# yangt1013/SPEINet

Measured on AMD Instinct MI355X. Metric: deblurred 720p frames/sec, higher is better.
Workload: dtype f16 (correlation top2)

## Files before the change

include/speinet_hip.h:

```cpp
#ifndef SPEINET_HIP_H
#define SPEINET_HIP_H

#include <stdint.h>

#ifdef __cplusplus
extern "C" {
#endif

typedef void* spei_stream_t;

#define SPEI_ACT_NONE 0
#define SPEI_ACT_RELU 1
#define SPEI_ACT_GELU 2

#define SPEI_F32 0
#define SPEI_BF16 1
#define SPEI_F16 2

#define SPEI_CONV 0
#define SPEI_CONV_TRANSPOSED 1

int spei_version(void);
const char* spei_last_error(void);
const char* spei_arch(void);

int spei_any_nonzero(const float* x, int64_t n, int32_t* flag, spei_stream_t stream);

int spei_rl_prior(const float* img, float* out, float* scratch, int C, int H, int W, int iters, float lam,
                  spei_stream_t stream);

int spei_conv5_in(const float* img_chw, const float* w, const float* bias, float* out_hwc, int H, int W,
                  int Cout, spei_stream_t stream);

int spei_conv5_out(const float* in_hwc, int ldi, const float* w, const float* bias, float* out_chw, int H,
                   int W, int Cin, spei_stream_t stream);

int spei_igemm_f32(const float* a0, int lda0, int k0, const float* a1, int lda1, int k1, const float* w,
                   const float* bias, float* out, int ldo, const float* residual, int ldr,
                   const float* rowscale, int Hin, int Win, int Hout, int Wout, int N, int ksize, int stride,
                   int pad, int mode, int act, spei_stream_t stream);

int spei_igemm_f32_batched(const float* a0, int lda0, int k0, const float* a1, int lda1, int k1, const float* w,
                           const float* bias, float* out, int ldo, const float* residual, int ldr,
                           const float* rowscale, int Hin, int Win, int Hout, int Wout, int N, int ksize, int stride,
                           int pad, int mode, int act, int batch, spei_stream_t stream);

int spei_conv_slab16(int fmt, const void* a0, int lda0, int k0, const void* a1, int lda1, int k1, int a_fmt,
                     const void* wfrag_hi, const void* wfrag_lo, const float* bias, void* out, int ldo, int out_fmt,
                     const float* residual, int ldr, const float* rowscale, int Hin, int Win, int Hout, int Wout,
                     int N, int ksize, int stride, int pad, int act, int ln_input, spei_stream_t stream);

int spei_conv_slab16_batched(int fmt, const void* a0, int k0, int a_fmt, const void* wfrag, const void* wfrag_lo, const float* bias,
                             void* out, int out_fmt, const float* residual, int batch, int Hin, int Win, int Hout, int Wout, int N,
                             int ksize, int stride, int pad, int act, spei_stream_t stream);

int spei_conv32_ws16(int fmt, const void* a, int a_fmt, const void* wfrag, const float* bias, void* out, int out_fmt, int batch,
                     int H, int W, int act, spei_stream_t stream);

int spei_conv64_ws16(int fmt, const void* a, int a_fmt, const void* wfrag, const float* bias, void* out, int out_fmt, int batch,
                     int H, int W, int act, spei_stream_t stream);

int spei_mlp_fused16(int fmt, const float* x, float* out, const void* w1_frag, const float* b1, const void* w2_frag,
                     const float* b2, int64_t M, spei_stream_t stream);

int spei_convt2_slab16(int fmt, const void* a0, int lda0, int k0, int a_fmt, const void* wfrag00, const void* wfrag01,
                       const void* wfrag10, const void* wfrag11, const float* bias, void* out, int ldo, int out_fmt,
                       int Hin, int Win, int N, int act, spei_stream_t stream);

int spei_convt2_slab16x3(const float* a0, int lda0, int k0, const void* const* whi4, const void* const* wlo4, const float* bias,
                         float* out, int ldo, int Hin, int Win, int N, int act, spei_stream_t stream);

int spei_conv3x3_256_pipe16(int fmt, const float* x, const void* w_frag, const float* bias, const float* residual, float* out,
                            int batch, int H, int W, spei_stream_t stream);

int spei_conv5_out_slab16(int fmt, const void* in, int ldi, int in_fmt, const void* wfrag, const float* bias32, float* out_chw,
                          int H, int W, spei_stream_t stream);

int spei_attn_fused16(int fmt, const float* x, float* out, const void* yhat, const void* wq_frag, const float* bq,
                      const void* wkv_frag, const float* bkv, const void* wproj_frag, const float* bproj,
                      const float* relbias, int H, int W, int shift, spei_stream_t stream);

int spei_attn_win4_16(int fmt, const float* x, float* out, const void* yhat, const void* wq_frag, const float* bq,
                      const void* wkv_frag, const float* bkv, const void* wproj_frag, const float* bproj,
                      const float* relbias, int batch, int H, int W, int shift, spei_stream_t stream);

int64_t spei_frame_metrics_ws_doubles(int H, int W, int border);
int spei_frame_metrics(const unsigned char* out_hwc, const unsigned char* gt_hwc, int H, int W, int border, double* ws, double* result,
                       spei_stream_t stream);

int64_t spei_gate_ws_floats(int H, int W, int C);
int spei_resblock_gates(const void* x1, int x1_fmt, int H, int W, int C, const float* se_w1, const float* se_b1,
                        const float* se_w2, const float* se_b2, const float* cw_w, const float* cw_bn,
                        const float* hc_w, const float* hc_bn, float* s, float* g1, float* g2, float* ws,
                        spei_stream_t stream);
int spei_resblock_apply(const float* x, const void* x1, int x1_fmt, const float* s, const float* g1, const float* g2,
                        const float* extra, float* out, int ldo, int H, int W, int C, spei_stream_t stream);

int spei_resblock_gates_batched(const void* x1, int x1_fmt, int batch, int H, int W, int C, const float* se_w1, const float* se_b1,
                                const float* se_w2, const float* se_b2, const float* cw_w, const float* cw_bn, const float* hc_w,
                                const float* hc_bn, float* s, float* g1, float* g2, float* ws, spei_stream_t stream);
int spei_resblock_apply_batched(const float* x, const void* x1, int x1_fmt, const float* s, const float* g1, const float* g2, float* out,
                                int batch, int H, int W, int C, spei_stream_t stream);

int spei_layernorm256(const float* x, void* y, int out_fmt, const float* gamma, const float* beta, int64_t M,
                      spei_stream_t stream);

int spei_window_attention(const void* q, const void* kv, int io_fmt, const float* relbias, void* out, int H, int W,
                          int shift, spei_stream_t stream);
int spei_window_attention_batched(const void* q, const void* kv, int io_fmt, const float* relbias, void* out, int H, int W,
                                  int shift, int batch, spei_stream_t stream);

int spei_patch_invnorm(const float* f, int ldf, float* inv, int H, int W, int C, spei_stream_t stream);

int64_t spei_corr_ws_floats(int64_t n_lr);
int spei_corr_argmax(const float* lr, int ldl, const float* ref, int ldr, const float* inv_lr,
                     const float* inv_ref, int Hl, int Wl, int Hr, int Wr, int C, float* S, int32_t* arg,
                     float* ws, spei_stream_t stream);

int spei_split16(int fmt, const float* x, int ld, void* hi, void* lo, int64_t M, int C, spei_stream_t stream);
int spei_corr_argmax_bf16(const void* lr_hi, const void* lr_lo, const void* ref_hi, const void* ref_lo,
                          const float* inv_lr, const float* inv_ref, int Hl, int Wl, int Hr, int Wr, int C, float* S,
                          int32_t* arg, float* ws, spei_stream_t stream);

int spei_corr_slab16(int fmt, const void* lr_hi, const void* lr_lo, const void* ref_hi, const void* ref_lo,
                     const float* inv_lr, const float* inv_ref, int Hl, int Wl, int Hr, int Wr, int C, float* S,
                     int32_t* arg, float* ws, spei_stream_t stream);

int spei_corr_slab_top2_16(int fmt, const void* lr16, const void* ref16, const float* inv_lr, const float* inv_ref,
                           int Hl, int Wl, int Hr, int Wr, int C, float* S, int32_t* arg, float* S2, int32_t* arg2,
                           float* ws, spei_stream_t stream);
int64_t spei_corr_diag_ws_floats(int Hl, int Wl, int Hr, int Wr);
int spei_corr_diag_top2_16(int fmt, const void* lr16, const void* ref16, const float* inv_ref, int Hl, int Wl, int Hr, int Wr,
                           int C, float* S, int32_t* arg, float* S2, int32_t* arg2, float* ws, spei_stream_t stream);
int spei_corr_rescore(const float* lr, int ldl, const float* ref, int ldr, const float* inv_lr, const float* inv_ref,
                      int Hl, int Wl, int Hr, int Wr, int C, float* S, int32_t* arg, const float* S2, const int32_t* arg2,
                      spei_stream_t stream);

int spei_gather_fold(const float* ref, int ldr, const int32_t* arg, float* out, int ldo, int H3, int W3,
                     int Hr3, int Wr3, int C, int s, spei_stream_t stream);

int spei_rot90(const float* in, int ldi, float* out, int H, int W, int C, spei_stream_t stream);

int spei_upsample_bicubic(const float* in, int ldi, float* out, int ldo, int H, int W, int C, int s, int act,
                          spei_stream_t stream);

int spei_add(const float* a, const float* b, float* out, int64_t n, spei_stream_t stream);


int64_t spei_wgrad_ws_floats(int Hout, int Wout, int N, int K, int ksize);
int spei_conv_wgrad_f32(const float* x, int ldx, const float* dy, int ldy, float* dw, float* dbias, float* ws, int Hin, int Win,
                        int Hout, int Wout, int N, int K, int ksize, int stride, int pad, spei_stream_t stream);

int spei_conv_wgrad_f32_batched(const float* x, int ldx, const float* dy, int ldy, float* dw, float* dbias, float* ws, int Hin, int Win,
                                int Hout, int Wout, int N, int K, int ksize, int stride, int pad, int batch, spei_stream_t stream);

int spei_pack_split16(const float* w, int N, int K, int ksize, int mode, void* frag_hi, void* frag_lo, spei_stream_t stream);

int spei_conv_wgrad_bf16x3_batched(const float* x, int ldx, const float* dy, int ldy, float* dw, float* dbias, float* ws, int Hin, int Win,
                                   int Hout, int Wout, int N, int K, int ksize, int stride, int pad, int batch, spei_stream_t stream);

int spei_conv_wgrad_bf16_batched(const float* x, int ldx, const float* dy, int ldy, float* dw, float* dbias, float* ws, int Hin, int Win,
                                 int Hout, int Wout, int N, int K, int ksize, int stride, int pad, int batch, spei_stream_t stream);

int spei_conv_s2_adjoint_slab16(const float* dy, int k0, const void* const* wfrag4, float* out, int N, int Hin, int Win, int ksize,
                                int batch, spei_stream_t stream);

int spei_relu_bwd(const float* y, const float* dy, float* dz, int64_t n, spei_stream_t stream);

int64_t spei_plane_ws_floats(int H, int W, int C);
int spei_plane_stats(const float* a, const float* b, int prod, int H, int W, int C, float* rowmax, int* rowarg, float* rowmean,
                     float* colmax, int* colarg, float* colmean, float* mean, float* ws, spei_stream_t stream);

int spei_plane_stats_batched(const float* a, const float* b, int prod, int H, int W, int C, float* rowmax, int* rowarg, float* rowmean,
                             float* colmax, int* colarg, float* colmean, float* mean, float* ws, int batch, spei_stream_t stream);

int spei_resblock_apply_bwd(const float* dout, const float* s, const float* g1, const float* g2, const int* rowarg, const int* colarg,
                            const float* d_rowmax, const float* d_rowmean, const float* d_colmax, const float* d_colmean,
                            const float* d_mean, float* dx1, int H, int W, int C, spei_stream_t stream);
int spei_resblock_apply_bwd_batched(const float* dout, const float* s, const float* g1, const float* g2, const int* rowarg,
                                    const int* colarg, const float* d_rowmax, const float* d_rowmean, const float* d_colmax,
                                    const float* d_colmean, const float* d_mean, float* dx1, int batch, int H, int W, int C,
                                    spei_stream_t stream);

int64_t spei_gate_train_saved_floats(int N, int groups, int H, int W, int C);
int64_t spei_gate_train_ws_floats(int N, int groups, int H, int W, int C);
int spei_gate_train_nparams(int C);
int spei_gate_maps_fwd(const float* rowmax, const float* rowmean, const float* colmax, const float* colmean, const float* mean,
                       const float* const* prm, float* const* run, int N, int groups, int H, int W, int C, int bn_train,
                       int update_running, float* s, float* g1, float* g2, float* saved, float* ws, spei_stream_t stream);
int spei_gate_maps_bwd(const float* rowmax, const float* rowmean, const float* colmax, const float* colmean, const float* mean,
                       const float* const* prm, float* const* run, int N, int groups, int H, int W, int C, int bn_train,
                       const float* s, const float* saved, const float* ds, const float* dg1, const float* dg2, float* d_rowmax,
                       float* d_rowmean, float* d_colmax, float* d_colmean, float* d_mean, float* dprm, float* ws,
                       spei_stream_t stream);


int64_t spei_ln_bwd_blocks(int64_t M);
int spei_layernorm256_bwd(const float* x, const float* gamma, const float* dy, float* dx, float* part, int64_t M, spei_stream_t stream);

int spei_gelu_fwd(const float* pre, float* out, int64_t n, spei_stream_t stream);
int spei_gelu_bwd(const float* pre, const float* dy, float* dpre, int64_t n, spei_stream_t stream);

int spei_window_attention_bwd(const float* q, const float* kv, const float* relbias, const float* dout, float* dq, float* dkv,
                              float* dbias_part, int H, int W, int shift, int batch, spei_stream_t stream);

int spei_window_attention16_train(const float* q, const float* kv, const float* relbias, float* out, int H, int W, int shift, int batch,
                                  spei_stream_t stream);
int spei_window_attention16_bwd(const float* q, const float* kv, const float* relbias, const float* dout, float* dq, float* dkv,
                                float* dbias_part, int H, int W, int shift, int batch, spei_stream_t stream);

int spei_scale_rows(const float* x, const float* rowscale, float* out, int64_t M, int N, spei_stream_t stream);


int spei_corr_s_bwd_lr(const float* lr, const float* ref, const float* inv_lr, const float* inv_ref, const float* S, const int32_t* arg,
                       const float* dS, float* dlr, int H, int W, int Hr, int Wr, int C, spei_stream_t stream);

int spei_search_bwd_ref(const float* ref, const float* dT, const float* lr, const float* inv_lr, const float* inv_ref, const float* S,
                        const float* dS, const int32_t* order, const int32_t* start, float* dref, int H3, int W3, int Hr3, int Wr3,
                        int C, int s, spei_stream_t stream);

int spei_upsample_bicubic_bwd(const float* dy, float* dx, int H, int W, int C, int s, spei_stream_t stream);

int spei_rowdot(const float* a, const float* b, float* out, int64_t M, int N, spei_stream_t stream);

int spei_det_gray(const float* rgb, float* gray, int N, int H, int W, spei_stream_t stream);
int64_t spei_det_ws_floats(int N, int H, int W, int k);
int spei_det_features(const float* gray, float* out, float* ws, int N, int H, int W, int k, spei_stream_t stream);


int spei_frames_u8_in(const unsigned char* src, int64_t frame_stride, float* dst, float* gray, int N, int H, int W, spei_stream_t stream);

int spei_frame_u8_out(const float* src, unsigned char* dst, int* nonfinite, int H, int W, int Hp, int Wp, spei_stream_t stream);


#define SPEI_CROP_HFLIP 1
#define SPEI_CROP_VFLIP 2
#define SPEI_CROP_ROT90 4
#define SPEI_CROP_ZERO 8
typedef struct {
    uint64_t src;
    int32_t pitch;
    int32_t y0, x0;
    int32_t flags;
    int32_t H, W;
} spei_crop_record;

int spei_train_batch_u8(const spei_crop_record* table, const spei_crop_record* table_host, int n_in, int n_gt, float* input, float* gt,
                        int P, float rgb_range, spei_stream_t stream);

#define SPEI_PSNR_WS_DOUBLES 256
int spei_psnr_f32(const float* a, const float* b, int H, int W, int shave, float rgb_range, double* ws, double* result,
                  spei_stream_t stream);


int spei_window_mean_u8(const unsigned char* src, int64_t frame_stride, int T, const int* runs, const int* runs_host, int M,
                        unsigned char* blur, unsigned char* gt, float* gray, int H, int W, spei_stream_t stream);

#ifdef __cplusplus
}
#endif
#endif
```

speinet_amd/csrc/common.h:

```cpp
#pragma once
#include <hip/hip_runtime.h>
#include <stdint.h>
#include <stdio.h>
#include "../../include/speinet_hip.h"

void spei_set_error(const char* fmt, ...);

#define SPEI_REQUIRE(cond, ...)            \
    do {                                   \
        if (!(cond)) {                     \
            spei_set_error(__VA_ARGS__);   \
            return -1;                     \
        }                                  \
    } while (0)

#define SPEI_CHECK_LAUNCH(name)                                                          \
    do {                                                                                 \
        hipError_t e__ = hipGetLastError();                                              \
        if (e__ != hipSuccess) {                                                         \
            spei_set_error("%s: launch failed: %s", name, hipGetErrorString(e__));       \
            return -2;                                                                   \
        }                                                                                \
    } while (0)

static inline int cdiv(int64_t a, int64_t b) { return (int)((a + b - 1) / b); }

#ifdef SPEI_TUNING
#include <stdlib.h>
static inline int spei_knob(const char* name, int dflt) { const char* v = getenv(name); return v ? atoi(v) : dflt; }
static inline long long* spei_stamp_buffer() { const char* v = getenv("SPEI_STAMP_PTR"); return v ? (long long*)strtoull(v, nullptr, 0) : nullptr; }
#define SPEI_STAMP(buf, i)                                                                            \
    do {                                                                                              \
        if ((buf) && threadIdx.x == 0) (buf)[(size_t)blockIdx.x * 16 + (i)] = __builtin_amdgcn_s_memrealtime(); \
    } while (0)
#define SPEI_STAMP_CLK(buf, i)                                                                        \
    do {                                                                                              \
        if ((buf) && threadIdx.x == 0) (buf)[(size_t)blockIdx.x * 16 + (i)] = __builtin_readcyclecounter(); \
    } while (0)
#define SPEI_STAMP_AT(buf, i, t)                                                                      \
    do {                                                                                              \
        if ((buf) && threadIdx.x == (t)) (buf)[(size_t)blockIdx.x * 16 + (i)] = __builtin_amdgcn_s_memrealtime(); \
    } while (0)
#else
static constexpr int spei_knob(const char*, int dflt) { return dflt; }
static inline long long* spei_stamp_buffer() { return nullptr; }
#define SPEI_STAMP(buf, i) do { } while (0)
#define SPEI_STAMP_CLK(buf, i) do { } while (0)
#define SPEI_STAMP_AT(buf, i, t) do { } while (0)
#endif

template <auto Kernel>
inline void ensure_dyn_lds(size_t lds) {
    static size_t have[32] = {};
    int dev = 0;
    (void)hipGetDevice(&dev);
    if (dev < 0 || dev >= 32 || lds > have[dev]) {
        (void)hipFuncSetAttribute(reinterpret_cast<const void*>(Kernel), hipFuncAttributeMaxDynamicSharedMemorySize, (int)lds);
        if (dev >= 0 && dev < 32) have[dev] = lds;
    }
}

inline int spei_num_cus() {
    static int have[32] = {};
    int dev = 0;
    (void)hipGetDevice(&dev);
    if (dev < 0 || dev >= 32) return 256;
    if (have[dev] == 0) {
        int n = 0;
        if (hipDeviceGetAttribute(&n, hipDeviceAttributeMultiprocessorCount, dev) != hipSuccess || n <= 0) n = 256;
        have[dev] = n;
    }
    return have[dev];
}

__device__ __forceinline__ void spei_stagger_start(int ntiles, int unit) {
    const int G = gridDim.x, b = blockIdx.x;
    const int mine = (ntiles - b + G - 1) / G, most = (ntiles + G - 1) / G;
    const int phase = (mine < most ? 4 : 0) + ((b >> 3) & 3);
    for (int i = 0; i < phase * unit; ++i) __builtin_amdgcn_s_sleep(32);
}

template <int CTRL>
__device__ __forceinline__ float dpp_mov(float v) {
    return __int_as_float(__builtin_amdgcn_update_dpp(0, __float_as_int(v), CTRL, 0xF, 0xF, true));
}
struct OpSum { static __device__ __forceinline__ float f(float a, float b) { return a + b; } };
struct OpMax { static __device__ __forceinline__ float f(float a, float b) { return fmaxf(a, b); } };
template <int M, typename Op>
__device__ __forceinline__ float xor_combine(float v) {
    if constexpr (M == 8) {
        return Op::f(v, dpp_mov<0x128>(v));
    } else if constexpr (M == 16) {
        const auto r = __builtin_amdgcn_permlane16_swap(__float_as_uint(v), __float_as_uint(v), false, false);
        return Op::f(__uint_as_float(r[0]), __uint_as_float(r[1]));
    } else {
        static_assert(M == 32, "xor_combine: M must be 8, 16 or 32");
        const auto r = __builtin_amdgcn_permlane32_swap(__float_as_uint(v), __float_as_uint(v), false, false);
        return Op::f(__uint_as_float(r[0]), __uint_as_float(r[1]));
    }
}
template <typename Op>
__device__ __forceinline__ float wave_allreduce(float v) {
    v = Op::f(v, dpp_mov<0xB1>(v));
    v = Op::f(v, dpp_mov<0x4E>(v));
    v = Op::f(v, dpp_mov<0x141>(v));
    v = Op::f(v, dpp_mov<0x140>(v));
    v = xor_combine<16, Op>(v);
    return xor_combine<32, Op>(v);
}
__device__ __forceinline__ float wave_sum(float v) { return wave_allreduce<OpSum>(v); }
__device__ __forceinline__ float wave_max(float v) { return wave_allreduce<OpMax>(v); }

__device__ __forceinline__ void lds_barrier() { asm volatile("s_waitcnt lgkmcnt(0)\n\ts_barrier" ::: "memory"); }

typedef float f32x16 __attribute__((ext_vector_type(16)));
typedef float f32x4 __attribute__((ext_vector_type(4)));

template <typename T>
struct lpv {
    typedef T x8 __attribute__((ext_vector_type(8)));
    typedef T x4 __attribute__((ext_vector_type(4)));
    typedef T x2 __attribute__((ext_vector_type(2)));
};
__device__ __forceinline__ f32x16 mfma16(lpv<__bf16>::x8 a, lpv<__bf16>::x8 b, f32x16 c) {
    return __builtin_amdgcn_mfma_f32_32x32x16_bf16(a, b, c, 0, 0, 0);
}
__device__ __forceinline__ f32x16 mfma16(lpv<_Float16>::x8 a, lpv<_Float16>::x8 b, f32x16 c) {
    return __builtin_amdgcn_mfma_f32_32x32x16_f16(a, b, c, 0, 0, 0);
}
template <typename LP>
__device__ __forceinline__ LP to_lp(float v) { return (LP)v; }
template <typename LP>
__device__ __forceinline__ typename lpv<LP>::x4 to_lp4(f32x4 v) {
    typename lpv<LP>::x4 h;
    h[0] = to_lp<LP>(v[0]); h[1] = to_lp<LP>(v[1]); h[2] = to_lp<LP>(v[2]); h[3] = to_lp<LP>(v[3]);
    return h;
}
typedef unsigned u32x4 __attribute__((ext_vector_type(4)));

template <int CTRL>
__device__ __forceinline__ float dpp_quad(float v) {
    return __int_as_float(__builtin_amdgcn_update_dpp(0, __float_as_int(v), CTRL, 0xF, 0xF, true));
}
__device__ __forceinline__ void quad_transpose4(float& a0, float& a1, float& a2, float& a3, int t) {
    const bool b0 = t & 1, b1 = t & 2;
    float s = b0 ? a0 : a1, r = dpp_quad<0xB1>(s);
    if (b0) a0 = r; else a1 = r;
    s = b0 ? a2 : a3; r = dpp_quad<0xB1>(s);
    if (b0) a2 = r; else a3 = r;
    s = b1 ? a0 : a2; r = dpp_quad<0x4E>(s);
    if (b1) a0 = r; else a2 = r;
    s = b1 ? a1 : a3; r = dpp_quad<0x4E>(s);
    if (b1) a1 = r; else a3 = r;
}

__device__ __forceinline__ float spei_gray_px(float r, float g, float b) {
    return __fmaf_rn(0.114f, b, __fmaf_rn(0.2989f, r, 0.587f * g)) / 255.0f;
}
```

speinet_amd/csrc/search.hip:

```cpp
#include "common.h"

namespace {

__global__ __launch_bounds__(256) void patch_invnorm_kernel(const float* __restrict__ f, int ldf, float* __restrict__ inv,
                                                            int H, int W, int C) {
    const int lane = threadIdx.x & 63;
    const int64_t p = (int64_t)blockIdx.x * 4 + (threadIdx.x >> 6);
    if (p >= (int64_t)H * W) return;
    const int y = (int)(p / W), x = (int)(p % W);
    float acc = 0.f;
    for (int dy = -1; dy <= 1; ++dy) {
        const int yy = y + dy;
        if (yy < 0 || yy >= H) continue;
        for (int dx = -1; dx <= 1; ++dx) {
            const int xx = x + dx;
            if (xx < 0 || xx >= W) continue;
            const float* row = f + ((size_t)yy * W + xx) * ldf;
            for (int c = lane; c < C; c += 64) acc = fmaf(row[c], row[c], acc);
        }
    }
    acc = wave_sum(acc);
    if (lane == 0) inv[p] = 1.0f / fmaxf(sqrtf(acc), 1e-12f);
}

constexpr int CBM = 128, CBN = 128, CBK = 32, CLD = CBK + 1, CMAXSPLIT = 8;

struct CorrParams {
    const float* lr;
    const float* ref;
    const float* inv_lr;
    const float* inv_ref;
    float* pval;
    int32_t* pidx;
    int ldl, ldr, Hl, Wl, Hr, Wr, C, Nl, Nr, njt, jt_per_split;
};

__device__ __forceinline__ bool better(float v, int i, float bv, int bi) { return v > bv || (v == bv && i < bi); }

__global__ __launch_bounds__(256) void corr_argmax_kernel(const CorrParams p) {
    extern __shared__ __attribute__((aligned(16))) float smem[];
    float* As = smem;
    float* Bs = smem + 2 * CBM * CLD;
    const int tid = threadIdx.x, lane = tid & 63, wave = tid >> 6;
    const int wm = wave >> 1, wn = wave & 1;
    const int fr = lane & 31, fk = lane >> 5;
    const int i0 = blockIdx.x * CBN;
    const int jt0 = blockIdx.y * p.jt_per_split;
    const int jt1 = min(p.njt, jt0 + p.jt_per_split);
    const int lrow = tid >> 3, lcol = (tid & 7) * 4;
    const int kchunks = p.C / CBK;
    const int per_tile = 9 * kchunks;

    int b_y[4], b_x[4];
#pragma unroll
    for (int j = 0; j < 4; ++j) {
        const int i = i0 + lrow + 32 * j;
        if (i < p.Nl) { b_y[j] = i / p.Wl; b_x[j] = i - b_y[j] * p.Wl; }
        else { b_y[j] = -0x10000000; b_x[j] = 0; }
    }
    int a_y[4], a_x[4];
    auto set_jtile = [&](int jt) {
#pragma unroll
        for (int j = 0; j < 4; ++j) {
            const int jj = jt * CBM + lrow + 32 * j;
            if (jj < p.Nr) { a_y[j] = jj / p.Wr; a_x[j] = jj - a_y[j] * p.Wr; }
            else { a_y[j] = -0x10000000; a_x[j] = 0; }
        }
    };
    float4 ra[4], rb[4];
    auto load_tile = [&](int it) {
        const int t = it / kchunks, kc = it - t * kchunks;
        const int ty = t / 3 - 1, tx = t - (t / 3) * 3 - 1;
        const int kofs = kc * CBK + lcol;
#pragma unroll
        for (int j = 0; j < 4; ++j) {
            const int yy = a_y[j] + ty, xx = a_x[j] + tx;
            ra[j] = ((yy >= 0) & (yy < p.Hr) & (xx >= 0) & (xx < p.Wr))
                        ? *reinterpret_cast<const float4*>(p.ref + ((size_t)yy * p.Wr + xx) * p.ldr + kofs)
                        : make_float4(0.f, 0.f, 0.f, 0.f);
            const int y2 = b_y[j] + ty, x2 = b_x[j] + tx;
            rb[j] = ((y2 >= 0) & (y2 < p.Hl) & (x2 >= 0) & (x2 < p.Wl))
                        ? *reinterpret_cast<const float4*>(p.lr + ((size_t)y2 * p.Wl + x2) * p.ldl + kofs)
                        : make_float4(0.f, 0.f, 0.f, 0.f);
        }
    };
    auto store_tile = [&](int buf) {
        float* a = As + buf * CBM * CLD;
        float* b = Bs + buf * CBN * CLD;
#pragma unroll
        for (int j = 0; j < 4; ++j) {
            float* d = a + (lrow + 32 * j) * CLD + lcol;
            d[0] = ra[j].x; d[1] = ra[j].y; d[2] = ra[j].z; d[3] = ra[j].w;
            d = b + (lrow + 32 * j) * CLD + lcol;
            d[0] = rb[j].x; d[1] = rb[j].y; d[2] = rb[j].z; d[3] = rb[j].w;
        }
    };

    float bestv[2] = {-INFINITY, -INFINITY};
    int besti[2] = {0x7fffffff, 0x7fffffff};
    float il[2];
#pragma unroll
    for (int tn = 0; tn < 2; ++tn) {
        const int i = i0 + (wn * 2 + tn) * 32 + fr;
        il[tn] = i < p.Nl ? p.inv_lr[i] : 0.f;
    }

    f32x16 acc[2][2];
    int buf = 0;
    if (jt0 < jt1) {
        set_jtile(jt0);
        load_tile(0);
        store_tile(0);
    }
    __syncthreads();
    for (int jt = jt0; jt < jt1; ++jt) {
#pragma unroll
        for (int a = 0; a < 2; ++a)
#pragma unroll
            for (int b = 0; b < 2; ++b)
#pragma unroll
                for (int r = 0; r < 16; ++r) acc[a][b][r] = 0.f;
        for (int it = 0; it < per_tile; ++it) {
            const bool last = (it + 1 == per_tile);
            const bool more = !last || (jt + 1 < jt1);
            if (more) {
                if (last) set_jtile(jt + 1);
                load_tile(last ? 0 : it + 1);
            }
            const float* a = As + buf * CBM * CLD + (wm * 64 + fr) * CLD + fk;
            const float* b = Bs + buf * CBN * CLD + (wn * 64 + fr) * CLD + fk;
#pragma unroll
            for (int kk = 0; kk < CBK; kk += 2) {
                const float a0 = a[kk], a1 = a[32 * CLD + kk];
                const float b0 = b[kk], b1 = b[32 * CLD + kk];
                acc[0][0] = __builtin_amdgcn_mfma_f32_32x32x2f32(a0, b0, acc[0][0], 0, 0, 0);
                acc[0][1] = __builtin_amdgcn_mfma_f32_32x32x2f32(a0, b1, acc[0][1], 0, 0, 0);
                acc[1][0] = __builtin_amdgcn_mfma_f32_32x32x2f32(a1, b0, acc[1][0], 0, 0, 0);
                acc[1][1] = __builtin_amdgcn_mfma_f32_32x32x2f32(a1, b1, acc[1][1], 0, 0, 0);
            }
            if (more) store_tile(buf ^ 1);
            __syncthreads();
            buf ^= 1;
        }
#pragma unroll
        for (int tm = 0; tm < 2; ++tm) {
#pragma unroll
            for (int r = 0; r < 16; ++r) {
                const int j = jt * CBM + (wm * 2 + tm) * 32 + (r & 3) + 8 * (r >> 2) + 4 * fk;
                if (j < p.Nr) {
                    const float ir = p.inv_ref[j];
#pragma unroll
                    for (int tn = 0; tn < 2; ++tn) {
                        const float v = acc[tm][tn][r] * ir * il[tn];
                        if (v > bestv[tn]) { bestv[tn] = v; besti[tn] = j; }
                    }
                }
            }
        }
    }
    __syncthreads();
    float* rv = smem;
    int* ri = reinterpret_cast<int*>(smem + 2 * CBN);
#pragma unroll
    for (int tn = 0; tn < 2; ++tn) {
        const float ov = __shfl_xor(bestv[tn], 32, 64);
        const int oi = __shfl_xor(besti[tn], 32, 64);
        if (better(ov, oi, bestv[tn], besti[tn])) { bestv[tn] = ov; besti[tn] = oi; }
        if (fk == 0) {
            const int col = (wn * 2 + tn) * 32 + fr;
            rv[wm * CBN + col] = bestv[tn];
            ri[wm * CBN + col] = besti[tn];
        }
    }
    __syncthreads();
    if (tid < CBN) {
        const int i = i0 + tid;
        if (i < p.Nl) {
            float v = rv[tid];
            int ix = ri[tid];
            if (better(rv[CBN + tid], ri[CBN + tid], v, ix)) { v = rv[CBN + tid]; ix = ri[CBN + tid]; }
            p.pval[(size_t)blockIdx.y * p.Nl + i] = v;
            p.pidx[(size_t)blockIdx.y * p.Nl + i] = ix;
        }
    }
}

__global__ __launch_bounds__(256) void corr_final_kernel(const float* __restrict__ pval, const int32_t* __restrict__ pidx,
                                                         int splits, int Nl, float* __restrict__ S, int32_t* __restrict__ arg) {
    const int i = blockIdx.x * 256 + threadIdx.x;
    if (i >= Nl) return;
    float v = pval[i];
    int ix = pidx[i];
    for (int s = 1; s < splits; ++s) {
        const float ov = pval[(size_t)s * Nl + i];
        const int oi = pidx[(size_t)s * Nl + i];
        if (better(ov, oi, v, ix)) { v = ov; ix = oi; }
    }
    S[i] = v;
    arg[i] = ix == 0x7fffffff ? 0 : ix;
}

__global__ __launch_bounds__(256) void corr_rescore_kernel(const float* __restrict__ lr, int ldl, const float* __restrict__ ref, int ldr,
                                                           const float* __restrict__ inv_lr, const float* __restrict__ inv_ref,
                                                           int Hl, int Wl, int Hr, int Wr, int C, float* __restrict__ S,
                                                           int32_t* __restrict__ arg, const int32_t* __restrict__ arg2) {
    const int lane = threadIdx.x & 63;
    const int64_t q = (int64_t)blockIdx.x * 4 + (threadIdx.x >> 6);
    if (q >= (int64_t)Hl * Wl) return;
    const int qy = (int)(q / Wl), qx = (int)(q - (int64_t)qy * Wl);
    int cand[2] = {arg[q], arg2[q]};
    const int nc = cand[1] >= 0 ? 2 : 1;
    double d[2] = {0.0, 0.0};
    for (int t = 0; t < 9; ++t) {
        const int ty = t / 3 - 1, tx = t - (t / 3) * 3 - 1;
        const int y = qy + ty, x = qx + tx;
        if (y < 0 || y >= Hl || x < 0 || x >= Wl) continue;
        const float* a = lr + ((size_t)y * Wl + x) * ldl;
        for (int k = 0; k < nc; ++k) {
            const int cy = cand[k] / Wr + ty, cx = cand[k] % Wr + tx;
            if (cy < 0 || cy >= Hr || cx < 0 || cx >= Wr) continue;
            const float* b = ref + ((size_t)cy * Wr + cx) * ldr;
            double acc = 0.0;
            for (int c = lane * 2; c < C; c += 128) {
                const float2 av = *reinterpret_cast<const float2*>(a + c);
                const float2 bv = *reinterpret_cast<const float2*>(b + c);
                acc += (double)av.x * (double)bv.x + (double)av.y * (double)bv.y;
            }
            d[k] += acc;
        }
    }
    for (int k = 0; k < 2; ++k)
        for (int m = 32; m >= 1; m >>= 1) d[k] += __shfl_xor(d[k], m, 64);
    if (lane == 0) {
        const double s0 = d[0] * (double)inv_ref[cand[0]];
        int win = cand[0];
        double sw = s0;
        if (nc == 2) {
            const double s1 = d[1] * (double)inv_ref[cand[1]];
            if (s1 > s0 || (s1 == s0 && cand[1] < cand[0])) { win = cand[1]; sw = s1; }
        }
        S[q] = (float)(sw * (double)inv_lr[q]);
        arg[q] = win;
    }
}

__global__ __launch_bounds__(256) void gather_fold_kernel(const float* __restrict__ ref, int ldr, const int32_t* __restrict__ arg,
                                                          float* __restrict__ out, int ldo, int H3, int W3, int Hr3, int Wr3,
                                                          int C, int s) {
    const int cg = C / 4;
    const int Ho = H3 * s, Wo = W3 * s, Hs = Hr3 * s, Wsrc = Wr3 * s;
    const int64_t total = (int64_t)Ho * Wo * cg;
    for (int64_t i = (int64_t)blockIdx.x * 256 + threadIdx.x; i < total; i += (int64_t)gridDim.x * 256) {
        const int c = (int)(i % cg) * 4;
        const int64_t pix = i / cg;
        const int x = (int)(pix % Wo), y = (int)(pix / Wo);
        const int by = y / s, bx = x / s;
        int a9[9];
        bool ok9[9];
#pragma unroll
        for (int t = 0; t < 9; ++t) {
            const int qy = by + 1 - t / 3, qx = bx + 1 - t % 3;
            ok9[t] = qy >= 0 && qy < H3 && qx >= 0 && qx < W3;
            a9[t] = arg[min(max(qy, 0), H3 - 1) * W3 + min(max(qx, 0), W3 - 1)];
        }
        float4 v9[9];
#pragma unroll
        for (int t = 0; t < 9; ++t) {
            const int qy = by + 1 - t / 3, qx = bx + 1 - t % 3;
            const int py = y - qy * s + s, px = x - qx * s + s;
            const int ay = a9[t] / Wr3, ax = a9[t] - ay * Wr3;
            const int sy = ay * s - s + py, sx = ax * s - s + px;
            ok9[t] = ok9[t] && sy >= 0 && sy < Hs && sx >= 0 && sx < Wsrc;
            v9[t] = *reinterpret_cast<const float4*>(ref + ((size_t)min(max(sy, 0), Hs - 1) * Wsrc + min(max(sx, 0), Wsrc - 1)) * ldr + c);
        }
        float4 acc = make_float4(0.f, 0.f, 0.f, 0.f);
#pragma unroll
        for (int t = 0; t < 9; ++t)
            if (ok9[t]) { acc.x += v9[t].x; acc.y += v9[t].y; acc.z += v9[t].z; acc.w += v9[t].w; }
        *reinterpret_cast<float4*>(out + pix * ldo + c) = make_float4(acc.x / 9.0f, acc.y / 9.0f, acc.z / 9.0f, acc.w / 9.0f);
    }
}

}

extern "C" int spei_patch_invnorm(const float* f, int ldf, float* inv, int H, int W, int C, spei_stream_t stream) {
    SPEI_REQUIRE(f && inv && H > 0 && W > 0 && C > 0 && ldf >= C, "spei_patch_invnorm: bad arguments");
    hipLaunchKernelGGL(patch_invnorm_kernel, dim3(cdiv((int64_t)H * W, 4)), dim3(256), 0, (hipStream_t)stream, f, ldf, inv, H, W, C);
    SPEI_CHECK_LAUNCH("spei_patch_invnorm");
    return 0;
}

extern "C" int64_t spei_corr_ws_floats(int64_t n_lr) { return 4 * (int64_t)CMAXSPLIT * n_lr; }

extern "C" int spei_corr_argmax(const float* lr, int ldl, const float* ref, int ldr, const float* inv_lr,
                                const float* inv_ref, int Hl, int Wl, int Hr, int Wr, int C, float* S, int32_t* arg,
                                float* ws, spei_stream_t stream) {
    SPEI_REQUIRE(lr && ref && inv_lr && inv_ref && S && arg && ws, "spei_corr_argmax: null pointer");
    SPEI_REQUIRE(C > 0 && C % 32 == 0 && ldl % 4 == 0 && ldr % 4 == 0 && ldl >= C && ldr >= C, "spei_corr_argmax: C=%d ldl=%d ldr=%d", C, ldl, ldr);
    SPEI_REQUIRE(Hl > 0 && Wl > 0 && Hr > 0 && Wr > 0, "spei_corr_argmax: empty map");
    SPEI_REQUIRE((int64_t)Hl * Wl < (1ll << 30) && (int64_t)Hr * Wr < (1ll << 30), "spei_corr_argmax: map too large");
    SPEI_REQUIRE(((uintptr_t)lr | (uintptr_t)ref) % 16 == 0, "spei_corr_argmax: 16-byte alignment required");
    CorrParams p;
    p.lr = lr; p.ref = ref; p.inv_lr = inv_lr; p.inv_ref = inv_ref;
    p.ldl = ldl; p.ldr = ldr; p.Hl = Hl; p.Wl = Wl; p.Hr = Hr; p.Wr = Wr; p.C = C;
    p.Nl = Hl * Wl; p.Nr = Hr * Wr;
    p.njt = cdiv(p.Nr, CBM);
    const int itiles = cdiv(p.Nl, CBN);
    int splits = 1024 / itiles;
    if (splits < 1) splits = 1;
    if (splits > CMAXSPLIT) splits = CMAXSPLIT;
    if (splits > p.njt) splits = p.njt;
    p.jt_per_split = cdiv(p.njt, splits);
    splits = cdiv(p.njt, p.jt_per_split);
    p.pval = ws;
    p.pidx = reinterpret_cast<int32_t*>(ws + (size_t)CMAXSPLIT * p.Nl);
    const size_t lds = (size_t)2 * (CBM + CBN) * CLD * sizeof(float);
    ensure_dyn_lds<&corr_argmax_kernel>(lds);
    hipStream_t st = (hipStream_t)stream;
    hipLaunchKernelGGL(corr_argmax_kernel, dim3(itiles, splits), dim3(256), lds, st, p);
    hipLaunchKernelGGL(corr_final_kernel, dim3(cdiv(p.Nl, 256)), dim3(256), 0, st, p.pval, p.pidx, splits, p.Nl, S, arg);
    SPEI_CHECK_LAUNCH("spei_corr_argmax");
    return 0;
}

extern "C" int spei_corr_rescore(const float* lr, int ldl, const float* ref, int ldr, const float* inv_lr, const float* inv_ref,
                                 int Hl, int Wl, int Hr, int Wr, int C, float* S, int32_t* arg, const float* S2, const int32_t* arg2,
                                 spei_stream_t stream) {
    (void)S2;
    SPEI_REQUIRE(lr && ref && inv_lr && inv_ref && S && arg && arg2, "spei_corr_rescore: null pointer");
    SPEI_REQUIRE(C > 0 && C % 2 == 0 && ldl % 2 == 0 && ldr % 2 == 0 && ldl >= C && ldr >= C, "spei_corr_rescore: C=%d ldl=%d ldr=%d", C, ldl, ldr);
    SPEI_REQUIRE(Hl > 0 && Wl > 0 && Hr > 0 && Wr > 0, "spei_corr_rescore: empty map");
    SPEI_REQUIRE(((uintptr_t)lr | (uintptr_t)ref) % 8 == 0, "spei_corr_rescore: 8-byte alignment required");
    hipLaunchKernelGGL(corr_rescore_kernel, dim3(cdiv((int64_t)Hl * Wl, 4)), dim3(256), 0, (hipStream_t)stream, lr, ldl, ref, ldr, inv_lr,
                       inv_ref, Hl, Wl, Hr, Wr, C, S, arg, arg2);
    SPEI_CHECK_LAUNCH("spei_corr_rescore");
    return 0;
}

extern "C" int spei_gather_fold(const float* ref, int ldr, const int32_t* arg, float* out, int ldo, int H3, int W3,
                                int Hr3, int Wr3, int C, int s, spei_stream_t stream) {
    SPEI_REQUIRE(ref && arg && out, "spei_gather_fold: null pointer");
    SPEI_REQUIRE((s == 1 || s == 2 || s == 4) && C % 4 == 0 && ldr % 4 == 0 && ldo % 4 == 0 && ldr >= C && ldo >= C,
                 "spei_gather_fold: s=%d C=%d ldr=%d ldo=%d", s, C, ldr, ldo);
    SPEI_REQUIRE(H3 > 0 && W3 > 0 && Hr3 > 0 && Wr3 > 0, "spei_gather_fold: empty map");
    const int64_t total = (int64_t)H3 * s * W3 * s * (C / 4);
    const int blocks = (int)((total + 255) / 256 < 16384 ? (total + 255) / 256 : 16384);
    hipLaunchKernelGGL(gather_fold_kernel, dim3(blocks), dim3(256), 0, (hipStream_t)stream, ref, ldr, arg, out, ldo, H3, W3, Hr3, Wr3, C, s);
    SPEI_CHECK_LAUNCH("spei_gather_fold");
    return 0;
}
```

speinet_amd/csrc/search_bf16.hip:

```cpp
#include "common.h"

namespace {

typedef __bf16 bf16x8 __attribute__((ext_vector_type(8)));
typedef __bf16 bf16x4 __attribute__((ext_vector_type(4)));

template <typename LP>
__global__ __launch_bounds__(256) void split16_kernel(const float* __restrict__ x, int ld, LP* __restrict__ hi,
                                                      LP* __restrict__ lo, int64_t M, int C) {
    typedef typename lpv<LP>::x4 lp4;
    const int cg = C / 4;
    const int64_t total = M * cg;
    for (int64_t i = (int64_t)blockIdx.x * 256 + threadIdx.x; i < total; i += (int64_t)gridDim.x * 256) {
        const int c = (int)(i % cg) * 4;
        const int64_t m = i / cg;
        const float4 v = *reinterpret_cast<const float4*>(x + m * ld + c);
        lp4 h;
        h[0] = (LP)v.x; h[1] = (LP)v.y; h[2] = (LP)v.z; h[3] = (LP)v.w;
        *reinterpret_cast<lp4*>(hi + m * C + c) = h;
        if (lo) {
            lp4 l;
            l[0] = (LP)(v.x - (float)h[0]); l[1] = (LP)(v.y - (float)h[1]);
            l[2] = (LP)(v.z - (float)h[2]); l[3] = (LP)(v.w - (float)h[3]);
            *reinterpret_cast<lp4*>(lo + m * C + c) = l;
        }
    }
}

constexpr int CBM = 128, CBN = 128, CMAXSPLIT = 8;

struct CorrParams {
    const __bf16* lrh;
    const __bf16* lrl;
    const __bf16* refh;
    const __bf16* refl;
    const float* inv_lr;
    const float* inv_ref;
    float* pval;
    int32_t* pidx;
    int Hl, Wl, Hr, Wr, C, Nl, Nr, njt, jt_per_split;
};

__device__ __forceinline__ bool better(float v, int i, float bv, int bi) { return v > bv || (v == bv && i < bi); }

template <int BK, bool SPLIT>
__global__ __launch_bounds__(256) void corr_bf16_kernel(const CorrParams p) {
    constexpr int PITCH = 2 * BK + 16;
    constexpr int TPR = BK / 8;
    constexpr int RPP = 256 / TPR;
    constexpr int NP = 128 / RPP;
    constexpr int NPART = SPLIT ? 2 : 1;
    constexpr int T_BYTES = 128 * PITCH;
    constexpr int BUF_BYTES = 2 * NPART * T_BYTES;
    extern __shared__ __attribute__((aligned(16))) unsigned char smem[];
    const int tid = threadIdx.x, lane = tid & 63, wave = tid >> 6;
    const int wm = wave >> 1, wn = wave & 1;
    const int fr = lane & 31, fk = lane >> 5;
    const int i0 = blockIdx.x * CBN;
    const int jt0 = blockIdx.y * p.jt_per_split;
    const int jt1 = min(p.njt, jt0 + p.jt_per_split);
    const int lrow = tid / TPR, lcol = (tid % TPR) * 8;
    const int kchunks = p.C / BK;
    const int per_tile = 9 * kchunks;

    int b_y[NP], b_x[NP], a_y[NP], a_x[NP];
#pragma unroll
    for (int j = 0; j < NP; ++j) {
        const int i = i0 + lrow + RPP * j;
        if (i < p.Nl) { b_y[j] = i / p.Wl; b_x[j] = i - b_y[j] * p.Wl; }
        else { b_y[j] = -0x10000000; b_x[j] = 0; }
    }
    auto set_jtile = [&](int jt) {
#pragma unroll
        for (int j = 0; j < NP; ++j) {
            const int jj = jt * CBM + lrow + RPP * j;
            if (jj < p.Nr) { a_y[j] = jj / p.Wr; a_x[j] = jj - a_y[j] * p.Wr; }
            else { a_y[j] = -0x10000000; a_x[j] = 0; }
        }
    };
    u32x4 rah[NP], rbh[NP], ral[SPLIT ? NP : 1], rbl[SPLIT ? NP : 1];
    const u32x4 zero = u32x4{0u, 0u, 0u, 0u};
    auto load_tile = [&](int it) {
        const int t = it / kchunks, kc = it - t * kchunks;
        const int ty = t / 3 - 1, tx = t - (t / 3) * 3 - 1;
        const int kofs = kc * BK + lcol;
#pragma unroll
        for (int j = 0; j < NP; ++j) {
            const int yy = a_y[j] + ty, xx = a_x[j] + tx;
            const bool oka = (yy >= 0) & (yy < p.Hr) & (xx >= 0) & (xx < p.Wr);
            const size_t oa = ((size_t)yy * p.Wr + xx) * p.C + kofs;
            rah[j] = oka ? *reinterpret_cast<const u32x4*>(p.refh + oa) : zero;
            if (SPLIT) ral[j] = oka ? *reinterpret_cast<const u32x4*>(p.refl + oa) : zero;
            const int y2 = b_y[j] + ty, x2 = b_x[j] + tx;
            const bool okb = (y2 >= 0) & (y2 < p.Hl) & (x2 >= 0) & (x2 < p.Wl);
            const size_t ob = ((size_t)y2 * p.Wl + x2) * p.C + kofs;
            rbh[j] = okb ? *reinterpret_cast<const u32x4*>(p.lrh + ob) : zero;
            if (SPLIT) rbl[j] = okb ? *reinterpret_cast<const u32x4*>(p.lrl + ob) : zero;
        }
    };
    auto store_tile = [&](int buf) {
        unsigned char* base = smem + buf * BUF_BYTES;
#pragma unroll
        for (int j = 0; j < NP; ++j) {
            const int o = (lrow + RPP * j) * PITCH + lcol * 2;
            *reinterpret_cast<u32x4*>(base + o) = rah[j];
            if (SPLIT) *reinterpret_cast<u32x4*>(base + T_BYTES + o) = ral[j];
            *reinterpret_cast<u32x4*>(base + NPART * T_BYTES + o) = rbh[j];
            if (SPLIT) *reinterpret_cast<u32x4*>(base + (NPART + 1) * T_BYTES + o) = rbl[j];
        }
    };

    float bestv[2] = {-INFINITY, -INFINITY};
    int besti[2] = {0x7fffffff, 0x7fffffff};
    float il[2];
#pragma unroll
    for (int tn = 0; tn < 2; ++tn) {
        const int i = i0 + (wn * 2 + tn) * 32 + fr;
        il[tn] = i < p.Nl ? p.inv_lr[i] : 0.f;
    }

    f32x16 acc[2][2];
    int buf = 0;
    if (jt0 < jt1) {
        set_jtile(jt0);
        load_tile(0);
        store_tile(0);
    }
    __syncthreads();
    for (int jt = jt0; jt < jt1; ++jt) {
#pragma unroll
        for (int a = 0; a < 2; ++a)
#pragma unroll
            for (int b = 0; b < 2; ++b)
#pragma unroll
                for (int r = 0; r < 16; ++r) acc[a][b][r] = 0.f;
        for (int it = 0; it < per_tile; ++it) {
            const bool last = (it + 1 == per_tile);
            const bool more = !last || (jt + 1 < jt1);
            if (more) {
                if (last) set_jtile(jt + 1);
                load_tile(last ? 0 : it + 1);
            }
            const unsigned char* base = smem + buf * BUF_BYTES;
            const unsigned char* pa = base + (wm * 64 + fr) * PITCH + fk * 16;
            const unsigned char* pb = base + NPART * T_BYTES + (wn * 64 + fr) * PITCH + fk * 16;
#pragma unroll
            for (int ks = 0; ks < BK / 16; ++ks) {
                bf16x8 av[2], bv[2], avl[2], bvl[2];
#pragma unroll
                for (int i = 0; i < 2; ++i) {
                    av[i] = *reinterpret_cast<const bf16x8*>(pa + i * 32 * PITCH + ks * 32);
                    bv[i] = *reinterpret_cast<const bf16x8*>(pb + i * 32 * PITCH + ks * 32);
                    if (SPLIT) {
                        avl[i] = *reinterpret_cast<const bf16x8*>(pa + T_BYTES + i * 32 * PITCH + ks * 32);
                        bvl[i] = *reinterpret_cast<const bf16x8*>(pb + T_BYTES + i * 32 * PITCH + ks * 32);
                    }
                }
#pragma unroll
                for (int i = 0; i < 2; ++i)
#pragma unroll
                    for (int j = 0; j < 2; ++j) {
                        if (SPLIT) {
                            acc[i][j] = __builtin_amdgcn_mfma_f32_32x32x16_bf16(avl[i], bv[j], acc[i][j], 0, 0, 0);
                            acc[i][j] = __builtin_amdgcn_mfma_f32_32x32x16_bf16(av[i], bvl[j], acc[i][j], 0, 0, 0);
                        }
                        acc[i][j] = __builtin_amdgcn_mfma_f32_32x32x16_bf16(av[i], bv[j], acc[i][j], 0, 0, 0);
                    }
            }
            if (more) store_tile(buf ^ 1);
            __syncthreads();
            buf ^= 1;
        }
#pragma unroll
        for (int tm = 0; tm < 2; ++tm) {
#pragma unroll
            for (int r = 0; r < 16; ++r) {
                const int j = jt * CBM + (wm * 2 + tm) * 32 + (r & 3) + 8 * (r >> 2) + 4 * fk;
                if (j < p.Nr) {
                    const float ir = p.inv_ref[j];
#pragma unroll
                    for (int tn = 0; tn < 2; ++tn) {
                        const float v = acc[tm][tn][r] * ir * il[tn];
                        if (v > bestv[tn]) { bestv[tn] = v; besti[tn] = j; }
                    }
                }
            }
        }
    }
    __syncthreads();
    float* rv = reinterpret_cast<float*>(smem);
    int* ri = reinterpret_cast<int*>(smem) + 2 * CBN;
#pragma unroll
    for (int tn = 0; tn < 2; ++tn) {
        const float ov = __shfl_xor(bestv[tn], 32, 64);
        const int oi = __shfl_xor(besti[tn], 32, 64);
        if (better(ov, oi, bestv[tn], besti[tn])) { bestv[tn] = ov; besti[tn] = oi; }
        if (fk == 0) {
            const int col = (wn * 2 + tn) * 32 + fr;
            rv[wm * CBN + col] = bestv[tn];
            ri[wm * CBN + col] = besti[tn];
        }
    }
    __syncthreads();
    if (tid < CBN) {
        const int i = i0 + tid;
        if (i < p.Nl) {
            float v = rv[tid];
            int ix = ri[tid];
            if (better(rv[CBN + tid], ri[CBN + tid], v, ix)) { v = rv[CBN + tid]; ix = ri[CBN + tid]; }
            p.pval[(size_t)blockIdx.y * p.Nl + i] = v;
            p.pidx[(size_t)blockIdx.y * p.Nl + i] = ix;
        }
    }
}

__global__ __launch_bounds__(256) void corr_final_bf16_kernel(const float* __restrict__ pval, const int32_t* __restrict__ pidx,
                                                              int splits, int Nl, float* __restrict__ S, int32_t* __restrict__ arg) {
    const int i = blockIdx.x * 256 + threadIdx.x;
    if (i >= Nl) return;
    float v = pval[i];
    int ix = pidx[i];
    for (int s = 1; s < splits; ++s) {
        const float ov = pval[(size_t)s * Nl + i];
        const int oi = pidx[(size_t)s * Nl + i];
        if (better(ov, oi, v, ix)) { v = ov; ix = oi; }
    }
    S[i] = v;
    arg[i] = ix == 0x7fffffff ? 0 : ix;
}

template <int BK, bool SPLIT>
int launch_corr(const CorrParams& p, int itiles, int splits, hipStream_t st) {
    constexpr int PITCH = 2 * BK + 16;
    const size_t lds = (size_t)2 * 2 * (SPLIT ? 2 : 1) * 128 * PITCH;
    ensure_dyn_lds<&corr_bf16_kernel<BK, SPLIT>>(lds);
    hipLaunchKernelGGL((corr_bf16_kernel<BK, SPLIT>), dim3(itiles, splits), dim3(256), lds, st, p);
    return 0;
}

}

extern "C" int spei_split16(int fmt, const float* x, int ld, void* hi, void* lo, int64_t M, int C, spei_stream_t stream) {
    SPEI_REQUIRE(x && hi && M > 0 && C > 0 && C % 4 == 0 && ld % 4 == 0 && ld >= C, "spei_split16: bad arguments");
    SPEI_REQUIRE(fmt == SPEI_BF16 || fmt == SPEI_F16, "spei_split16: fmt=%d", fmt);
    const int64_t total = M * (C / 4);
    const int blocks = (int)((total + 255) / 256 < 8192 ? (total + 255) / 256 : 8192);
    if (fmt == SPEI_F16)
        hipLaunchKernelGGL(split16_kernel<_Float16>, dim3(blocks), dim3(256), 0, (hipStream_t)stream, x, ld, (_Float16*)hi, (_Float16*)lo, M, C);
    else
        hipLaunchKernelGGL(split16_kernel<__bf16>, dim3(blocks), dim3(256), 0, (hipStream_t)stream, x, ld, (__bf16*)hi, (__bf16*)lo, M, C);
    SPEI_CHECK_LAUNCH("spei_split16");
    return 0;
}

extern "C" int spei_corr_argmax_bf16(const void* lr_hi, const void* lr_lo, const void* ref_hi, const void* ref_lo,
                                     const float* inv_lr, const float* inv_ref, int Hl, int Wl, int Hr, int Wr, int C,
                                     float* S, int32_t* arg, float* ws, spei_stream_t stream) {
    SPEI_REQUIRE(lr_hi && ref_hi && inv_lr && inv_ref && S && arg && ws, "spei_corr_argmax_bf16: null pointer");
    SPEI_REQUIRE((lr_lo == nullptr) == (ref_lo == nullptr), "spei_corr_argmax_bf16: lo parts must both be given or both be NULL");
    SPEI_REQUIRE(C > 0 && C % 64 == 0, "spei_corr_argmax_bf16: C=%d must be a multiple of 64", C);
    SPEI_REQUIRE(Hl > 0 && Wl > 0 && Hr > 0 && Wr > 0, "spei_corr_argmax_bf16: empty map");
    SPEI_REQUIRE((int64_t)Hl * Wl < (1ll << 30) && (int64_t)Hr * Wr < (1ll << 30), "spei_corr_argmax_bf16: map too large");
    SPEI_REQUIRE(((uintptr_t)lr_hi | (uintptr_t)ref_hi | (uintptr_t)lr_lo | (uintptr_t)ref_lo) % 16 == 0, "spei_corr_argmax_bf16: 16-byte alignment required");
    CorrParams p;
    p.lrh = (const __bf16*)lr_hi; p.lrl = (const __bf16*)lr_lo; p.refh = (const __bf16*)ref_hi; p.refl = (const __bf16*)ref_lo;
    p.inv_lr = inv_lr; p.inv_ref = inv_ref;
    p.Hl = Hl; p.Wl = Wl; p.Hr = Hr; p.Wr = Wr; p.C = C;
    p.Nl = Hl * Wl; p.Nr = Hr * Wr;
    p.njt = cdiv(p.Nr, CBM);
    const int itiles = cdiv(p.Nl, CBN);
    int splits = 1024 / itiles;
    if (splits < 1) splits = 1;
    if (splits > CMAXSPLIT) splits = CMAXSPLIT;
    if (splits > p.njt) splits = p.njt;
    p.jt_per_split = cdiv(p.njt, splits);
    splits = cdiv(p.njt, p.jt_per_split);
    p.pval = ws;
    p.pidx = reinterpret_cast<int32_t*>(ws + (size_t)CMAXSPLIT * p.Nl);
    hipStream_t st = (hipStream_t)stream;
    if (lr_lo) launch_corr<32, true>(p, itiles, splits, st);
    else launch_corr<64, false>(p, itiles, splits, st);
    hipLaunchKernelGGL(corr_final_bf16_kernel, dim3(cdiv(p.Nl, 256)), dim3(256), 0, st, p.pval, p.pidx, splits, p.Nl, S, arg);
    SPEI_CHECK_LAUNCH("spei_corr_argmax_bf16");
    return 0;
}
```

speinet_amd/csrc/stencil.hip:

```cpp
#include <stdarg.h>
#include <string.h>
#include "common.h"

static thread_local char g_err[512] = "";
void spei_set_error(const char* fmt, ...) {
    va_list ap;
    va_start(ap, fmt);
    vsnprintf(g_err, sizeof(g_err), fmt, ap);
    va_end(ap);
}
extern "C" const char* spei_last_error(void) { return g_err; }
extern "C" int spei_version(void) { return 100; }
extern "C" const char* spei_arch(void) { return "gfx950"; }

__global__ void any_nonzero_kernel(const float* __restrict__ x, int64_t n, int32_t* flag) {
    int64_t i = (int64_t)blockIdx.x * blockDim.x + threadIdx.x;
    const int64_t step = (int64_t)gridDim.x * blockDim.x;
    bool nz = false;
    for (; i < n; i += step) nz |= (x[i] != 0.0f);
    if (__any(nz) && (threadIdx.x & 63) == 0) atomicOr(flag, 1);
}
extern "C" int spei_any_nonzero(const float* x, int64_t n, int32_t* flag, spei_stream_t stream) {
    SPEI_REQUIRE(x && flag && n > 0, "spei_any_nonzero: bad arguments");
    hipStream_t s = (hipStream_t)stream;
    (void)hipMemsetAsync(flag, 0, sizeof(int32_t), s);
    const int blocks = (int)((n + 256 * 16 - 1) / (256 * 16));
    hipLaunchKernelGGL(any_nonzero_kernel, dim3(blocks < 2048 ? blocks : 2048), dim3(256), 0, s, x, n, flag);
    SPEI_CHECK_LAUNCH("spei_any_nonzero");
    return 0;
}

constexpr int RL_T = 32;
__global__ __launch_bounds__(256) void rl_iter_kernel(const float* __restrict__ img, const float* __restrict__ d,
                                                      float* __restrict__ out, int H, int W, float lam) {
    __shared__ float t[RL_T + 4][RL_T + 4 + 1];
    const size_t plane = (size_t)blockIdx.z * H * W;
    const int x0 = blockIdx.x * RL_T, y0 = blockIdx.y * RL_T;
    for (int i = threadIdx.x; i < (RL_T + 4) * (RL_T + 4); i += 256) {
        const int ly = i / (RL_T + 4), lx = i - ly * (RL_T + 4);
        const int gy = y0 + ly - 2, gx = x0 + lx - 2;
        t[ly][lx] = (gy >= 0 && gy < H && gx >= 0 && gx < W) ? d[plane + (size_t)gy * W + gx] : 0.0f;
    }
    __syncthreads();
    const int lx = threadIdx.x & 31;
    for (int ly = threadIdx.x >> 5; ly < RL_T; ly += 8) {
        const int gy = y0 + ly, gx = x0 + lx;
        if (gy >= H || gx >= W) continue;
        float b = 0.0f;
#pragma unroll
        for (int dy = 0; dy < 5; ++dy)
#pragma unroll
            for (int dx = 0; dx < 5; ++dx) b = fmaf(t[ly + dy][lx + dx], 0.04f, b);
        const float c0 = t[ly + 2][lx + 2];
        float lap = -t[ly + 1][lx + 2];
        lap -= t[ly + 2][lx + 1];
        lap = fmaf(4.0f, c0, lap);
        lap -= t[ly + 2][lx + 3];
        lap -= t[ly + 3][lx + 2];
        const float I = img[plane + (size_t)gy * W + gx];
        float c = I / b;
        if (c != c) c = 0.0f;
        if (c < 0.0f) c = 0.0f;
        out[plane + (size_t)gy * W + gx] = c * (c0 + lam * lap);
    }
}
extern "C" int spei_rl_prior(const float* img, float* out, float* scratch, int C, int H, int W, int iters, float lam,
                             spei_stream_t stream) {
    SPEI_REQUIRE(img && out && scratch && C > 0 && H > 0 && W > 0 && iters >= 1, "spei_rl_prior: bad arguments");
    SPEI_REQUIRE(out != img && scratch != img && out != scratch, "spei_rl_prior: buffers must be distinct");
    hipStream_t s = (hipStream_t)stream;
    dim3 grid(cdiv(W, RL_T), cdiv(H, RL_T), C);
    const float* src = img;
    for (int it = 0; it < iters; ++it) {
        float* dst = ((iters - 1 - it) % 2 == 0) ? out : scratch;
        hipLaunchKernelGGL(rl_iter_kernel, grid, dim3(256), 0, s, img, src, dst, H, W, lam);
        src = dst;
    }
    SPEI_CHECK_LAUNCH("spei_rl_prior");
    return 0;
}

constexpr int CI_TH = 8, CI_TW = 32, CI_P = CI_TW + 4 + 1;
__global__ __launch_bounds__(256) void conv5_in_kernel(const float* __restrict__ img, const float* __restrict__ w,
                                                       const float* __restrict__ bias, float* __restrict__ out,
                                                       int H, int W, int tiles_x, int ntiles) {
    __shared__ float tin[3 * (CI_TH + 4) * CI_P];
    const int tid = threadIdx.x, lane = tid & 63, wave = tid >> 6;
    const int fr = lane & 31, fk = lane >> 5;
    int koff[38];
    float bw[38];
#pragma unroll
    for (int kk = 0; kk < 38; ++kk) {
        const int k = 2 * kk + fk;
        const int t = k / 3, ci = k - 3 * t;
        const int dy = t / 5, dx = t - 5 * dy;
        koff[kk] = k < 75 ? (ci * (CI_TH + 4) + dy) * CI_P + dx : 0;
        bw[kk] = k < 75 ? w[(t * 32 + fr) * 3 + ci] : 0.0f;
    }
    const float bv = bias[fr];
    const float* a0 = tin + (wave * 2) * CI_P + fr;
    const int et = fr & 3, ecol = (fr >> 2) * 4;
    for (int tile = blockIdx.x; tile < ntiles; tile += gridDim.x) {
        const int ty = tile / tiles_x, tx = tile - ty * tiles_x;
        const int x0 = tx * CI_TW, y0 = ty * CI_TH;
        for (int i = tid; i < 3 * (CI_TH + 4) * (CI_TW + 4); i += 256) {
            const int c = i / ((CI_TH + 4) * (CI_TW + 4));
            const int r = i - c * (CI_TH + 4) * (CI_TW + 4);
            const int ly = r / (CI_TW + 4), lx = r - ly * (CI_TW + 4);
            const int gy = y0 + ly - 2, gx = x0 + lx - 2;
            tin[(c * (CI_TH + 4) + ly) * CI_P + lx] = (gy >= 0 && gy < H && gx >= 0 && gx < W) ? img[((size_t)c * H + gy) * W + gx] : 0.0f;
        }
        __syncthreads();
        float av[2][38];
#pragma unroll
        for (int kk = 0; kk < 38; ++kk) {
            av[0][kk] = a0[koff[kk]];
            av[1][kk] = a0[koff[kk] + CI_P];
        }
        __syncthreads();
        f32x16 acc[2];
#pragma unroll
        for (int i = 0; i < 2; ++i)
#pragma unroll
            for (int r = 0; r < 16; ++r) acc[i][r] = 0.f;
#pragma unroll
        for (int kk = 0; kk < 38; ++kk) {
            acc[0] = __builtin_amdgcn_mfma_f32_32x32x2f32(av[0][kk], bw[kk], acc[0], 0, 0, 0);
            acc[1] = __builtin_amdgcn_mfma_f32_32x32x2f32(av[1][kk], bw[kk], acc[1], 0, 0, 0);
        }
#pragma unroll
        for (int i = 0; i < 2; ++i) {
            const int gy = y0 + wave * 2 + i;
#pragma unroll
            for (int k = 0; k < 4; ++k) {
                float a[4];
#pragma unroll
                for (int e = 0; e < 4; ++e) a[e] = fmaxf(acc[i][4 * k + e] + bv, 0.f);
                quad_transpose4(a[0], a[1], a[2], a[3], et);
                const int gx = x0 + 8 * k + 4 * fk + et;
                if (gy < H && gx < W) *reinterpret_cast<f32x4*>(out + ((size_t)gy * W + gx) * 32 + ecol) = f32x4{a[0], a[1], a[2], a[3]};
            }
        }
    }
}
extern "C" int spei_conv5_in(const float* img_chw, const float* w, const float* bias, float* out_hwc, int H, int W,
                             int Cout, spei_stream_t stream) {
    SPEI_REQUIRE(img_chw && w && bias && out_hwc && H > 0 && W > 0, "spei_conv5_in: bad arguments");
    SPEI_REQUIRE(Cout == 32, "spei_conv5_in: Cout=%d (only n_feat=32 is built)", Cout);
    const int tiles_x = cdiv(W, CI_TW), ntiles = tiles_x * cdiv(H, CI_TH);
    hipLaunchKernelGGL(conv5_in_kernel, dim3(ntiles < 1024 ? ntiles : 1024), dim3(256), 0, (hipStream_t)stream,
                       img_chw, w, bias, out_hwc, H, W, tiles_x, ntiles);
    SPEI_CHECK_LAUNCH("spei_conv5_in");
    return 0;
}

constexpr int CO_TH = 8, CO_TW = 32, CO_P = 36;
__global__ __launch_bounds__(256) void conv5_out_kernel(const float* __restrict__ in, int ldi, const float* __restrict__ w,
                                                        const float* __restrict__ bias, float* __restrict__ out,
                                                        int H, int W) {
    extern __shared__ __attribute__((aligned(16))) float sm[];
    float* tin = sm;
    float* wl = sm + (CO_TH + 4) * (CO_TW + 4) * CO_P;
    const int x0 = blockIdx.x * CO_TW, y0 = blockIdx.y * CO_TH;
    for (int i = threadIdx.x; i < (CO_TH + 4) * (CO_TW + 4) * 8; i += 256) {
        const int pix = i >> 3, q = i & 7;
        const int ly = pix / (CO_TW + 4), lx = pix - ly * (CO_TW + 4);
        const int gy = y0 + ly - 2, gx = x0 + lx - 2;
        float4 v = make_float4(0.f, 0.f, 0.f, 0.f);
        if (gy >= 0 && gy < H && gx >= 0 && gx < W) v = *reinterpret_cast<const float4*>(in + ((size_t)gy * W + gx) * ldi + q * 4);
        *reinterpret_cast<float4*>(tin + pix * CO_P + q * 4) = v;
    }
    for (int i = threadIdx.x; i < 25 * 3 * 32; i += 256) {
        const int t = i / 96, r = i - t * 96, co = r / 32, ci = r - co * 32;
        wl[(co * 25 + t) * 32 + ci] = w[i];
    }
    __syncthreads();
    const int lx = threadIdx.x & 31, ly = threadIdx.x >> 5;
    const int gy = y0 + ly, gx = x0 + lx;
    float a0 = bias[0], a1 = bias[1], a2 = bias[2];
    for (int t = 0; t < 25; ++t) {
        const int dy = t / 5, dx = t - dy * 5;
        const float4* pin = reinterpret_cast<const float4*>(tin + ((ly + dy) * (CO_TW + 4) + lx + dx) * CO_P);
        const float4* w0 = reinterpret_cast<const float4*>(wl + (0 * 25 + t) * 32);
        const float4* w1 = reinterpret_cast<const float4*>(wl + (1 * 25 + t) * 32);
        const float4* w2 = reinterpret_cast<const float4*>(wl + (2 * 25 + t) * 32);
#pragma unroll
        for (int q = 0; q < 8; ++q) {
            const float4 v = pin[q];
            const float4 u0 = w0[q], u1 = w1[q], u2 = w2[q];
            a0 = fmaf(v.x, u0.x, a0); a0 = fmaf(v.y, u0.y, a0); a0 = fmaf(v.z, u0.z, a0); a0 = fmaf(v.w, u0.w, a0);
            a1 = fmaf(v.x, u1.x, a1); a1 = fmaf(v.y, u1.y, a1); a1 = fmaf(v.z, u1.z, a1); a1 = fmaf(v.w, u1.w, a1);
            a2 = fmaf(v.x, u2.x, a2); a2 = fmaf(v.y, u2.y, a2); a2 = fmaf(v.z, u2.z, a2); a2 = fmaf(v.w, u2.w, a2);
        }
    }
    if (gy < H && gx < W) {
        const size_t o = (size_t)gy * W + gx, hw = (size_t)H * W;
        out[o] = a0; out[hw + o] = a1; out[2 * hw + o] = a2;
    }
}
extern "C" int spei_conv5_out(const float* in_hwc, int ldi, const float* w, const float* bias, float* out_chw, int H,
                              int W, int Cin, spei_stream_t stream) {
    SPEI_REQUIRE(in_hwc && w && bias && out_chw && H > 0 && W > 0, "spei_conv5_out: bad arguments");
    SPEI_REQUIRE(Cin == 32 && ldi % 4 == 0 && ldi >= 32, "spei_conv5_out: Cin=%d ldi=%d (only n_feat=32 is built)", Cin, ldi);
    const size_t lds = ((size_t)(CO_TH + 4) * (CO_TW + 4) * CO_P + 3 * 25 * 32) * sizeof(float);
    ensure_dyn_lds<&conv5_out_kernel>(lds);
    hipLaunchKernelGGL(conv5_out_kernel, dim3(cdiv(W, CO_TW), cdiv(H, CO_TH)), dim3(256), lds, (hipStream_t)stream,
                       in_hwc, ldi, w, bias, out_chw, H, W);
    SPEI_CHECK_LAUNCH("spei_conv5_out");
    return 0;
}

__device__ __forceinline__ void cubic_coeffs(float t, float c[4]) {
    const float A = -0.75f;
    float x = t + 1.0f;
    c[0] = ((A * x - 5.0f * A) * x + 8.0f * A) * x - 4.0f * A;
    x = t;
    c[1] = ((A + 2.0f) * x - (A + 3.0f)) * x * x + 1.0f;
    x = 1.0f - t;
    c[2] = ((A + 2.0f) * x - (A + 3.0f)) * x * x + 1.0f;
    x = 2.0f - t;
    c[3] = ((A * x - 5.0f * A) * x + 8.0f * A) * x - 4.0f * A;
}
template <int VEC>
__global__ __launch_bounds__(256) void bicubic_kernel(const float* __restrict__ in, int ldi, float* __restrict__ out, int ldo,
                                                      int H, int W, int C, int s, int relu) {
    const int cg = C / VEC;
    const int64_t total = (int64_t)H * s * W * s * cg;
    const float scale = 1.0f / (float)s;
    for (int64_t i = (int64_t)blockIdx.x * 256 + threadIdx.x; i < total; i += (int64_t)gridDim.x * 256) {
        const int c = (int)(i % cg) * VEC;
        const int64_t pix = i / cg;
        const int ox = (int)(pix % (W * s)), oy = (int)(pix / (W * s));
        const float ry = scale * ((float)oy + 0.5f) - 0.5f, rx = scale * ((float)ox + 0.5f) - 0.5f;
        const float fy = floorf(ry), fx = floorf(rx);
        float cy[4], cx[4];
        cubic_coeffs(ry - fy, cy);
        cubic_coeffs(rx - fx, cx);
        const int iy = (int)fy, ix = (int)fx;
        float acc[VEC];
#pragma unroll
        for (int a = 0; a < 4; ++a) {
            const int yy = min(max(iy - 1 + a, 0), H - 1);
            float row[VEC];
#pragma unroll
            for (int b = 0; b < 4; ++b) {
                const int xx = min(max(ix - 1 + b, 0), W - 1);
                const float* p = in + ((size_t)yy * W + xx) * ldi + c;
                if (VEC == 4) {
                    const float4 v = *reinterpret_cast<const float4*>(p);
                    const float vv[4] = {v.x, v.y, v.z, v.w};
#pragma unroll
                    for (int e = 0; e < VEC; ++e) row[e] = (b == 0) ? vv[e] * cx[0] : fmaf(vv[e], cx[b], row[e]);
                } else {
                    row[0] = (b == 0) ? p[0] * cx[0] : fmaf(p[0], cx[b], row[0]);
                }
            }
#pragma unroll
            for (int e = 0; e < VEC; ++e) acc[e] = (a == 0) ? row[e] * cy[0] : fmaf(row[e], cy[a], acc[e]);
        }
        if (relu) {
#pragma unroll
            for (int e = 0; e < VEC; ++e) acc[e] = fmaxf(acc[e], 0.f);
        }
        float* o = out + ((size_t)oy * (W * s) + ox) * ldo + c;
        if (VEC == 4) *reinterpret_cast<float4*>(o) = make_float4(acc[0], acc[1], acc[2], acc[3]);
        else o[0] = acc[0];
    }
}
__global__ __launch_bounds__(256) void bicubic2x_kernel(const float* __restrict__ in, int ldi, float* __restrict__ out, int ldo,
                                                        int H, int W, int C, int relu) {
    const int cg = C / 4;
    const int64_t total = (int64_t)H * W * cg;
    float ce[4], co[4];
    cubic_coeffs(0.75f, ce);
    cubic_coeffs(0.25f, co);
    for (int64_t i = (int64_t)blockIdx.x * 256 + threadIdx.x; i < total; i += (int64_t)gridDim.x * 256) {
        const int c = (int)(i % cg) * 4;
        const int64_t pix = i / cg;
        const int x = (int)(pix % W), y = (int)(pix / W);
        int xs[5];
#pragma unroll
        for (int b = 0; b < 5; ++b) xs[b] = min(max(x - 2 + b, 0), W - 1);
        f32x4 he[5], ho[5];
#pragma unroll
        for (int a = 0; a < 5; ++a) {
            const int yy = min(max(y - 2 + a, 0), H - 1);
            const float* rowp = in + (size_t)yy * W * ldi + c;
            f32x4 v[5];
#pragma unroll
            for (int b = 0; b < 5; ++b) v[b] = *reinterpret_cast<const f32x4*>(rowp + (size_t)xs[b] * ldi);
#pragma unroll
            for (int e = 0; e < 4; ++e) {
                float re = v[0][e] * ce[0], ro = v[1][e] * co[0];
#pragma unroll
                for (int b = 1; b < 4; ++b) { re = fmaf(v[b][e], ce[b], re); ro = fmaf(v[b + 1][e], co[b], ro); }
                he[a][e] = re;
                ho[a][e] = ro;
            }
        }
#pragma unroll
        for (int py = 0; py < 2; ++py)
#pragma unroll
            for (int px = 0; px < 2; ++px) {
                const f32x4* h = px ? ho : he;
                const float* cy = py ? co : ce;
                f32x4 acc;
#pragma unroll
                for (int e = 0; e < 4; ++e) {
                    float r = h[py][e] * cy[0];
#pragma unroll
                    for (int a = 1; a < 4; ++a) r = fmaf(h[py + a][e], cy[a], r);
                    acc[e] = relu ? fmaxf(r, 0.f) : r;
                }
                *reinterpret_cast<f32x4*>(out + ((size_t)(2 * y + py) * (2 * W) + 2 * x + px) * ldo + c) = acc;
            }
    }
}

extern "C" int spei_upsample_bicubic(const float* in, int ldi, float* out, int ldo, int H, int W, int C, int s, int act,
                                     spei_stream_t stream) {
    SPEI_REQUIRE(in && out && H > 0 && W > 0 && C > 0 && (s == 2 || s == 4), "spei_upsample_bicubic: bad arguments");
    SPEI_REQUIRE(act == SPEI_ACT_NONE || act == SPEI_ACT_RELU, "spei_upsample_bicubic: act=%d", act);
    SPEI_REQUIRE(ldi >= C && ldo >= C, "spei_upsample_bicubic: bad row strides");
    const bool v4 = (C % 4 == 0) && (ldi % 4 == 0) && (ldo % 4 == 0);
    if (v4 && s == 2 && ((uintptr_t)in | (uintptr_t)out) % 16 == 0) {
        const int64_t tot2 = (int64_t)H * W * (C / 4);
        const int blocks2 = (int)((tot2 + 255) / 256 < 8192 ? (tot2 + 255) / 256 : 8192);
        hipLaunchKernelGGL(bicubic2x_kernel, dim3(blocks2), dim3(256), 0, (hipStream_t)stream, in, ldi, out, ldo, H, W, C, act == SPEI_ACT_RELU);
        SPEI_CHECK_LAUNCH("spei_upsample_bicubic");
        return 0;
    }
    const int64_t total = (int64_t)H * s * W * s * (v4 ? C / 4 : C);
    const int blocks = (int)((total + 255) / 256 < 8192 ? (total + 255) / 256 : 8192);
    if (v4) hipLaunchKernelGGL(bicubic_kernel<4>, dim3(blocks), dim3(256), 0, (hipStream_t)stream, in, ldi, out, ldo, H, W, C, s, act == SPEI_ACT_RELU);
    else    hipLaunchKernelGGL(bicubic_kernel<1>, dim3(blocks), dim3(256), 0, (hipStream_t)stream, in, ldi, out, ldo, H, W, C, s, act == SPEI_ACT_RELU);
    SPEI_CHECK_LAUNCH("spei_upsample_bicubic");
    return 0;
}

__global__ __launch_bounds__(256) void rot90_kernel(const float* __restrict__ in, int ldi, float* __restrict__ out, int H, int W, int C) {
    const int cg = C / 4;
    const int64_t total = (int64_t)H * W * cg;
    for (int64_t i = (int64_t)blockIdx.x * 256 + threadIdx.x; i < total; i += (int64_t)gridDim.x * 256) {
        const int c = (int)(i % cg) * 4;
        const int64_t pix = i / cg;
        const int b = (int)(pix % H), a = (int)(pix / H);
        *reinterpret_cast<float4*>(out + ((size_t)a * H + b) * C + c) =
            *reinterpret_cast<const float4*>(in + ((size_t)b * W + (W - 1 - a)) * ldi + c);
    }
}
extern "C" int spei_rot90(const float* in, int ldi, float* out, int H, int W, int C, spei_stream_t stream) {
    SPEI_REQUIRE(in && out && H > 0 && W > 0 && C % 4 == 0 && ldi % 4 == 0, "spei_rot90: bad arguments");
    const int64_t total = (int64_t)H * W * (C / 4);
    const int blocks = (int)((total + 255) / 256 < 8192 ? (total + 255) / 256 : 8192);
    hipLaunchKernelGGL(rot90_kernel, dim3(blocks), dim3(256), 0, (hipStream_t)stream, in, ldi, out, H, W, C);
    SPEI_CHECK_LAUNCH("spei_rot90");
    return 0;
}

__global__ __launch_bounds__(256) void add_kernel(const float* __restrict__ a, const float* __restrict__ b, float* __restrict__ o, int64_t n4, int64_t n) {
    for (int64_t i = (int64_t)blockIdx.x * 256 + threadIdx.x; i < n4; i += (int64_t)gridDim.x * 256) {
        const float4 x = reinterpret_cast<const float4*>(a)[i], y = reinterpret_cast<const float4*>(b)[i];
        reinterpret_cast<float4*>(o)[i] = make_float4(x.x + y.x, x.y + y.y, x.z + y.z, x.w + y.w);
    }
    if (blockIdx.x == 0) for (int64_t i = n4 * 4 + threadIdx.x; i < n; i += 256) o[i] = a[i] + b[i];
}
extern "C" int spei_add(const float* a, const float* b, float* out, int64_t n, spei_stream_t stream) {
    SPEI_REQUIRE(a && b && out && n > 0, "spei_add: bad arguments");
    SPEI_REQUIRE(((uintptr_t)a | (uintptr_t)b | (uintptr_t)out) % 16 == 0, "spei_add: 16-byte alignment required");
    const int64_t n4 = n / 4;
    const int blocks = (int)((n4 + 255) / 256 < 4096 ? (n4 + 255) / 256 : 4096);
    hipLaunchKernelGGL(add_kernel, dim3(blocks > 0 ? blocks : 1), dim3(256), 0, (hipStream_t)stream, a, b, out, n4, n);
    SPEI_CHECK_LAUNCH("spei_add");
    return 0;
}
```

speinet_amd/csrc/swin.hip:

```cpp
#include "common.h"

namespace {

template <typename TO>
__global__ __launch_bounds__(256) void layernorm256_kernel(const float* __restrict__ x, TO* __restrict__ y,
                                                           const float* __restrict__ gamma, const float* __restrict__ beta,
                                                           int64_t M) {
    const int lane = threadIdx.x & 63;
    const int64_t wave = (int64_t)blockIdx.x * 4 + (threadIdx.x >> 6);
    const int64_t nwaves = (int64_t)gridDim.x * 4;
    float4 g = make_float4(1.f, 1.f, 1.f, 1.f), b = make_float4(0.f, 0.f, 0.f, 0.f);
    if (gamma) g = reinterpret_cast<const float4*>(gamma)[lane];
    if (beta) b = reinterpret_cast<const float4*>(beta)[lane];
    for (int64_t m = wave; m < M; m += nwaves) {
        const float4 v = reinterpret_cast<const float4*>(x + m * 256)[lane];
        const float mean = wave_sum((v.x + v.y) + (v.z + v.w)) * (1.0f / 256.0f);
        const float dx = v.x - mean, dy = v.y - mean, dz = v.z - mean, dw = v.w - mean;
        const float var = wave_sum((dx * dx + dy * dy) + (dz * dz + dw * dw)) * (1.0f / 256.0f);
        const float rstd = 1.0f / sqrtf(var + 1e-5f);
        float4 o;
        o.x = dx * rstd * g.x + b.x;
        o.y = dy * rstd * g.y + b.y;
        o.z = dz * rstd * g.z + b.z;
        o.w = dw * rstd * g.w + b.w;
        if (sizeof(TO) == 4) {
            reinterpret_cast<float4*>(y + m * 256)[lane] = o;
        } else {
            typename lpv<TO>::x4 h;
            h[0] = (TO)o.x; h[1] = (TO)o.y; h[2] = (TO)o.z; h[3] = (TO)o.w;
            reinterpret_cast<typename lpv<TO>::x4*>(y + m * 256)[lane] = h;
        }
    }
}

constexpr int WS = 5, NT = 25, HD = 32, LDT = HD + 1;

__device__ __forceinline__ int mask_region(int v, int n, int shift) {
    return v < n - WS ? 0 : (v < n - shift ? 1 : 2);
}

template <typename T>
__device__ __forceinline__ float4 load4(const T* p) {
    if constexpr (sizeof(T) == 4) {
        return *reinterpret_cast<const float4*>(p);
    } else {
        const typename lpv<T>::x4 h = *reinterpret_cast<const typename lpv<T>::x4*>(p);
        return make_float4((float)h[0], (float)h[1], (float)h[2], (float)h[3]);
    }
}

template <typename T>
__global__ __launch_bounds__(256) void window_attention_kernel(const T* __restrict__ q, const T* __restrict__ kv,
                                                               const float* __restrict__ relbias, T* __restrict__ out,
                                                               int H, int W, int shift) {
    __shared__ float sQ[4][32][LDT], sK[4][32][LDT], sV[4][32][LDT];
    __shared__ int tok_pix[32], tok_reg[32];
    {
        const size_t z = (size_t)blockIdx.y * H * W;
        q += z * 256; kv += z * 512; out += z * 256;
    }
    const int wave = threadIdx.x >> 6, lane = threadIdx.x & 63;
    const int nwx = W / WS;
    const int win = blockIdx.x >> 1;
    const int wy = win / nwx, wx = win - wy * nwx;
    if (threadIdx.x < 32) {
        int pix = 0, reg = 0;
        if (threadIdx.x < NT) {
            const int ys = wy * WS + threadIdx.x / WS, xs = wx * WS + threadIdx.x % WS;
            int yo = ys + shift, xo = xs + shift;
            if (yo >= H) yo -= H;
            if (xo >= W) xo -= W;
            pix = yo * W + xo;
            reg = shift > 0 ? 3 * mask_region(ys, H, shift) + mask_region(xs, W, shift) : 0;
        }
        tok_pix[threadIdx.x] = pix;
        tok_reg[threadIdx.x] = reg;
    }
    __syncthreads();
    const int h = (blockIdx.x & 1) * 4 + wave;
    const int hl = wave;
    for (int i = lane; i < 32 * 8; i += 64) {
        const int r = i >> 3, c4 = (i & 7) * 4;
        float4 vq = make_float4(0.f, 0.f, 0.f, 0.f), vk = vq, vv = vq;
        if (r < NT) {
            const size_t p = (size_t)tok_pix[r];
            vq = load4<T>(q + p * 256 + h * HD + c4);
            vk = load4<T>(kv + p * 512 + h * HD + c4);
            vv = load4<T>(kv + p * 512 + 256 + h * HD + c4);
        }
        float* d = &sQ[hl][r][c4]; d[0] = vq.x; d[1] = vq.y; d[2] = vq.z; d[3] = vq.w;
        d = &sK[hl][r][c4];        d[0] = vk.x; d[1] = vk.y; d[2] = vk.z; d[3] = vk.w;
        d = &sV[hl][r][c4];        d[0] = vv.x; d[1] = vv.y; d[2] = vv.z; d[3] = vv.w;
    }
    __syncthreads();
    const int fr = lane & 31, fk = lane >> 5;
    f32x16 st;
#pragma unroll
    for (int r = 0; r < 16; ++r) st[r] = 0.f;
#pragma unroll
    for (int kk = 0; kk < HD; kk += 2)
        st = __builtin_amdgcn_mfma_f32_32x32x2f32(sK[hl][fr][kk + fk], sQ[hl][fr][kk + fk], st, 0, 0, 0);
    const int qi = fr < NT ? fr : 0;
    const int qreg = tok_reg[qi];
    float mx = -INFINITY;
#pragma unroll
    for (int r = 0; r < 16; ++r) {
        const int key = (r & 3) + 8 * (r >> 2) + 4 * fk;
        float v = -INFINITY;
        if (key < NT) {
            v = st[r] + relbias[(h * NT + qi) * NT + key];
            if (shift > 0 && tok_reg[key] != qreg) v += -100.0f;
        }
        st[r] = v;
        mx = fmaxf(mx, v);
    }
    mx = fmaxf(mx, __shfl_xor(mx, 32, 64));
    float sum = 0.f;
#pragma unroll
    for (int r = 0; r < 16; ++r) {
        const float e = expf(st[r] - mx);
        st[r] = e;
        sum += e;
    }
    sum += __shfl_xor(sum, 32, 64);
    const float inv = 1.0f / sum;
    f32x16 o;
#pragma unroll
    for (int r = 0; r < 16; ++r) o[r] = 0.f;
#pragma unroll
    for (int r = 0; r < 16; ++r) {
        const int key = (r & 3) + 8 * (r >> 2) + 4 * fk;
        o = __builtin_amdgcn_mfma_f32_32x32x2f32(st[r] * inv, sV[hl][key][fr], o, 0, 0, 0);
    }
#pragma unroll
    for (int r = 0; r < 16; ++r) {
        const int qq = (r & 3) + 8 * (r >> 2) + 4 * fk;
        if (qq < NT) out[(size_t)tok_pix[qq] * 256 + h * HD + fr] = (T)o[r];
    }
}

}

extern "C" int spei_layernorm256(const float* x, void* y, int out_fmt, const float* gamma, const float* beta, int64_t M,
                                 spei_stream_t stream) {
    SPEI_REQUIRE(x && y && M > 0, "spei_layernorm256: bad arguments");
    SPEI_REQUIRE(out_fmt == SPEI_F32 || out_fmt == SPEI_BF16 || out_fmt == SPEI_F16, "spei_layernorm256: out_fmt=%d", out_fmt);
    const int64_t blocks = (M + 3) / 4;
    const dim3 grid((unsigned)(blocks < 8192 ? blocks : 8192));
    if (out_fmt == SPEI_BF16) hipLaunchKernelGGL(layernorm256_kernel<__bf16>, grid, dim3(256), 0, (hipStream_t)stream, x, (__bf16*)y, gamma, beta, M);
    else if (out_fmt == SPEI_F16) hipLaunchKernelGGL(layernorm256_kernel<_Float16>, grid, dim3(256), 0, (hipStream_t)stream, x, (_Float16*)y, gamma, beta, M);
    else hipLaunchKernelGGL(layernorm256_kernel<float>, grid, dim3(256), 0, (hipStream_t)stream, x, (float*)y, gamma, beta, M);
    SPEI_CHECK_LAUNCH("spei_layernorm256");
    return 0;
}

static int window_attention_run(const void* q, const void* kv, int io_fmt, const float* relbias, void* out, int H, int W, int shift, int batch,
                                spei_stream_t stream) {
    SPEI_REQUIRE(q && kv && relbias && out, "spei_window_attention: null pointer");
    SPEI_REQUIRE(batch >= 1 && batch <= 65535, "spei_window_attention: batch=%d", batch);
    SPEI_REQUIRE(H > 0 && W > 0 && H % WS == 0 && W % WS == 0, "spei_window_attention: %dx%d is not a multiple of the 5x5 window", H, W);
    SPEI_REQUIRE(shift >= 0 && shift < WS, "spei_window_attention: shift=%d", shift);
    SPEI_REQUIRE(io_fmt == SPEI_F32 || io_fmt == SPEI_BF16 || io_fmt == SPEI_F16, "spei_window_attention: io_fmt=%d", io_fmt);
    const dim3 grid(2 * (H / WS) * (W / WS), batch);
    if (io_fmt == SPEI_BF16) hipLaunchKernelGGL(window_attention_kernel<__bf16>, grid, dim3(256), 0, (hipStream_t)stream, (const __bf16*)q, (const __bf16*)kv, relbias, (__bf16*)out, H, W, shift);
    else if (io_fmt == SPEI_F16) hipLaunchKernelGGL(window_attention_kernel<_Float16>, grid, dim3(256), 0, (hipStream_t)stream, (const _Float16*)q, (const _Float16*)kv, relbias, (_Float16*)out, H, W, shift);
    else hipLaunchKernelGGL(window_attention_kernel<float>, grid, dim3(256), 0, (hipStream_t)stream, (const float*)q, (const float*)kv, relbias, (float*)out, H, W, shift);
    SPEI_CHECK_LAUNCH("spei_window_attention");
    return 0;
}

extern "C" int spei_window_attention(const void* q, const void* kv, int io_fmt, const float* relbias, void* out, int H, int W,
                                     int shift, spei_stream_t stream) {
    return window_attention_run(q, kv, io_fmt, relbias, out, H, W, shift, 1, stream);
}

extern "C" int spei_window_attention_batched(const void* q, const void* kv, int io_fmt, const float* relbias, void* out, int H, int W,
                                             int shift, int batch, spei_stream_t stream) {
    return window_attention_run(q, kv, io_fmt, relbias, out, H, W, shift, batch, stream);
}
```

speinet_amd/engine.py:

```python
from __future__ import annotations

import torch

from .ops import ACT_GELU, ACT_RELU, CONV_T, BMap, Ctx, FMap


def _resblocks(ctx: Ctx, f: FMap, blocks, extra=None, out=None) -> FMap:
    n = len(blocks)
    for i, pk in enumerate(blocks):
        last = i == n - 1
        f = ctx.resblock(f, pk, extra=extra if last else None, out=out if last else None)
    return f


def in_block(ctx: Ctx, frame: torch.Tensor, pk: dict) -> FMap:
    ctx = ctx.for_stage("enc")
    return _resblocks(ctx, ctx.conv5_in(frame, pk["head_w"], pk["head_b"]), pk["blocks"])


def enc_stage(ctx: Ctx, f: FMap, pk: dict, extra=None, out=None) -> FMap:
    ctx = ctx.for_stage("enc")
    n = pk["head_b"].numel()
    f = ctx.igemm(f, pk["head_w"], pk["head_b"], n, ksize=5, stride=2, act=ACT_RELU)
    return _resblocks(ctx, f, pk["blocks"], extra, out)


def enc(ctx: Ctx, frame: torch.Tensor, P: dict, extra=None, out=None) -> FMap:
    return enc_stage(ctx, enc_stage(ctx, in_block(ctx, frame, P["inBlock"]), P["encoder_first"]), P["encoder_second"], extra, out)


def enc_batched(ctx: Ctx, frames: list, P: dict):
    ctx = ctx.for_stage("enc")
    assert ctx.batched_available()
    b, (h, w) = len(frames), frames[0].shape[-2:]
    ib = P["inBlock"]
    lv1 = BMap.empty(b, h, w, ib["head_b"].numel(), frames[0].device)
    lib_in = lambda i: ctx.conv5_in(frames[i], ib["head_w"], ib["head_b"], out=lv1.map(i))
    for i in range(b):
        lib_in(i)
    for pk in ib["blocks"]:
        lv1 = ctx.resblock_batched(lv1, pk)
    levels = [lv1]
    f = lv1
    for name in ("encoder_first", "encoder_second"):
        st = P[name]
        f = ctx.igemm_batched(f, st["head_w"], st["head_b"], st["head_b"].numel(), 5, stride=2, act=ACT_RELU)
        for pk in st["blocks"]:
            f = ctx.resblock_batched(f, pk)
        levels.append(f)
    return levels


def dec_stage(ctx: Ctx, f: FMap, pk: dict) -> FMap:
    f = _resblocks(ctx, f, pk["blocks"])
    return ctx.for_stage("convt").igemm(f, pk["tail_w"], pk["tail_b"], pk["tail_b"].numel(), ksize=3, stride=2, mode=CONV_T, act=ACT_RELU)


class SwinX:

    def __init__(self, ctx: Ctx, f_mid: FMap, sw: dict):
        ctx = ctx.for_stage("swin")
        self.f_mid = f_mid
        self.x_first = ctx.igemm(f_mid, sw["conv_first_w"], sw["conv_first_b"], 256, ksize=3)
        self.xt0 = ctx.layernorm(self.x_first.t, sw["pe_g"], sw["pe_b"])


def swin(ctx: Ctx, sx: SwinX, feat: FMap, sw: dict, out: FMap) -> FMap:
    ctx = ctx.for_stage("swin")
    h, w = feat.H, feat.W
    m = h * w
    dev = feat.t.device
    y_first = ctx.igemm(feat, sw["conv_first_w"], sw["conv_first_b"], 256, ksize=3)
    yt = ctx.layernorm(y_first.t, sw["pe_g"], sw["pe_b"])
    idt = ctx.inter_dtype()
    yhat = ctx.layernorm(yt, out_dtype=idt)
    del y_first, yt
    r = sx.xt0.clone()
    bufs = [torch.empty(m, 256, device=dev), torch.empty(m, 256, device=dev)]
    xh = torch.empty(m, 256, device=dev, dtype=idt)
    q = torch.empty(m, 256, device=dev, dtype=idt)
    kv = torch.empty(m, 512, device=dev, dtype=idt)
    att = torch.empty(m, 256, device=dev, dtype=idt)
    hid = torch.empty(m, 512, device=dev, dtype=idt)
    for layer in sw["layers"]:
        cur = r
        for bi, bk in enumerate(layer["blocks"]):
            shift = 0 if bi % 2 == 0 else 2
            nxt = bufs[bi % 2]
            if ctx.attn_fused_available():
                ctx.attn_fused(cur, yhat, bk, h, w, shift, out=nxt)
            else:
                if ctx.ln_fused_available():
                    ctx.linear(cur, bk["wkv"], bk["bkv"], out=kv, ln_input=True)
                else:
                    ctx.layernorm(cur, out=xh)
                    ctx.linear(xh, bk["wkv"], bk["bkv"], out=kv)
                ctx.linear(yhat, bk["wq"], bk["bq"], out=q)
                ctx.window_attention(q, kv, bk["relbias"], h, w, shift, out=att)
                ctx.linear(att, bk["wproj"], bk["bproj"], residual=cur, out=nxt)
            if ctx.mlp_fused_available():
                ctx.mlp_fused(nxt, bk["w1"], bk["b1"], bk["w2"], bk["b2"], out=nxt)
            else:
                if ctx.ln_fused_available():
                    ctx.linear(nxt, bk["w1"], bk["b1"], act=ACT_GELU, out=hid, ln_input=True)
                else:
                    ctx.layernorm(nxt, out=xh)
                    ctx.linear(xh, bk["w1"], bk["b1"], act=ACT_GELU, out=hid)
                ctx.linear(hid, bk["w2"], bk["b2"], residual=nxt, out=nxt)
            cur = nxt
        rf = FMap(r, h, w, 256)
        ctx.igemm(FMap(cur, h, w, 256), layer["conv_w"], layer["conv_b"], 256, ksize=3, residual=rf, out=rf)
    xt = ctx.layernorm(r, sw["norm_g"], sw["norm_b"])
    res = ctx.igemm(FMap(xt, h, w, 256), sw["cab_w"], sw["cab_b"], 256, ksize=3, residual=sx.x_first)
    return ctx.igemm(res, sw["conv_last_w"], sw["conv_last_b"], 128, ksize=3, residual=sx.f_mid, out=out)


def swin_multi(ctx: Ctx, sx: SwinX, feats: BMap, sw: dict, outs: list) -> None:
    ctx = ctx.for_stage("swin")
    B, h, w = feats.B, feats.H, feats.W
    m = h * w
    dev = feats.t.device
    y_first = ctx.igemm_batched(feats, sw["conv_first_w"], sw["conv_first_b"], 256, 3)
    yt = ctx.layernorm(y_first.t, sw["pe_g"], sw["pe_b"])
    idt = ctx.inter_dtype()
    yhat = ctx.layernorm(yt, out_dtype=idt)
    del y_first, yt
    r = sx.xt0.repeat(B, 1)
    bufs = [torch.empty(B * m, 256, device=dev), torch.empty(B * m, 256, device=dev)]
    for layer in sw["layers"]:
        cur = r
        for bi, bk in enumerate(layer["blocks"]):
            shift = 0 if bi % 2 == 0 else 2
            nxt = bufs[bi % 2]
            ctx.attn_fused(cur, yhat, bk, h, w, shift, out=nxt)
            ctx.mlp_fused(nxt, bk["w1"], bk["b1"], bk["w2"], bk["b2"], out=nxt)
            cur = nxt
        rb = BMap(r, B, h, w, 256)
        ctx.igemm_batched(BMap(cur, B, h, w, 256), layer["conv_w"], layer["conv_b"], 256, 3, residual=rb, out=rb)
    xt = ctx.layernorm(r, sw["norm_g"], sw["norm_b"])
    x_first = BMap(sx.x_first.t.repeat(B, 1), B, h, w, 256)
    res = ctx.igemm_batched(BMap(xt, B, h, w, 256), sw["cab_w"], sw["cab_b"], 256, 3, residual=x_first)
    for b in range(B):
        ctx.igemm(res.map(b), sw["conv_last_w"], sw["conv_last_b"], 128, ksize=3, residual=sx.f_mid, out=outs[b])


def search_plan(ctx: Ctx, f_fusion: FMap, lv3: FMap):
    ctx = ctx.for_stage("search")
    return ctx.corr_plan(f_fusion, lv3, ctx.patch_invnorm(f_fusion), ctx.patch_invnorm(lv3))


def search_finish(ctx: Ctx, plan, f_fusion: FMap, lv1: FMap, lv2: FMap, lv3: FMap, return_arg=False):
    ctx = ctx.for_stage("search")
    s, arg = plan.s, plan.arg
    if ctx.capture is not None:
        ctx.capture.update(arg=arg, s=s)
    h3, w3 = f_fusion.H, f_fusion.W
    t3 = ctx.gather_fold(lv3, arg, h3, w3, lv3.H, lv3.W, 1)
    t2 = ctx.gather_fold(lv2, arg, h3, w3, lv3.H, lv3.W, 2)
    t1 = ctx.gather_fold(lv1, arg, h3, w3, lv3.H, lv3.W, 4)
    if return_arg:
        return s, t3, t2, t1, arg
    return s, t3, t2, t1


def search_transfer(ctx: Ctx, f_fusion: FMap, lv1: FMap, lv2: FMap, lv3: FMap, return_arg=False):
    plan = search_plan(ctx, f_fusion, lv3)
    plan.launch()
    return search_finish(ctx, plan, f_fusion, lv1, lv2, lv3, return_arg)


def self_plan(ctx: Ctx, f_fusion: FMap):
    ctx = ctx.for_stage("search")
    ref = ctx.rot90(f_fusion)
    return ctx.corr_plan(f_fusion, ref, ctx.patch_invnorm(f_fusion), ctx.patch_invnorm(ref))


def self_finish(ctx: Ctx, plan, f_fusion: FMap, P: dict):
    ctx = ctx.for_stage("search")
    s = plan.s
    if ctx.capture is not None:
        ctx.capture.update(s_self=s)
    p1, p2 = P["SelfTransfer.search1"], P["SelfTransfer.search2"]
    t2 = ctx.up_conv1x1_relu(f_fusion, p1["w"], p1["b"], 64)
    t1 = ctx.up_conv1x1_relu(t2, p2["w"], p2["b"], 32)
    return s, f_fusion, t2, t1


def self_transfer(ctx: Ctx, f_fusion: FMap, P: dict):
    plan = self_plan(ctx, f_fusion)
    plan.launch()
    return self_finish(ctx, plan, f_fusion, P)


def decode(ctx: Ctx, ff: FMap, s: torch.Tensor, t3: FMap, t2: FMap, t1: FMap, P: dict, out: torch.Tensor) -> torch.Tensor:
    ctx = ctx.for_stage("decode")
    g = ctx.for_stage("glue")
    g1 = ctx.for_stage("glue1")
    c = lambda name: (P[name]["w"], P[name]["b"])
    h3, w3 = ff.H, ff.W
    smap = FMap(s.view(h3 * w3, 1), h3, w3, 1)
    f_lv3 = g.igemm(ff, *c("conv_lv3"), 128, a1=t3, rowscale=s, residual=ff)
    dec2 = dec_stage(ctx.for_stage("dec2"), f_lv3, P["decoder_second"])
    s2 = ctx.upsample(smap, 2).t.view(-1)
    f_lv2 = g.igemm(dec2, *c("conv_lv2"), 64, a1=t2, rowscale=s2, residual=dec2)
    s1 = g.up_conv1x1_relu(f_lv3, *c("search1"), 64)
    sr2 = g.igemm(f_lv2, *c("search3"), 64, ksize=3, act=ACT_RELU)
    f_v3 = g.igemm(dec2, *c("search2"), 64, a1=s1, act=ACT_RELU, residual=dec2)
    f_lv2 = g.igemm(f_lv2, *c("search2"), 64, a1=sr2, act=ACT_RELU, residual=f_lv2)
    dec1 = dec_stage(ctx.for_stage("dec1"), f_lv2, P["decoder_first"])
    s4 = ctx.upsample(smap, 4).t.view(-1)
    f_lv1 = g1.igemm(dec1, *c("conv_lv1"), 32, a1=t1, rowscale=s4, residual=dec1)
    s13 = g.up_conv1x1_relu(f_v3, *c("search13"), 32)
    s23 = g1.igemm(ctx.upsample(f_lv2, 2), *c("search33"), 32, ksize=3, act=ACT_RELU)
    s33 = g1.igemm(f_lv1, *c("search43"), 32, ksize=3, act=ACT_RELU)
    acc = g1.igemm(s13, *c("search33"), 32, ksize=3, a1=s23, act=ACT_RELU, residual=f_lv1)
    g1.igemm(s13, *c("search33"), 32, ksize=3, a1=s33, act=ACT_RELU, residual=acc, out=acc)
    g1.igemm(s23, *c("search33"), 32, ksize=3, a1=s33, act=ACT_RELU, residual=acc, out=acc)
    ob = P["outBlock"]
    ctx = ctx.for_stage("out")
    f = _resblocks(ctx, acc, ob["blocks"])
    return ctx.for_stage("tail").conv5_out(f, ob["tail_w"], ob["tail_b"], out, ob.get("tail_w32"), ob.get("tail_b32"))


def _lanes(ctx: Ctx, sides) -> list:
    return [torch.cuda.current_stream(ctx.device)] + list(sides or ())


def forward_sample(ctx: Ctx, x: torch.Tensor, P: dict, n_seq: int, has_ref: bool, out: torch.Tensor, sides=()) -> torch.Tensor:
    return _run(forward_sample_steps(ctx, x, P, n_seq, has_ref, out, sides), out)


def _run(steps, out):
    for plan in steps:
        plan.launch()
    return out


def forward_sample_steps(ctx: Ctx, x: torch.Tensor, P: dict, n_seq: int, has_ref: bool, out: torch.Tensor, sides=()):
    h, w = x.shape[-2:]
    h3, w3 = h // 4, w // 4
    dev = x.device
    lanes = _lanes(ctx, sides)
    main = lanes[0]
    if ctx.for_stage("enc").batched_available():
        yield from forward_batch_steps(ctx, x[None], P, n_seq, [not has_ref], out[None], sides)
        return
    for s_ in lanes[1:]:
        s_.wait_stream(main)
    lv = None
    if has_ref:
        with torch.cuda.stream(lanes[-1]):
            lv = reference_pyramid(ctx, x[n_seq + 1], P)
    cat = FMap(torch.empty(h3 * w3, 128 * n_seq, device=dev), h3, w3, 128 * n_seq)
    mid = x[n_seq // 2]
    e0 = enc(ctx, mid, P)
    f_mid = enc(ctx, ctx.rl_prior(mid, 5, 0.01), P, extra=e0, out=cat.view(0, 128))
    others = [i for i in range(n_seq) if i != n_seq // 2]
    if ctx.for_stage("swin").swin_multi_available():
        fb = BMap.empty(len(others), h3, w3, 128, dev)
        for k, i in enumerate(others):
            with torch.cuda.stream(lanes[k % len(lanes)]):
                e = enc(ctx, x[i], P)
                enc(ctx, ctx.rl_prior(x[i], 1, 0.01), P, extra=e, out=fb.map(k))
                del e
        for s_ in lanes[1:]:
            main.wait_stream(s_)
        yield from _fuse_tail(ctx, f_mid, fb, cat, lv, P, out, lanes)
        return
    sx = SwinX(ctx, f_mid, P["swin"])
    ready = torch.cuda.Event()
    ready.record(main)
    for slot, i in enumerate(others, start=1):
        lane = lanes[(slot - 1) % len(lanes)]
        with torch.cuda.stream(lane):
            e = enc(ctx, x[i], P)
            feat = enc(ctx, ctx.rl_prior(x[i], 1, 0.01), P, extra=e)
            if lane is not main:
                lane.wait_event(ready)
            swin(ctx, sx, feat, P["swin"], out=cat.view(128 * slot, 128))
            del e, feat
    for s_ in lanes[1:]:
        main.wait_stream(s_)
    yield from _tail(ctx, cat, lv, P, out)


def forward_batch_steps(ctx: Ctx, x: torch.Tensor, P: dict, n_seq: int, zero_ref: list, out: torch.Tensor, sides=(), max_maps: int = 16):
    B = x.shape[0]
    h, w = x.shape[-2:]
    h3, w3 = h // 4, w // 4
    dev = x.device
    lanes = _lanes(ctx, sides)
    main = lanes[0]
    others = [i for i in range(n_seq) if i != n_seq // 2]
    b0 = 0
    while b0 < B:
        group, maps = [], 0
        while b0 + len(group) < B:
            need = 2 + 2 * len(others) + (0 if zero_ref[b0 + len(group)] else 1)
            if group and maps + need > max_maps:
                break
            group.append(b0 + len(group))
            maps += need
        frames, first = [], {}
        for b in group:
            first[b] = len(frames)
            mid = x[b, n_seq // 2]
            frames += [mid, ctx.rl_prior(mid, 5, 0.01)]
            for i in others:
                frames += [x[b, i], ctx.rl_prior(x[b, i], 1, 0.01)]
            if not zero_ref[b]:
                frames.append(x[b, n_seq + 1])
        lv1, lv2, lv3 = enc_batched(ctx, frames, P)
        del frames
        for b in group:
            m0 = first[b]
            cat = FMap(torch.empty(h3 * w3, 128 * n_seq, device=dev), h3, w3, 128 * n_seq)
            f_mid = FMap(ctx.add(lv3.map(m0 + 1).t, lv3.map(m0).t), h3, w3, 128)
            cat.t[:, :128].copy_(f_mid.t)
            fb = BMap.empty(len(others), h3, w3, 128, dev)
            for k in range(len(others)):
                ctx.add(lv3.map(m0 + 3 + 2 * k).t, lv3.map(m0 + 2 + 2 * k).t, out=fb.map(k).t)
            mr = m0 + 2 + 2 * len(others)
            lv = None if zero_ref[b] else (lv1.map(mr), lv2.map(mr), lv3.map(mr))
            yield from _fuse_tail(ctx, f_mid, fb, cat, lv, P, out[b], lanes)
        b0 += len(group)


def _fuse_tail(ctx: Ctx, f_mid: FMap, fb: BMap, cat: FMap, lv, P: dict, out: torch.Tensor, lanes: list):
    main = lanes[0]
    sx = SwinX(ctx, f_mid, P["swin"])
    if ctx.for_stage("swin").swin_multi_available():
        swin_multi(ctx, sx, fb, P["swin"], [cat.view(128 * slot, 128) for slot in range(1, fb.B + 1)])
    else:
        ready = torch.cuda.Event()
        ready.record(main)
        for slot in range(1, fb.B + 1):
            lane = lanes[(slot - 1) % len(lanes)]
            if lane is not main:
                lane.wait_event(ready)
            with torch.cuda.stream(lane):
                swin(ctx, sx, fb.map(slot - 1), P["swin"], out=cat.view(128 * slot, 128))
        for s_ in lanes[1:]:
            main.wait_stream(s_)
    yield from _tail(ctx, cat, lv, P, out)


def _tail(ctx: Ctx, cat: FMap, lv, P: dict, out: torch.Tensor):
    fw = P["fusion"]
    ff = ctx.igemm(cat, fw["w"], fw["b"], 128)
    plan = search_plan(ctx, ff, lv[2]) if lv is not None else self_plan(ctx, ff)
    yield plan
    if lv is not None:
        s, t3, t2, t1 = search_finish(ctx, plan, ff, *lv)
    else:
        s, t3, t2, t1 = self_finish(ctx, plan, ff, P)
    decode(ctx, ff, s, t3, t2, t1, P, out)


def encode_raw(ctx: Ctx, frame: torch.Tensor, P: dict) -> FMap:
    return enc(ctx, frame, P)


def encode_sum(ctx: Ctx, frame: torch.Tensor, iters: int, e_raw: FMap, P: dict) -> FMap:
    return enc(ctx, ctx.rl_prior(frame, iters, 0.01), P, extra=e_raw)


def reference_pyramid(ctx: Ctx, frame: torch.Tensor, P: dict):
    lv1 = in_block(ctx, frame, P["inBlock"])
    lv2 = enc_stage(ctx, lv1, P["encoder_first"])
    return lv1, lv2, enc_stage(ctx, lv2, P["encoder_second"])


def fuse_and_decode(ctx: Ctx, f_mid: FMap, feats: list, lv, P: dict, n_seq: int, out: torch.Tensor, sides=()) -> torch.Tensor:
    return _run(fuse_and_decode_steps(ctx, f_mid, feats, lv, P, n_seq, out, sides), out)


def fuse_and_decode_steps(ctx: Ctx, f_mid: FMap, feats: list, lv, P: dict, n_seq: int, out: torch.Tensor, sides=()):
    h3, w3 = f_mid.H, f_mid.W
    dev = f_mid.t.device
    lanes = _lanes(ctx, sides)
    main = lanes[0]
    cat = FMap(torch.empty(h3 * w3, 128 * n_seq, device=dev), h3, w3, 128 * n_seq)
    cat.t[:, :128].copy_(f_mid.t)
    fb = BMap(torch.cat([f.t for f in feats]), len(feats), h3, w3, 128)
    yield from _fuse_tail(ctx, f_mid, fb, cat, lv, P, out, lanes)


def forward_swint(ctx: Ctx, x: torch.Tensor, P: dict, n_seq: int, out: torch.Tensor, sides=()) -> torch.Tensor:
    h, w = x.shape[-2:]
    h3, w3 = h // 4, w // 4
    dev = x.device
    lanes = _lanes(ctx, sides)
    main = lanes[0]
    for s_ in lanes[1:]:
        s_.wait_stream(main)
    cat = FMap(torch.empty(h3 * w3, 128 * n_seq, device=dev), h3, w3, 128 * n_seq)
    f_mid = enc(ctx, x[n_seq // 2], P, out=cat.view(0, 128))
    sx = SwinX(ctx, f_mid, P["swin"])
    if n_seq == 1:
        f_trans = FMap.empty(h3, w3, 128, dev)
        swin(ctx, sx, f_mid, P["swin"], out=f_trans)
        cat = FMap(ctx.add(f_mid.t, f_trans.t), h3, w3, 128)
    else:
        ready = torch.cuda.Event()
        ready.record(main)
        for slot, i in enumerate([i for i in range(n_seq) if i != n_seq // 2], start=1):
            lane = lanes[(slot - 1) % len(lanes)]
            if lane is not main:
                lane.wait_event(ready)
            with torch.cuda.stream(lane):
                swin(ctx, sx, enc(ctx, x[i], P), P["swin"], out=cat.view(128 * slot, 128))
        for s_ in lanes[1:]:
            main.wait_stream(s_)
    fw = P["conv"]
    ff = ctx.igemm(cat, fw["w"], fw["b"], 128)
    dctx = ctx.for_stage("decode")
    dec1 = dec_stage(dctx, dec_stage(dctx, ff, P["decoder_second"]), P["decoder_first"])
    ob = P["outBlock"]
    octx = dctx.for_stage("out")
    f = _resblocks(octx, dec1, ob["blocks"])
    return octx.for_stage("tail").conv5_out(f, ob["tail_w"], ob["tail_b"], out, ob.get("tail_w32"), ob.get("tail_b32"))
```

speinet_amd/ops.py:

```python
from __future__ import annotations

import ctypes as C
import dataclasses
from typing import Optional

import numpy as np
import torch

from . import _lib
from .pack import BF16, F16, F32, LP_DTYPE, PackedW, fmt_of

ACT_NONE, ACT_RELU, ACT_GELU = 0, 1, 2
CONV, CONV_T = 0, 1

PRECISIONS = ("f32", "bf16x3", "bf16", "f16")
CORR_PRECISIONS = ("bf16x3", "single", "top2")
_CORR_ALIASES = {"bf16": "single", "bf16r": "top2", "f16": "single"}


class FMap:
    __slots__ = ("t", "H", "W", "C", "ld", "off")

    def __init__(self, t: torch.Tensor, H: int, W: int, C_: int, off: int = 0):
        assert t.is_cuda and t.dtype in (torch.float32, torch.bfloat16, torch.float16) and t.is_contiguous() and t.dim() == 2 and t.shape[0] == H * W
        self.t, self.H, self.W, self.C, self.ld, self.off = t, H, W, C_, t.shape[1], off
        assert off + C_ <= self.ld

    @staticmethod
    def empty(H: int, W: int, C_: int, device, dtype=torch.float32) -> "FMap":
        return FMap(torch.empty(H * W, C_, device=device, dtype=dtype), H, W, C_)

    @property
    def lp(self) -> bool:
        return self.t.dtype != torch.float32

    @property
    def fmt(self) -> int:
        return fmt_of(self.t.dtype)

    def view(self, off: int, C_: int) -> "FMap":
        return FMap(self.t, self.H, self.W, C_, self.off + off)

    @property
    def ptr(self) -> int:
        return self.t.data_ptr() + self.t.element_size() * self.off

    def dense(self) -> torch.Tensor:
        return self.t[:, self.off:self.off + self.C].float().reshape(self.H, self.W, self.C)

    def nchw(self) -> torch.Tensor:
        return self.dense().permute(2, 0, 1).unsqueeze(0).contiguous()

    @staticmethod
    def from_nchw(x: torch.Tensor) -> "FMap":
        if x.dim() == 4:
            x = x[0]
        c, h, w = x.shape
        return FMap(x.permute(1, 2, 0).reshape(h * w, c).contiguous().float(), h, w, c)


class BMap:
    __slots__ = ("t", "B", "H", "W", "C")

    def __init__(self, t: torch.Tensor, B: int, H: int, W: int, C_: int):
        assert t.is_cuda and t.is_contiguous() and t.shape == (B * H * W, C_)
        self.t, self.B, self.H, self.W, self.C = t, B, H, W, C_

    @staticmethod
    def empty(B: int, H: int, W: int, C_: int, device, dtype=torch.float32) -> "BMap":
        return BMap(torch.empty(B * H * W, C_, device=device, dtype=dtype), B, H, W, C_)

    @property
    def fmt(self) -> int:
        return fmt_of(self.t.dtype)

    def map(self, b: int) -> FMap:
        n = self.H * self.W
        return FMap(self.t[b * n:(b + 1) * n], self.H, self.W, self.C)


def _vp(p) -> C.c_void_p:
    return C.c_void_p(p)


class _timed:
    def __init__(self, ctx: "Ctx", name: str):
        self.on = ctx.profile is not None and name in ctx.profile
        self.ctx, self.name = ctx, name

    def __enter__(self):
        if self.on:
            self.s = torch.cuda.Event(enable_timing=True)
            self.e = torch.cuda.Event(enable_timing=True)
            self.s.record(torch.cuda.current_stream(self.ctx.device))
        return self

    def __exit__(self, *a):
        if self.on:
            self.e.record(torch.cuda.current_stream(self.ctx.device))
            self.ctx.profile[self.name].append((self.s, self.e))
        return False


def _tensor_bytes(x) -> int:
    t = x.t if hasattr(x, "t") else x
    return t.numel() * t.element_size() if torch.is_tensor(t) else 0


def _conv_sub(method: str, a, k, out):
    if method == "conv5_in":
        return "level1", 2.0 * 25 * 3 * 32 * a[0].shape[-2] * a[0].shape[-1], _tensor_bytes(a[0]) + _tensor_bytes(out)
    if method == "conv5_out":
        return "level1", 2.0 * 25 * 32 * 3 * a[0].H * a[0].W, _tensor_bytes(a[0]) + 12 * a[0].H * a[0].W
    src, n = a[0], a[3]
    ks = a[4] if len(a) > 4 else k.get("ksize", 1)
    if n == 32 and src.C == 32 and ks == 5 and k.get("stride", a[5] if len(a) > 5 else 1) == 1:
        maps = getattr(src, "B", 1)
        return "level1", 2.0 * 25 * 32 * 32 * maps * src.H * src.W, _tensor_bytes(src) + _tensor_bytes(out)
    return "rest", 0.0, 0


def _family(name: str):
    def deco(fn):
        def wrapper(self, *a, **k):
            pr = self.profile
            if pr is None or "families" not in pr:
                return fn(self, *a, **k)
            st = torch.cuda.current_stream(self.device)
            s_, e_ = torch.cuda.Event(enable_timing=True), torch.cuda.Event(enable_timing=True)
            s_.record(st)
            out = fn(self, *a, **k)
            e_.record(st)
            pr["families"].setdefault(name, []).append((s_, e_))
            if name == "conv":
                sub, fl, by = _conv_sub(fn.__name__, a, k, out)
                rec = pr.setdefault("conv_sub", {}).setdefault(sub, {"events": [], "flops": 0.0, "bytes": 0})
                rec["events"].append((s_, e_))
                rec["flops"] += fl
                rec["bytes"] += by
            return out
        wrapper.__name__, wrapper.__doc__ = fn.__name__, fn.__doc__
        return wrapper
    return deco


def frame_metrics(u8: torch.Tensor, gt_hwc: torch.Tensor, border: int = 4) -> torch.Tensor:
    assert u8.is_cuda and u8.dtype == torch.uint8 and u8.dim() == 3 and u8.shape[2] == 3 and u8.is_contiguous()
    h, w = u8.shape[:2]
    assert gt_hwc.shape == u8.shape and gt_hwc.dtype == torch.uint8 and gt_hwc.device == u8.device and gt_hwc.is_contiguous()
    lib = _lib.lib()
    n = lib.spei_frame_metrics_ws_doubles(h, w, border)
    if n < 0:
        raise ValueError(f"frame {w}x{h} with border {border} is smaller than the 11x11 SSIM window")
    dev = u8.device
    ws = torch.empty(n, dtype=torch.float64, device=dev)
    res = torch.empty(2, dtype=torch.float64, device=dev)
    with torch.cuda.device(dev):
        st = C.c_void_p(torch.cuda.current_stream(dev).cuda_stream)
        _lib.check(lib.spei_frame_metrics(_vp(u8.data_ptr()), _vp(gt_hwc.data_ptr()), h, w, border, _vp(ws.data_ptr()), _vp(res.data_ptr()),
                                          st), "spei_frame_metrics")
    return res


def padded_size(n: int) -> int:
    return -(-n // 20) * 20


def frames_u8_in(u8: torch.Tensor, out: Optional[torch.Tensor] = None, gray: bool = False, planes: bool = True):
    assert u8.is_cuda and u8.dtype == torch.uint8 and u8.dim() in (3, 4) and (planes or gray)
    fr = u8 if u8.dim() == 4 else u8.unsqueeze(0)
    n, h, w, c = fr.shape
    assert c == 3 and fr.stride()[1:] == (w * 3, 3, 1), "frames must be packed [H,W,3] (any frame stride)"
    hp, wp = padded_size(h), padded_size(w)
    dev = u8.device
    if planes:
        if out is None:
            out = torch.empty(n, 3, hp, wp, device=dev)
        assert out.is_cuda and out.device == dev and out.dtype == torch.float32 and out.is_contiguous() and out.numel() == n * 3 * hp * wp
    else:
        out = None
    g = torch.empty(n, h, w, device=dev) if gray else None
    lib = _lib.lib()
    with torch.cuda.device(dev):
        st = C.c_void_p(torch.cuda.current_stream(dev).cuda_stream)
        _lib.check(lib.spei_frames_u8_in(_vp(fr.data_ptr()), fr.stride(0), _vp(out.data_ptr() if out is not None else 0),
                                         _vp(g.data_ptr() if g is not None else 0), n, h, w, st), "spei_frames_u8_in")
    return out, g


def window_mean_u8(u8: torch.Tensor, starts, lengths, gray: bool = False, blur: Optional[torch.Tensor] = None,
                   gt: Optional[torch.Tensor] = None):
    assert u8.is_cuda and u8.dtype == torch.uint8 and u8.dim() == 4
    t, h, w, c = u8.shape
    assert c == 3 and u8.stride()[1:] == (w * 3, 3, 1), "frames must be packed [H,W,3] (any frame stride)"
    runs_host = torch.from_numpy(np.ascontiguousarray(np.stack([np.asarray(starts), np.asarray(lengths)], axis=1).astype(np.int32)))
    m = runs_host.shape[0]
    dev = u8.device
    for name, buf in (("blur", blur), ("gt", gt)):
        assert buf is None or (buf.device == dev and buf.dtype == torch.uint8 and tuple(buf.shape) == (m, h, w, 3) and buf.is_contiguous()), name
    blur = torch.empty(m, h, w, 3, dtype=torch.uint8, device=dev) if blur is None else blur
    gt = torch.empty(m, h, w, 3, dtype=torch.uint8, device=dev) if gt is None else gt
    g = torch.empty(m, h, w, device=dev) if gray else None
    lib = _lib.lib()
    with torch.cuda.device(dev):
        runs = runs_host.to(dev)
        st = C.c_void_p(torch.cuda.current_stream(dev).cuda_stream)
        _lib.check(lib.spei_window_mean_u8(_vp(u8.data_ptr()), u8.stride(0), t, _vp(runs.data_ptr()), _vp(runs_host.data_ptr()), m,
                                           _vp(blur.data_ptr()), _vp(gt.data_ptr()), _vp(g.data_ptr() if g is not None else 0), h, w, st),
                   "spei_window_mean_u8")
    return blur, gt, g


def frame_u8_out(x: torch.Tensor, h: int, w: int, out: Optional[torch.Tensor] = None,
                 nonfinite: Optional[torch.Tensor] = None) -> torch.Tensor:
    assert x.is_cuda and x.dtype == torch.float32 and x.dim() == 3 and x.shape[0] == 3 and x.is_contiguous()
    hp, wp = x.shape[1:]
    if out is None:
        out = torch.empty(h, w, 3, dtype=torch.uint8, device=x.device)
    assert out.device == x.device and out.dtype == torch.uint8 and tuple(out.shape) == (h, w, 3) and out.is_contiguous()
    assert nonfinite is None or (nonfinite.device == x.device and nonfinite.dtype == torch.int32 and nonfinite.numel() >= 1)
    lib = _lib.lib()
    with torch.cuda.device(x.device):
        st = C.c_void_p(torch.cuda.current_stream(x.device).cuda_stream)
        _lib.check(lib.spei_frame_u8_out(_vp(x.data_ptr()), _vp(out.data_ptr()), _vp(nonfinite.data_ptr() if nonfinite is not None else 0),
                                         h, w, hp, wp, st), "spei_frame_u8_out")
    return out


def psnr_f32(a: torch.Tensor, b: torch.Tensor, shave: int = 4, rgb_range: float = 1.0) -> torch.Tensor:
    assert a.is_cuda and a.dtype == torch.float32 and a.dim() == 3 and a.shape[0] == 3 and a.is_contiguous()
    assert b.shape == a.shape and b.dtype == torch.float32 and b.device == a.device and b.is_contiguous()
    lib = _lib.lib()
    dev = a.device
    ws = torch.empty(PSNR_WS_DOUBLES, dtype=torch.float64, device=dev)
    res = torch.empty(2, dtype=torch.float64, device=dev)
    with torch.cuda.device(dev):
        st = C.c_void_p(torch.cuda.current_stream(dev).cuda_stream)
        _lib.check(lib.spei_psnr_f32(_vp(a.data_ptr()), _vp(b.data_ptr()), a.shape[1], a.shape[2], shave, float(rgb_range), _vp(ws.data_ptr()),
                                     _vp(res.data_ptr()), st), "spei_psnr_f32")
    return res


PSNR_WS_DOUBLES = 256


def psnr_of(sq_sum: float, count: float) -> float:
    import math
    mse = sq_sum / count
    return 100.0 if mse == 0 else 20 * math.log10(1.0 / math.sqrt(mse))


CORR_DIAG_WS_MAX = 8 << 30


class CorrPlan:
    __slots__ = ("ctx", "s", "arg", "kernel", "main", "post", "keep")

    def __init__(self, ctx, s, arg, kernel, main, post, keep):
        self.ctx, self.s, self.arg, self.kernel, self.main, self.post, self.keep = ctx, s, arg, kernel, main, post, keep

    def launch(self, profile: Optional[dict] = None) -> None:
        ctx = self.ctx if profile is None else self.ctx.replace(profile=profile)
        st = ctx._stream()
        if ctx.profile is not None:
            ctx.profile["corr_kernel"] = self.kernel
        fam = ctx.profile is not None and "families" in ctx.profile
        if fam:
            f0, f1 = torch.cuda.Event(enable_timing=True), torch.cuda.Event(enable_timing=True)
            f0.record(torch.cuda.current_stream(ctx.device))
        with _timed(ctx, "corr_argmax"):
            for fn, name, args in self.main:
                _lib.check(fn(*args, st), name)
        for fn, name, args in self.post:
            _lib.check(fn(*args, st), name)
        if fam:
            f1.record(torch.cuda.current_stream(ctx.device))
            ctx.profile["families"].setdefault("correlation", []).append((f0, f1))


@dataclasses.dataclass(frozen=True, slots=True, eq=False)
class Ctx:
    ACT_NONE, ACT_RELU, ACT_GELU = ACT_NONE, ACT_RELU, ACT_GELU
    CONV, CONV_T = CONV, CONV_T
    SPLIT_STAGES = ("glue", "dec2")

    precision: str = "f32"
    corr_precision: str = "bf16x3"
    device: Optional[torch.device] = None
    bf16_storage: bool = True
    x1_bf16: bool = True
    fuse_mlp: bool = True
    fuse_attn: bool = True
    commute_upconv: bool = True
    commute_any: bool = False
    corr_bf16: bool = True
    corr_diag: bool = True
    split_decode: bool = True
    batch_enc: bool = True
    attn_win4: bool = True
    conv32_ws: bool = True
    conv64_ws: Optional[bool] = None
    conv3_pipe: bool = True
    stage: Optional[dict] = None
    profile: Optional[dict] = None
    capture: Optional[dict] = None

    def __post_init__(self):
        put = object.__setattr__
        if self.precision not in PRECISIONS:
            raise ValueError(f"unknown precision {self.precision!r}")
        put(self, "corr_precision", _CORR_ALIASES.get(self.corr_precision, self.corr_precision))
        if self.corr_precision not in CORR_PRECISIONS:
            raise ValueError(f"unknown correlation precision {self.corr_precision!r}")
        cur = torch.cuda.current_device() if torch.cuda.is_available() else 0
        device = torch.device("cuda", cur) if self.device is None else torch.device(self.device)
        if device.type != "cuda":
            raise RuntimeError("speinet_amd runs on MI355X only (HIP kernels); there is no CPU path")
        put(self, "device", torch.device("cuda", cur) if device.index is None else device)
        for k in _BOOL_KNOBS:
            if type(getattr(self, k)) is not bool:
                put(self, k, bool(getattr(self, k)))
        if self.conv64_ws is not None:
            put(self, "conv64_ws", bool(self.conv64_ws))
        put(self, "stage", dict(self.stage) if self.stage else {})

    def replace(self, **kw) -> "Ctx":
        return dataclasses.replace(self, **kw)

    def for_stage(self, name: str) -> "Ctx":
        o = self.stage.get(name)
        if o is None and self.split_decode and self.precision == "f16" and name in self.SPLIT_STAGES:
            o = {"precision": "bf16x3", "commute_any": True}
        return self.replace(**o) if o else self

    def _tp(self, t: Optional[torch.Tensor]) -> C.c_void_p:
        if t is None:
            return C.c_void_p(0)
        assert t.is_cuda and t.is_contiguous()
        assert t.device == self.device, f"tensor on {t.device}, call context on {self.device}"
        return C.c_void_p(t.data_ptr())

    def _fp(self, f: Optional[FMap]) -> C.c_void_p:
        if f is None:
            return C.c_void_p(0)
        assert f.t.device == self.device, f"feature map on {f.t.device}, call context on {self.device}"
        return C.c_void_p(f.ptr)

    def _stream(self) -> C.c_void_p:
        assert torch.cuda.current_device() == self.device.index, \
            f"current device cuda:{torch.cuda.current_device()} != call context {self.device}"
        return C.c_void_p(torch.cuda.current_stream(self.device).cuda_stream)

    @property
    def lp16(self) -> bool:
        return self.precision in ("bf16", "f16")

    @property
    def fmt(self) -> int:
        return F16 if self.precision == "f16" else BF16

    def inter_dtype(self) -> torch.dtype:
        return LP_DTYPE[self.fmt] if (self.lp16 and self.bf16_storage) else torch.float32

    def any_nonzero(self, x: torch.Tensor, flag: torch.Tensor) -> None:
        _lib.check(_lib.lib().spei_any_nonzero(self._tp(x), x.numel(), self._tp(flag), self._stream()), "spei_any_nonzero")

    def train_batch(self, table: torch.Tensor, table_host: torch.Tensor, n_in: int, n_gt: int, input: torch.Tensor, gt: torch.Tensor,
                    patch: int, rgb_range: float = 1.0) -> None:
        nb = (n_in + n_gt) * 32
        assert table.dtype == torch.uint8 and table.numel() >= nb and not table_host.is_cuda and table_host.dtype == torch.uint8 \
            and table_host.is_contiguous() and table_host.numel() >= nb
        assert input.dtype == torch.float32 and input.numel() == n_in * 3 * patch * patch
        assert gt.dtype == torch.float32 and gt.numel() == n_gt * 3 * patch * patch
        _lib.check(_lib.lib().spei_train_batch_u8(self._tp(table), C.c_void_p(table_host.data_ptr()), n_in, n_gt, self._tp(input), self._tp(gt),
                                                  patch, float(rgb_range), self._stream()), "spei_train_batch_u8")

    def rl_prior(self, img: torch.Tensor, iters: int, lam: float = 0.01) -> torch.Tensor:
        c, h, w = img.shape
        out = torch.empty_like(img)
        scratch = torch.empty_like(img)
        _lib.check(_lib.lib().spei_rl_prior(self._tp(img), self._tp(out), self._tp(scratch), c, h, w, iters, lam, self._stream()),
                   "spei_rl_prior")
        return out

    @_family("conv")
    def conv5_in(self, img: torch.Tensor, w: torch.Tensor, b: torch.Tensor, out: Optional[FMap] = None) -> FMap:
        c, h, wd = img.shape
        assert c == 3
        if out is None:
            out = FMap.empty(h, wd, b.numel(), img.device)
        assert (out.H, out.W, out.C, out.ld, out.off) == (h, wd, b.numel(), b.numel(), 0) and not out.lp
        _lib.check(_lib.lib().spei_conv5_in(self._tp(img), self._tp(w), self._tp(b), self._fp(out), h, wd, b.numel(), self._stream()),
                   "spei_conv5_in")
        return out

    @_family("conv")
    def conv5_out(self, f: FMap, w: torch.Tensor, b: torch.Tensor, out: torch.Tensor, w32=None,
                  b32: Optional[torch.Tensor] = None) -> torch.Tensor:
        assert out.shape == (3, f.H, f.W) and out.is_contiguous() and out.dtype == torch.float32
        if self.lp16 and w32 is not None and f.C == 32:
            _lib.check(_lib.lib().spei_conv5_out_slab16(self.fmt, self._fp(f), f.ld, f.fmt, self._tp(w32.frag(self.fmt)), self._tp(b32),
                                                       self._tp(out), f.H, f.W, self._stream()), "spei_conv5_out_slab16")
            return out
        if f.lp:
            f = FMap(f.t.float(), f.H, f.W, f.C, f.off)
        _lib.check(_lib.lib().spei_conv5_out(self._fp(f), f.ld, self._tp(w), self._tp(b), self._tp(out), f.H, f.W, f.C, self._stream()),
                   "spei_conv5_out")
        return out

    def _conv3_pipe_ok(self, a, w, N: int, ksize: int, stride: int, act: int, residual, out) -> bool:
        return (self.conv3_pipe and self.lp16 and ksize == 3 and stride == 1 and N == 256 and a.C == 256 and act == ACT_NONE
                and a.H % 6 == 0 and a.W % 16 == 0 and a.H * a.W <= (1 << 21) and a.t.dtype == torch.float32 and getattr(a, "ld", 256) == 256
                and getattr(a, "off", 0) == 0 and getattr(w, "fhi", None) is not None and tuple(w.shape) == (9, 256, 256)
                and (out is None or (out.t.dtype == torch.float32 and getattr(out, "ld", 256) == 256 and getattr(out, "off", 0) == 0
                                     and out.t.data_ptr() != a.t.data_ptr()))
                and (residual is None or (residual.t.dtype == torch.float32 and getattr(residual, "ld", 256) == 256 and getattr(residual, "off", 0) == 0)))

    def _persistent_conv(self, a, w, bias, N: int, ksize: int, stride: int, act: int, residual, out, batch: int) -> bool:
        tp, lib, f = self._tp, _lib.lib(), self.fmt
        if self._conv3_pipe_ok(a, w, N, ksize, stride, act, residual, out):
            _lib.check(lib.spei_conv3x3_256_pipe16(f, tp(a.t), tp(w.frag(f)), tp(bias), tp(residual.t) if residual is not None else _vp(0),
                                                   tp(out.t), batch, a.H, a.W, self._stream()), "spei_conv3x3_256_pipe16")
            return True
        if not (ksize == 5 and stride == 1 and a.C == N and residual is None and act in (ACT_NONE, ACT_RELU) and w.fhi is not None
                and (getattr(a, "ld", N), getattr(a, "off", 0), getattr(out, "ld", N), getattr(out, "off", 0)) == (N, 0, N, 0)
                and a.t.data_ptr() != out.t.data_ptr()):
            return False
        if N == 32 and self.conv32_ws_available():
            _lib.check(lib.spei_conv32_ws16(f, tp(a.t), a.fmt, tp(w.frag(f)), tp(bias), tp(out.t), out.fmt, batch, a.H, a.W, act,
                                            self._stream()), "spei_conv32_ws16")
            return True
        if N == 64 and self.conv64_ws_available():
            _lib.check(lib.spei_conv64_ws16(f, tp(a.t), a.fmt, tp(w.frag(f)), tp(bias), tp(out.t), out.fmt, batch, a.H, a.W, act,
                                            self._stream()), "spei_conv64_ws16")
            return True
        return False

    @_family("conv")
    def igemm(self, a0: FMap, w, bias: Optional[torch.Tensor], N: int, ksize: int = 1, stride: int = 1,
              mode: int = CONV, act: int = ACT_NONE, a1: Optional[FMap] = None, residual: Optional[FMap] = None,
              rowscale: Optional[torch.Tensor] = None, out: Optional[FMap] = None, out_dtype=torch.float32,
              ln_input: bool = False) -> FMap:
        prec = self.precision
        pad = ksize // 2
        if mode == CONV:
            ho, wo = (a0.H + 2 * pad - ksize) // stride + 1, (a0.W + 2 * pad - ksize) // stride + 1
        else:
            ho, wo = a0.H * stride, a0.W * stride
        if out is None:
            out = FMap.empty(ho, wo, N, a0.t.device, out_dtype)
        assert out.H == ho and out.W == wo and out.C == N
        k0, k1 = a0.C, (a1.C if a1 is not None else 0)
        slab = prec != "f32" and mode == CONV
        assert slab or (mode == CONV_T and self.lp16) or not (a0.lp or out.lp), \
            "16-bit activations are only supported by the slab kernel"
        assert a1 is None or a1.t.dtype == a0.t.dtype
        assert residual is None or not residual.lp
        assert all(f.t.dtype in (torch.float32, LP_DTYPE[self.fmt]) for f in (a0, out)), "16-bit tensors must be in the mode's format"
        if torch.is_tensor(w):
            w = PackedW(w, a0.t.device)
        assert not ln_input or (slab and w.fhi is not None), "ln_input is a feature of the slab kernel"
        assert tuple(w.shape) == (ksize * ksize, N, k0 + k1), (tuple(w.shape), ksize, N, k0, k1)
        if a1 is not None:
            assert (a1.H, a1.W) == (a0.H, a0.W)
        if residual is not None:
            assert (residual.H, residual.W, residual.C) == (ho, wo, N)
        if rowscale is not None:
            assert rowscale.numel() == ho * wo
        tp, fp = self._tp, self._fp
        srcs = (fp(a0), a0.ld, k0, fp(a1), a1.ld if a1 is not None else 0, k1)
        lib = _lib.lib()
        if (mode == CONV and a1 is None and rowscale is None and not ln_input
                and self._persistent_conv(a0, w, bias, N, ksize, stride, act, residual, out, 1)):
            return out
        if (mode == CONV_T and self.lp16 and ksize == 3 and stride == 2 and a1 is None and residual is None
                and rowscale is None and N % 32 == 0 and k0 % 32 == 0):
            cf = w.convT_class_frags(self.fmt)
            _lib.check(lib.spei_convt2_slab16(self.fmt, fp(a0), a0.ld, k0, a0.fmt, tp(cf[(0, 0)]), tp(cf[(0, 1)]), tp(cf[(1, 0)]),
                                              tp(cf[(1, 1)]), tp(bias), fp(out), out.ld, out.fmt, a0.H, a0.W, N, act,
                                              self._stream()), "spei_convt2_slab16")
        elif (mode == CONV_T and prec == "bf16x3" and ksize == 3 and stride == 2 and a1 is None and residual is None
                and rowscale is None and N % 32 == 0 and k0 % 32 == 0 and not a0.lp and not out.lp):
            _hi, _lo, ph, pl = w.convT_class_frags_split()
            _lib.check(lib.spei_convt2_slab16x3(fp(a0), a0.ld, k0, ph, pl, tp(bias), fp(out), out.ld, a0.H, a0.W, N, act, self._stream()),
                       "spei_convt2_slab16x3")
        elif prec == "f32":
            _lib.check(lib.spei_igemm_f32(*srcs, tp(w.f32), tp(bias), fp(out), out.ld, fp(residual), residual.ld if residual is not None else 0,
                                          tp(rowscale), a0.H, a0.W, ho, wo, N, ksize, stride, pad, mode, act, self._stream()), "spei_igemm_f32")
        elif slab and w.fhi is not None:
            dims = (a0.H * a0.W, 1, ho * wo, 1) if (ksize == 1 and stride == 1) else (a0.H, a0.W, ho, wo)
            _lib.check(lib.spei_conv_slab16(
                self.fmt, *srcs, a0.fmt, tp(w.frag(self.fmt)), tp(w.flo) if prec == "bf16x3" else _vp(0), tp(bias), fp(out), out.ld,
                out.fmt, fp(residual), residual.ld if residual is not None else 0,
                tp(rowscale), *dims, N, ksize, stride, pad, act, int(ln_input), self._stream()), "spei_conv_slab16")
        else:
            raise ValueError(f"no {prec} kernel for N={N} K={k0 + k1} ksize={ksize} stride={stride} mode={mode}: N and K must be multiples "
                             "of 32; transposed convs 3x3 stride 2")
        return out

    def linear(self, x: torch.Tensor, w, b: Optional[torch.Tensor], act: int = ACT_NONE,
               residual: Optional[torch.Tensor] = None, out: Optional[torch.Tensor] = None, out_dtype=torch.float32,
               ln_input: bool = False) -> torch.Tensor:
        m, k = x.shape
        if torch.is_tensor(w):
            w = PackedW(w.reshape(1, *w.shape), x.device)
        n = w.shape[1]
        if out is None:
            out = torch.empty(m, n, device=x.device, dtype=out_dtype)
        self.igemm(FMap(x, m, 1, k), w, b, n, act=act, ln_input=ln_input,
                   residual=FMap(residual, m, 1, n) if residual is not None else None, out=FMap(out, m, 1, n))
        return out

    @_family("streaming")
    def resblock_gates(self, x1: FMap, pk: dict):
        dev = x1.t.device
        lib = _lib.lib()
        tp = self._tp
        assert x1.off == 0 and x1.ld == x1.C
        s = torch.empty(x1.C, device=dev)
        g1 = torch.empty(x1.H, x1.C, device=dev)
        g2 = torch.empty(x1.W, x1.C, device=dev)
        ws = torch.empty(lib.spei_gate_ws_floats(x1.H, x1.W, x1.C), device=dev)
        _lib.check(lib.spei_resblock_gates(self._fp(x1), x1.fmt, x1.H, x1.W, x1.C, tp(pk["se_w1"]), tp(pk["se_b1"]), tp(pk["se_w2"]),
                                           tp(pk["se_b2"]), tp(pk["cw_w"]), tp(pk["cw_bn"]), tp(pk["hc_w"]), tp(pk["hc_bn"]),
                                           tp(s), tp(g1), tp(g2), tp(ws), self._stream()), "spei_resblock_gates")
        return s, g1, g2

    def resblock(self, x: FMap, pk: dict, extra: Optional[FMap] = None, out: Optional[FMap] = None) -> FMap:
        idt = self.inter_dtype()
        c = x.C
        assert x.off == 0 and x.ld == c
        t = self.igemm(x, pk["w1"], pk["b1"], c, ksize=5, act=ACT_RELU, out_dtype=idt)
        x1 = self.igemm(t, pk["w2"], pk["b2"], c, ksize=5, out_dtype=idt if self.x1_bf16 else torch.float32)
        s, g1, g2 = self.resblock_gates(x1, pk)
        if out is None:
            out = FMap.empty(x.H, x.W, c, x.t.device)
        if extra is not None:
            assert extra.off == 0 and extra.ld == c
        self._apply(x, x1, s, g1, g2, extra, out, c)
        return out

    @_family("streaming")
    def _apply(self, x, x1, s, g1, g2, extra, out, c):
        _lib.check(_lib.lib().spei_resblock_apply(self._fp(x), self._fp(x1), x1.fmt, self._tp(s), self._tp(g1), self._tp(g2),
                                                  self._fp(extra), self._fp(out), out.ld, x.H, x.W, c, self._stream()),
                   "spei_resblock_apply")

    def batched_available(self) -> bool:
        return self.batched_kernels() and self.x1_bf16 and self.bf16_storage and self.batch_enc

    def conv32_ws_available(self) -> bool:
        return self.lp16 and self.conv32_ws

    def conv64_ws_available(self) -> bool:
        return self.lp16 and (self.conv32_ws if self.conv64_ws is None else self.conv64_ws)

    def batched_kernels(self) -> bool:
        return self.lp16

    @_family("conv")
    def igemm_batched(self, a: BMap, w, bias: torch.Tensor, N: int, ksize: int, stride: int = 1, act: int = ACT_NONE,
                      out_dtype=torch.float32, residual: Optional[BMap] = None, out: Optional[BMap] = None) -> BMap:
        assert self.batched_kernels() and not torch.is_tensor(w) and w.fhi is not None
        pad = ksize // 2
        ho, wo = (a.H + 2 * pad - ksize) // stride + 1, (a.W + 2 * pad - ksize) // stride + 1
        assert tuple(w.shape) == (ksize * ksize, N, a.C) and a.t.dtype in (torch.float32, LP_DTYPE[self.fmt])
        if out is None:
            out = BMap.empty(a.B, ho, wo, N, a.t.device, out_dtype)
        assert (out.B, out.H, out.W, out.C) == (a.B, ho, wo, N) and out.t.data_ptr() != a.t.data_ptr()
        if residual is not None:
            assert (residual.B, residual.H, residual.W, residual.C) == (a.B, ho, wo, N) and residual.t.dtype == torch.float32
            assert residual.t.data_ptr() != a.t.data_ptr()
        tp = self._tp
        if self._persistent_conv(a, w, bias, N, ksize, stride, act, residual, out, a.B):
            return out
        _lib.check(_lib.lib().spei_conv_slab16_batched(self.fmt, tp(a.t), a.C, a.fmt, tp(w.frag(self.fmt)), _vp(0), tp(bias), tp(out.t), out.fmt,
                                                       tp(residual.t) if residual is not None else _vp(0), a.B, a.H, a.W, ho, wo, N, ksize,
                                                       stride, pad, act, self._stream()),
                   "spei_conv_slab16_batched")
        return out

    def resblock_batched(self, x: BMap, pk: dict) -> BMap:
        idt = self.inter_dtype()
        c, dev = x.C, x.t.device
        lib = _lib.lib()
        tp = self._tp
        t = self.igemm_batched(x, pk["w1"], pk["b1"], c, 5, act=ACT_RELU, out_dtype=idt)
        x1 = self.igemm_batched(t, pk["w2"], pk["b2"], c, 5, out_dtype=idt)
        del t
        return self._gates_apply_batched(x, x1, pk)

    @_family("streaming")
    def _gates_apply_batched(self, x: BMap, x1: BMap, pk: dict) -> BMap:
        c, dev = x.C, x.t.device
        lib = _lib.lib()
        tp = self._tp
        s = torch.empty(x.B, c, device=dev)
        g1 = torch.empty(x.B, x.H, c, device=dev)
        g2 = torch.empty(x.B, x.W, c, device=dev)
        ws = torch.empty(x.B * lib.spei_gate_ws_floats(x.H, x.W, c), device=dev)
        _lib.check(lib.spei_resblock_gates_batched(tp(x1.t), x1.fmt, x.B, x.H, x.W, c, tp(pk["se_w1"]), tp(pk["se_b1"]), tp(pk["se_w2"]),
                                                   tp(pk["se_b2"]), tp(pk["cw_w"]), tp(pk["cw_bn"]), tp(pk["hc_w"]), tp(pk["hc_bn"]),
                                                   tp(s), tp(g1), tp(g2), tp(ws), self._stream()), "spei_resblock_gates_batched")
        out = BMap.empty(x.B, x.H, x.W, c, dev)
        _lib.check(lib.spei_resblock_apply_batched(tp(x.t), tp(x1.t), x1.fmt, tp(s), tp(g1), tp(g2), tp(out.t), x.B, x.H, x.W, c,
                                                   self._stream()), "spei_resblock_apply_batched")
        return out

    def ln_fused_available(self) -> bool:
        return self.precision != "f32"

    def attn_fused_available(self) -> bool:
        return self.lp16 and self.fuse_attn and self.bf16_storage

    def mlp_fused_available(self) -> bool:
        return self.lp16 and self.fuse_mlp

    def swin_multi_available(self) -> bool:
        return self.attn_fused_available() and self.attn_win4 and self.mlp_fused_available() and self.batched_kernels()

    @_family("swin")
    def attn_fused(self, x: torch.Tensor, yhat: torch.Tensor, bk: dict, H: int, W: int, shift: int, out: torch.Tensor) -> torch.Tensor:
        assert x.shape[0] % (H * W) == 0 and x.shape[1] == 256 and x.dtype == torch.float32 and out.shape == x.shape and out.dtype == torch.float32
        f = self.fmt
        assert yhat.shape == x.shape and yhat.dtype == LP_DTYPE[f]
        tp = self._tp
        batch = x.shape[0] // (H * W)
        if self.attn_win4:
            _lib.check(_lib.lib().spei_attn_win4_16(f, tp(x), tp(out), tp(yhat), tp(bk["wq"].frag(f)), tp(bk["bq"]), tp(bk["wkv"].frag(f)),
                                                    tp(bk["bkv"]), tp(bk["wproj"].frag(f)), tp(bk["bproj"]), tp(bk["relbias"]), batch, H, W,
                                                    shift, self._stream()), "spei_attn_win4_16")
            return out
        assert batch == 1, "the two-window kernel takes one map per launch"
        _lib.check(_lib.lib().spei_attn_fused16(f, tp(x), tp(out), tp(yhat), tp(bk["wq"].frag(f)), tp(bk["bq"]), tp(bk["wkv"].frag(f)),
                                                tp(bk["bkv"]), tp(bk["wproj"].frag(f)), tp(bk["bproj"]), tp(bk["relbias"]), H, W, shift,
                                                self._stream()), "spei_attn_fused16")
        return out

    @_family("swin")
    def mlp_fused(self, x: torch.Tensor, w1, b1: torch.Tensor, w2, b2: torch.Tensor, out: torch.Tensor) -> torch.Tensor:
        assert x.shape[1] == 256 and x.dtype == torch.float32 and out.shape == x.shape and out.dtype == torch.float32
        assert tuple(w1.shape) == (1, 512, 256) and tuple(w2.shape) == (1, 256, 512)
        tp = self._tp
        f = self.fmt
        _lib.check(_lib.lib().spei_mlp_fused16(f, tp(x), tp(out), tp(w1.frag(f)), tp(b1), tp(w2.frag(f)), tp(b2), x.shape[0], self._stream()),
                   "spei_mlp_fused16")
        return out

    def layernorm(self, x: torch.Tensor, g: Optional[torch.Tensor] = None, b: Optional[torch.Tensor] = None,
                  out: Optional[torch.Tensor] = None, out_dtype=torch.float32) -> torch.Tensor:
        assert x.shape[1] == 256 and x.is_contiguous() and x.dtype == torch.float32
        if out is None:
            out = torch.empty(x.shape, device=x.device, dtype=out_dtype)
        tp = self._tp
        _lib.check(_lib.lib().spei_layernorm256(tp(x), tp(out), fmt_of(out.dtype), tp(g), tp(b), x.shape[0], self._stream()),
                   "spei_layernorm256")
        return out

    def window_attention(self, q: torch.Tensor, kv: torch.Tensor, relbias: torch.Tensor, H: int, W: int, shift: int,
                         out: Optional[torch.Tensor] = None) -> torch.Tensor:
        assert q.shape == (H * W, 256) and kv.shape == (H * W, 512) and relbias.shape == (8, 25, 25)
        if out is None:
            out = torch.empty_like(q)
        assert q.dtype == kv.dtype == out.dtype
        tp = self._tp
        _lib.check(_lib.lib().spei_window_attention(tp(q), tp(kv), fmt_of(q.dtype), tp(relbias), tp(out), H, W, shift,
                                                    self._stream()), "spei_window_attention")
        return out

    def patch_invnorm(self, f: FMap) -> torch.Tensor:
        inv = torch.empty(f.H * f.W, device=f.t.device)
        _lib.check(_lib.lib().spei_patch_invnorm(self._fp(f), f.ld, self._tp(inv), f.H, f.W, f.C, self._stream()), "spei_patch_invnorm")
        return inv

    def corr_plan(self, lr: FMap, ref: FMap, inv_lr: torch.Tensor, inv_ref: torch.Tensor) -> "CorrPlan":
        lib = _lib.lib()
        dev = lr.t.device
        tp, fp = self._tp, self._fp
        n = lr.H * lr.W
        s = torch.empty(n, device=dev)
        arg = torch.empty(n, device=dev, dtype=torch.int32)
        dims = (lr.H, lr.W, ref.H, ref.W, lr.C)
        rescore = self.precision != "f32" and self.corr_precision == "top2" and lr.C == 128
        diag, diag_floats = False, 0
        if rescore and self.corr_diag and ref.H >= lr.H:
            diag_floats = lib.spei_corr_diag_ws_floats(lr.H, lr.W, ref.H, ref.W)
            diag = 4 * diag_floats <= min(torch.cuda.mem_get_info(dev)[0] // 4, CORR_DIAG_WS_MAX)
        ws = torch.empty(diag_floats if diag else lib.spei_corr_ws_floats(n), device=dev)
        if self.precision == "f32":
            args = (fp(lr), lr.ld, fp(ref), ref.ld, tp(inv_lr), tp(inv_ref), *dims, tp(s), tp(arg), tp(ws))
            return CorrPlan(self, s, arg, "corr_argmax_kernel (f32 MFMA)", [(lib.spei_corr_argmax, "spei_corr_argmax", args)], [],
                            (lr, ref, inv_lr, inv_ref, ws))
        split = self.corr_precision == "bf16x3"
        f16 = BF16 if (rescore and self.corr_bf16) else self.fmt
        assert f16 == BF16 or (not split and lr.C == 128), "f16 correlation: slab kernel, single / top2"
        parts = []
        for f in (lr, ref):
            hi = torch.empty(f.H * f.W, f.C, device=dev, dtype=LP_DTYPE[f16])
            lo = torch.empty_like(hi) if split else None
            _lib.check(lib.spei_split16(f16, fp(f), f.ld, tp(hi), tp(lo), f.H * f.W, f.C, self._stream()), "spei_split16")
            parts += [hi, lo]
        fname = "f16" if f16 == F16 else "bf16"
        if rescore:
            arg2 = torch.empty(n, device=dev, dtype=torch.int32)
            s2 = torch.empty(n, device=dev)
            if diag:
                main = (lib.spei_corr_diag_top2_16, "spei_corr_diag_top2_16",
                        (f16, tp(parts[0]), tp(parts[2]), tp(inv_ref), *dims, tp(s), tp(arg), tp(s2), tp(arg2), tp(ws)))
            else:
                main = (lib.spei_corr_slab_top2_16, "spei_corr_slab_top2_16",
                        (f16, tp(parts[0]), tp(parts[2]), tp(inv_lr), tp(inv_ref), *dims, tp(s), tp(arg), tp(s2), tp(arg2), tp(ws)))
            post = (lib.spei_corr_rescore, "spei_corr_rescore",
                    (fp(lr), lr.ld, fp(ref), ref.ld, tp(inv_lr), tp(inv_ref), *dims, tp(s), tp(arg), tp(s2), tp(arg2)))
            return CorrPlan(self, s, arg, f"corr_{'diag' if diag else 'slab'}_kernel<top2, {fname}>", [main], [post],
                            (lr, ref, inv_lr, inv_ref, ws, parts, s2, arg2))
        args = (tp(parts[0]), tp(parts[1]), tp(parts[2]), tp(parts[3]), tp(inv_lr), tp(inv_ref), *dims, tp(s), tp(arg), tp(ws))
        if lr.C == 128:
            main = (lib.spei_corr_slab16, "spei_corr_slab16", (f16, *args))
            kname = f"corr_slab_kernel<{'bf16x3' if split else 'top1, ' + fname}>"
        else:
            main = (lib.spei_corr_argmax_bf16, "spei_corr_argmax_bf16", args)
            kname = f"corr_bf16_kernel<{'bf16x3' if split else 'bf16'}>"
        return CorrPlan(self, s, arg, kname, [main], [], (lr, ref, inv_lr, inv_ref, ws, parts))

    def corr_argmax(self, lr: FMap, ref: FMap, inv_lr: torch.Tensor, inv_ref: torch.Tensor):
        plan = self.corr_plan(lr, ref, inv_lr, inv_ref)
        plan.launch()
        return plan.s, plan.arg

    def gather_fold(self, ref: FMap, arg: torch.Tensor, H3: int, W3: int, Hr3: int, Wr3: int, s: int) -> FMap:
        assert ref.H == Hr3 * s and ref.W == Wr3 * s
        out = FMap.empty(H3 * s, W3 * s, ref.C, ref.t.device)
        _lib.check(_lib.lib().spei_gather_fold(self._fp(ref), ref.ld, self._tp(arg), self._fp(out), out.ld, H3, W3, Hr3, Wr3, ref.C, s,
                                               self._stream()), "spei_gather_fold")
        return out

    def rot90(self, f: FMap) -> FMap:
        out = FMap.empty(f.W, f.H, f.C, f.t.device)
        _lib.check(_lib.lib().spei_rot90(self._fp(f), f.ld, self._fp(out), f.H, f.W, f.C, self._stream()), "spei_rot90")
        return out

    def upsample(self, f: FMap, s: int, act: int = ACT_NONE) -> FMap:
        out = FMap.empty(f.H * s, f.W * s, f.C, f.t.device)
        _lib.check(_lib.lib().spei_upsample_bicubic(self._fp(f), f.ld, self._fp(out), out.ld, f.H, f.W, f.C, s, act, self._stream()),
                   "spei_upsample_bicubic")
        return out

    def up_conv1x1_relu(self, f: FMap, w, b: torch.Tensor, n: int, s: int = 2) -> FMap:
        if (self.lp16 and self.commute_upconv) or self.commute_any:
            return self.upsample(self.igemm(f, w, b, n), s, act=ACT_RELU)
        return self.igemm(self.upsample(f, s), w, b, n, act=ACT_RELU)

    def add(self, a: torch.Tensor, b: torch.Tensor, out: Optional[torch.Tensor] = None) -> torch.Tensor:
        if out is None:
            out = torch.empty_like(a)
        assert out.shape == a.shape == b.shape and out.dtype == a.dtype == torch.float32
        _lib.check(_lib.lib().spei_add(self._tp(a), self._tp(b), self._tp(out), a.numel(), self._stream()), "spei_add")
        return out


_BOOL_KNOBS = tuple(f.name for f in dataclasses.fields(Ctx) if f.type in (bool, "bool"))
```

Baseline: 42.41.

## Fuse correlation prep, layernorm pair, batched adds, and multi-query rescore

Several independent fusions are added. Patch inverse-norm and the f16 split are computed in one tiled kernel, and the two back-to-back layernorms become one paired kernel. The per-pair add calls plus the copy into the concat buffer become a single batched launch that writes directly into the concat slice. The rescore kernel is replaced by one that handles two queries per wave, with predicated, fully unrolled loads of the 3x3 neighbourhoods. Together these cut kernel launches and repeated global reads of the feature maps, at the cost of larger register use in the rescore kernel and shared-memory tiling in the prep kernel.

Result: no change. 42.57 (median of 6 runs) (+0.4%).

```diff
diff --git a/include/speinet_hip.h b/include/speinet_hip.h
--- a/include/speinet_hip.h
+++ b/include/speinet_hip.h
@@ -105,6 +105,9 @@
 int spei_layernorm256(const float* x, void* y, int out_fmt, const float* gamma, const float* beta, int64_t M,
                       spei_stream_t stream);
 
+int spei_layernorm256_pair(const float* x, void* y, int out_fmt, const float* gamma, const float* beta, int64_t M,
+                           spei_stream_t stream);
+
 int spei_window_attention(const void* q, const void* kv, int io_fmt, const float* relbias, void* out, int H, int W,
                           int shift, spei_stream_t stream);
 int spei_window_attention_batched(const void* q, const void* kv, int io_fmt, const float* relbias, void* out, int H, int W,
@@ -118,6 +121,7 @@
                      float* ws, spei_stream_t stream);
 
 int spei_split16(int fmt, const float* x, int ld, void* hi, void* lo, int64_t M, int C, spei_stream_t stream);
+int spei_corr_prep16(int fmt, const float* f, int ldf, float* inv, void* hi, void* lo, int H, int W, int C, spei_stream_t stream);
 int spei_corr_argmax_bf16(const void* lr_hi, const void* lr_lo, const void* ref_hi, const void* ref_lo,
                           const float* inv_lr, const float* inv_ref, int Hl, int Wl, int Hr, int Wr, int C, float* S,
                           int32_t* arg, float* ws, spei_stream_t stream);
@@ -136,6 +140,9 @@
                       int Hl, int Wl, int Hr, int Wr, int C, float* S, int32_t* arg, const float* S2, const int32_t* arg2,
                       spei_stream_t stream);
 
+int spei_corr_rescore_mq(const float* lr, int ldl, const float* ref, int ldr, const float* inv_lr, const float* inv_ref,
+                         int Hl, int Wl, int Hr, int Wr, int C, float* S, int32_t* arg, const int32_t* arg2, spei_stream_t stream);
+
 int spei_gather_fold(const float* ref, int ldr, const int32_t* arg, float* out, int ldo, int H3, int W3,
                      int Hr3, int Wr3, int C, int s, spei_stream_t stream);
 
@@ -145,6 +152,8 @@
                           spei_stream_t stream);
 
 int spei_add(const float* a, const float* b, float* out, int64_t n, spei_stream_t stream);
+int spei_add_batched(const float* const* a, const float* const* b, float* const* out, const int32_t* ldo, int batch, int64_t rows,
+                     int C, spei_stream_t stream);
 
 
 int64_t spei_wgrad_ws_floats(int Hout, int Wout, int N, int K, int ksize);
diff --git a/speinet_amd/csrc/common.h b/speinet_amd/csrc/common.h
--- a/speinet_amd/csrc/common.h
+++ b/speinet_amd/csrc/common.h
@@ -136,6 +136,21 @@
     h[0] = to_lp<LP>(v[0]); h[1] = to_lp<LP>(v[1]); h[2] = to_lp<LP>(v[2]); h[3] = to_lp<LP>(v[3]);
     return h;
 }
+__device__ __forceinline__ float patch_sumsq_step(float v, float acc) { return __builtin_fmaf(v, v, acc); }
+__device__ __forceinline__ float patch_invnorm_of(float sumsq) { return 1.0f / fmaxf(sqrtf(sumsq), 1e-12f); }
+template <typename LP>
+__device__ __forceinline__ typename lpv<LP>::x4 split16_hi(float4 v) {
+    typename lpv<LP>::x4 h;
+    h[0] = (LP)v.x; h[1] = (LP)v.y; h[2] = (LP)v.z; h[3] = (LP)v.w;
+    return h;
+}
+template <typename LP>
+__device__ __forceinline__ typename lpv<LP>::x4 split16_lo(float4 v, typename lpv<LP>::x4 h) {
+    typename lpv<LP>::x4 l;
+    l[0] = (LP)(v.x - (float)h[0]); l[1] = (LP)(v.y - (float)h[1]);
+    l[2] = (LP)(v.z - (float)h[2]); l[3] = (LP)(v.w - (float)h[3]);
+    return l;
+}
 typedef unsigned u32x4 __attribute__((ext_vector_type(4)));
 
 template <int CTRL>
diff --git a/speinet_amd/csrc/search.hip b/speinet_amd/csrc/search.hip
--- a/speinet_amd/csrc/search.hip
+++ b/speinet_amd/csrc/search.hip
@@ -16,11 +16,11 @@
             const int xx = x + dx;
             if (xx < 0 || xx >= W) continue;
             const float* row = f + ((size_t)yy * W + xx) * ldf;
-            for (int c = lane; c < C; c += 64) acc = fmaf(row[c], row[c], acc);
+            for (int c = lane; c < C; c += 64) acc = patch_sumsq_step(row[c], acc);
         }
     }
     acc = wave_sum(acc);
-    if (lane == 0) inv[p] = 1.0f / fmaxf(sqrtf(acc), 1e-12f);
+    if (lane == 0) inv[p] = patch_invnorm_of(acc);
 }
 
 constexpr int CBM = 128, CBN = 128, CBK = 32, CLD = CBK + 1, CMAXSPLIT = 8;
@@ -200,6 +200,22 @@
     arg[i] = ix == 0x7fffffff ? 0 : ix;
 }
 
+__device__ __forceinline__ double rescore_dot2(float2 a, float2 b, double acc) {
+#pragma clang fp contract(off)
+    return acc + ((double)a.x * (double)b.x + (double)a.y * (double)b.y);
+}
+__device__ __forceinline__ void rescore_decide(const double d[2], const int cand[2], int nc, const float* __restrict__ inv_lr,
+                                               const float* __restrict__ inv_ref, int64_t q, float* __restrict__ S, int32_t* __restrict__ arg) {
+    const double s0 = d[0] * (double)inv_ref[cand[0]];
+    int win = cand[0];
+    double sw = s0;
+    if (nc == 2) {
+        const double s1 = d[1] * (double)inv_ref[cand[1]];
+        if (s1 > s0 || (s1 == s0 && cand[1] < cand[0])) { win = cand[1]; sw = s1; }
+    }
+    S[q] = (float)(sw * (double)inv_lr[q]);
+    arg[q] = win;
+}
 __global__ __launch_bounds__(256) void corr_rescore_kernel(const float* __restrict__ lr, int ldl, const float* __restrict__ ref, int ldr,
                                                            const float* __restrict__ inv_lr, const float* __restrict__ inv_ref,
                                                            int Hl, int Wl, int Hr, int Wr, int C, float* __restrict__ S,
@@ -224,23 +240,67 @@
             for (int c = lane * 2; c < C; c += 128) {
                 const float2 av = *reinterpret_cast<const float2*>(a + c);
                 const float2 bv = *reinterpret_cast<const float2*>(b + c);
-                acc += (double)av.x * (double)bv.x + (double)av.y * (double)bv.y;
+                acc = rescore_dot2(av, bv, acc);
             }
             d[k] += acc;
         }
     }
     for (int k = 0; k < 2; ++k)
         for (int m = 32; m >= 1; m >>= 1) d[k] += __shfl_xor(d[k], m, 64);
-    if (lane == 0) {
-        const double s0 = d[0] * (double)inv_ref[cand[0]];
-        int win = cand[0];
-        double sw = s0;
-        if (nc == 2) {
-            const double s1 = d[1] * (double)inv_ref[cand[1]];
-            if (s1 > s0 || (s1 == s0 && cand[1] < cand[0])) { win = cand[1]; sw = s1; }
-        }
-        S[q] = (float)(sw * (double)inv_lr[q]);
-        arg[q] = win;
+    if (lane == 0) rescore_decide(d, cand, nc, inv_lr, inv_ref, q, S, arg);
+}
+
+constexpr int RQ = 2;
+__global__ __launch_bounds__(256) void corr_rescore_mq_kernel(const float* __restrict__ lr, int ldl, const float* __restrict__ ref, int ldr,
+                                                              const float* __restrict__ inv_lr, const float* __restrict__ inv_ref,
+                                                              int Hl, int Wl, int Hr, int Wr, float* __restrict__ S,
+                                                              int32_t* __restrict__ arg, const int32_t* __restrict__ arg2) {
+    const int lane = threadIdx.x & 63;
+    const int64_t N = (int64_t)Hl * Wl;
+    const int64_t q0 = ((int64_t)blockIdx.x * 4 + (threadIdx.x >> 6)) * RQ;
+    if (q0 >= N) return;
+    int cand[RQ][2], nc[RQ], qy[RQ], qx[RQ];
+#pragma unroll
+    for (int u = 0; u < RQ; ++u) {
+        const int64_t q = q0 + u < N ? q0 + u : N - 1;
+        cand[u][0] = arg[q];
+        cand[u][1] = arg2[q];
+        qy[u] = (int)(q / Wl);
+        qx[u] = (int)(q - (int64_t)qy[u] * Wl);
+    }
+    float2 av[RQ][9], bv[RQ][2][9];
+    bool oka[RQ][9], okb[RQ][2][9];
+#pragma unroll
+    for (int u = 0; u < RQ; ++u) {
+        nc[u] = cand[u][1] >= 0 ? 2 : 1;
+#pragma unroll
+        for (int t = 0; t < 9; ++t) {
+            const int ty = t / 3 - 1, tx = t - (t / 3) * 3 - 1;
+            const int y = qy[u] + ty, x = qx[u] + tx;
+            oka[u][t] = y >= 0 && y < Hl && x >= 0 && x < Wl;
+            av[u][t] = *reinterpret_cast<const float2*>(lr + ((size_t)min(max(y, 0), Hl - 1) * Wl + min(max(x, 0), Wl - 1)) * ldl + lane * 2);
+#pragma unroll
+            for (int k = 0; k < 2; ++k) {
+                const int cj = k < nc[u] ? cand[u][k] : 0;
+                const int cy = cj / Wr + ty, cx = cj % Wr + tx;
+                okb[u][k][t] = k < nc[u] && cy >= 0 && cy < Hr && cx >= 0 && cx < Wr;
+                bv[u][k][t] = *reinterpret_cast<const float2*>(ref + ((size_t)min(max(cy, 0), Hr - 1) * Wr + min(max(cx, 0), Wr - 1)) * ldr + lane * 2);
+            }
+        }
+    }
+#pragma unroll
+    for (int u = 0; u < RQ; ++u) {
+        double d[2] = {0.0, 0.0};
+#pragma unroll
+        for (int t = 0; t < 9; ++t)
+#pragma unroll
+            for (int k = 0; k < 2; ++k) {
+                const double term = rescore_dot2(av[u][t], bv[u][k][t], 0.0);
+                d[k] = (oka[u][t] && okb[u][k][t]) ? d[k] + term : d[k];
+            }
+        for (int k = 0; k < 2; ++k)
+            for (int m = 32; m >= 1; m >>= 1) d[k] += __shfl_xor(d[k], m, 64);
+        if (lane == 0 && q0 + u < N) rescore_decide(d, cand[u], nc[u], inv_lr, inv_ref, q0 + u, S, arg);
     }
 }
 
@@ -337,6 +397,19 @@
     return 0;
 }
 
+extern "C" int spei_corr_rescore_mq(const float* lr, int ldl, const float* ref, int ldr, const float* inv_lr, const float* inv_ref,
+                                    int Hl, int Wl, int Hr, int Wr, int C, float* S, int32_t* arg, const int32_t* arg2, spei_stream_t stream) {
+    SPEI_REQUIRE(lr && ref && inv_lr && inv_ref && S && arg && arg2, "spei_corr_rescore_mq: null pointer");
+    SPEI_REQUIRE(C == 128 && ldl % 2 == 0 && ldr % 2 == 0 && ldl >= C && ldr >= C, "spei_corr_rescore_mq: C=%d (must be 128) ldl=%d ldr=%d", C, ldl, ldr);
+    SPEI_REQUIRE(Hl > 0 && Wl > 0 && Hr > 0 && Wr > 0, "spei_corr_rescore_mq: empty map");
+    SPEI_REQUIRE((int64_t)Hl * Wl < (1ll << 30) && (int64_t)Hr * Wr < (1ll << 30), "spei_corr_rescore_mq: map too large");
+    SPEI_REQUIRE(((uintptr_t)lr | (uintptr_t)ref) % 8 == 0, "spei_corr_rescore_mq: 8-byte alignment required");
+    hipLaunchKernelGGL(corr_rescore_mq_kernel, dim3(cdiv((int64_t)Hl * Wl, 4 * RQ)), dim3(256), 0, (hipStream_t)stream, lr, ldl, ref, ldr,
+                       inv_lr, inv_ref, Hl, Wl, Hr, Wr, S, arg, arg2);
+    SPEI_CHECK_LAUNCH("spei_corr_rescore_mq");
+    return 0;
+}
+
 extern "C" int spei_gather_fold(const float* ref, int ldr, const int32_t* arg, float* out, int ldo, int H3, int W3,
                                 int Hr3, int Wr3, int C, int s, spei_stream_t stream) {
     SPEI_REQUIRE(ref && arg && out, "spei_gather_fold: null pointer");
diff --git a/speinet_amd/csrc/search_bf16.hip b/speinet_amd/csrc/search_bf16.hip
--- a/speinet_amd/csrc/search_bf16.hip
+++ b/speinet_amd/csrc/search_bf16.hip
@@ -15,15 +15,53 @@
         const int c = (int)(i % cg) * 4;
         const int64_t m = i / cg;
         const float4 v = *reinterpret_cast<const float4*>(x + m * ld + c);
-        lp4 h;
-        h[0] = (LP)v.x; h[1] = (LP)v.y; h[2] = (LP)v.z; h[3] = (LP)v.w;
+        const lp4 h = split16_hi<LP>(v);
         *reinterpret_cast<lp4*>(hi + m * C + c) = h;
-        if (lo) {
-            lp4 l;
-            l[0] = (LP)(v.x - (float)h[0]); l[1] = (LP)(v.y - (float)h[1]);
-            l[2] = (LP)(v.z - (float)h[2]); l[3] = (LP)(v.w - (float)h[3]);
-            *reinterpret_cast<lp4*>(lo + m * C + c) = l;
-        }
+        if (lo) *reinterpret_cast<lp4*>(lo + m * C + c) = split16_lo<LP>(v, h);
+    }
+}
+
+constexpr int PT = 8, PTH = PT + 2, PC = 128;
+template <typename LP>
+__global__ __launch_bounds__(256) void corr_prep_kernel(const float* __restrict__ f, int ld, float* __restrict__ inv, LP* __restrict__ hi,
+                                                        LP* __restrict__ lo, int H, int W) {
+    typedef typename lpv<LP>::x4 lp4;
+    __shared__ __attribute__((aligned(16))) float t[PTH * PTH * PC];
+    const int tid = threadIdx.x, lane = tid & 63, wave = tid >> 6;
+    const int x0 = blockIdx.x * PT, y0 = blockIdx.y * PT;
+    for (int i = tid; i < PTH * PTH * (PC / 4); i += 256) {
+        const int pix = i / (PC / 4), c = (i - pix * (PC / 4)) * 4;
+        const int ly = pix / PTH, lx = pix - ly * PTH;
+        const int gy = y0 + ly - 1, gx = x0 + lx - 1;
+        float4 v = make_float4(0.f, 0.f, 0.f, 0.f);
+        if (gy >= 0 && gy < H && gx >= 0 && gx < W) {
+            const size_t m = (size_t)gy * W + gx;
+            v = *reinterpret_cast<const float4*>(f + m * ld + c);
+            if (ly >= 1 && ly <= PT && lx >= 1 && lx <= PT) {
+                const lp4 h = split16_hi<LP>(v);
+                *reinterpret_cast<lp4*>(hi + m * PC + c) = h;
+                if (lo) *reinterpret_cast<lp4*>(lo + m * PC + c) = split16_lo<LP>(v, h);
+            }
+        }
+        *reinterpret_cast<float4*>(t + pix * PC + c) = v;
+    }
+    __syncthreads();
+#pragma unroll 4
+    for (int j = 0; j < PT * PT / 4; ++j) {
+        const int p = wave * (PT * PT / 4) + j, py = p / PT, px = p - py * PT;
+        const int gy = y0 + py, gx = x0 + px;
+        if (gy >= H || gx >= W) continue;
+        float acc = 0.f;
+#pragma unroll
+        for (int dy = 0; dy < 3; ++dy)
+#pragma unroll
+            for (int dx = 0; dx < 3; ++dx) {
+                const float* row = t + ((py + dy) * PTH + px + dx) * PC;
+                acc = patch_sumsq_step(row[lane], acc);
+                acc = patch_sumsq_step(row[lane + 64], acc);
+            }
+        acc = wave_sum(acc);
+        if (lane == 0) inv[(size_t)gy * W + gx] = patch_invnorm_of(acc);
     }
 }
 
@@ -250,6 +288,20 @@
     else
         hipLaunchKernelGGL(split16_kernel<__bf16>, dim3(blocks), dim3(256), 0, (hipStream_t)stream, x, ld, (__bf16*)hi, (__bf16*)lo, M, C);
     SPEI_CHECK_LAUNCH("spei_split16");
+    return 0;
+}
+
+extern "C" int spei_corr_prep16(int fmt, const float* f, int ldf, float* inv, void* hi, void* lo, int H, int W, int C, spei_stream_t stream) {
+    SPEI_REQUIRE(f && inv && hi && H > 0 && W > 0, "spei_corr_prep16: bad arguments");
+    SPEI_REQUIRE(C == PC && ldf % 4 == 0 && ldf >= C, "spei_corr_prep16: C=%d (must be %d) ldf=%d", C, PC, ldf);
+    SPEI_REQUIRE(fmt == SPEI_BF16 || fmt == SPEI_F16, "spei_corr_prep16: fmt=%d", fmt);
+    SPEI_REQUIRE((uintptr_t)f % 16 == 0 && ((uintptr_t)hi | (uintptr_t)lo) % 8 == 0, "spei_corr_prep16: alignment");
+    const dim3 grid(cdiv(W, PT), cdiv(H, PT));
+    if (fmt == SPEI_F16)
+        hipLaunchKernelGGL(corr_prep_kernel<_Float16>, grid, dim3(256), 0, (hipStream_t)stream, f, ldf, inv, (_Float16*)hi, (_Float16*)lo, H, W);
+    else
+        hipLaunchKernelGGL(corr_prep_kernel<__bf16>, grid, dim3(256), 0, (hipStream_t)stream, f, ldf, inv, (__bf16*)hi, (__bf16*)lo, H, W);
+    SPEI_CHECK_LAUNCH("spei_corr_prep16");
     return 0;
 }
 
diff --git a/speinet_amd/csrc/stencil.hip b/speinet_amd/csrc/stencil.hip
--- a/speinet_amd/csrc/stencil.hip
+++ b/speinet_amd/csrc/stencil.hip
@@ -374,3 +374,41 @@
     SPEI_CHECK_LAUNCH("spei_add");
     return 0;
 }
+
+constexpr int ADD_MAX_BATCH = 8;
+struct AddBatch {
+    const float* a[ADD_MAX_BATCH];
+    const float* b[ADD_MAX_BATCH];
+    float* o[ADD_MAX_BATCH];
+    int ldo[ADD_MAX_BATCH];
+};
+__global__ __launch_bounds__(256) void add_batched_kernel(const AddBatch p, int64_t rows, int C) {
+    const int m = blockIdx.y;
+    const float* __restrict__ a = p.a[m];
+    const float* __restrict__ b = p.b[m];
+    float* __restrict__ o = p.o[m];
+    const int ldo = p.ldo[m], cg = C / 4;
+    const int64_t total = rows * cg;
+    for (int64_t i = (int64_t)blockIdx.x * 256 + threadIdx.x; i < total; i += (int64_t)gridDim.x * 256) {
+        const int64_t r = i / cg;
+        const int c = (int)(i - r * cg) * 4;
+        const float4 x = reinterpret_cast<const float4*>(a)[i], y = reinterpret_cast<const float4*>(b)[i];
+        *reinterpret_cast<float4*>(o + r * ldo + c) = make_float4(x.x + y.x, x.y + y.y, x.z + y.z, x.w + y.w);
+    }
+}
+extern "C" int spei_add_batched(const float* const* a, const float* const* b, float* const* out, const int32_t* ldo, int batch,
+                                int64_t rows, int C, spei_stream_t stream) {
+    SPEI_REQUIRE(a && b && out && ldo && batch >= 1 && batch <= ADD_MAX_BATCH && rows > 0 && C > 0 && C % 4 == 0,
+                 "spei_add_batched: bad arguments (batch 1..%d, C %% 4 == 0)", ADD_MAX_BATCH);
+    AddBatch p = {};
+    for (int m = 0; m < batch; ++m) {
+        SPEI_REQUIRE(a[m] && b[m] && out[m] && ldo[m] >= C && ldo[m] % 4 == 0, "spei_add_batched: map %d: null pointer or ldo=%d", m, ldo[m]);
+        SPEI_REQUIRE(((uintptr_t)a[m] | (uintptr_t)b[m] | (uintptr_t)out[m]) % 16 == 0, "spei_add_batched: 16-byte alignment required");
+        p.a[m] = a[m]; p.b[m] = b[m]; p.o[m] = out[m]; p.ldo[m] = ldo[m];
+    }
+    const int64_t total = rows * (C / 4);
+    const int blocks = (int)((total + 255) / 256 < 2048 ? (total + 255) / 256 : 2048);
+    hipLaunchKernelGGL(add_batched_kernel, dim3(blocks, batch), dim3(256), 0, (hipStream_t)stream, p, rows, C);
+    SPEI_CHECK_LAUNCH("spei_add_batched");
+    return 0;
+}
diff --git a/speinet_amd/csrc/swin.hip b/speinet_amd/csrc/swin.hip
--- a/speinet_amd/csrc/swin.hip
+++ b/speinet_amd/csrc/swin.hip
@@ -2,6 +2,29 @@
 
 namespace {
 
+__device__ __forceinline__ float4 ln256_row(float4 v, float4 g, float4 b) {
+#pragma clang fp contract(off)
+    const float mean = wave_sum((v.x + v.y) + (v.z + v.w)) * (1.0f / 256.0f);
+    const float dx = v.x - mean, dy = v.y - mean, dz = v.z - mean, dw = v.w - mean;
+    const float ss = wave_sum((dx * dx + dy * dy) + (dz * dz + dw * dw));
+    const float rstd = 1.0f / sqrtf(__builtin_fmaf(ss, 1.0f / 256.0f, 1e-5f));
+    float4 o;
+    o.x = __builtin_fmaf(g.x, dx * rstd, b.x);
+    o.y = __builtin_fmaf(g.y, dy * rstd, b.y);
+    o.z = __builtin_fmaf(g.z, dz * rstd, b.z);
+    o.w = __builtin_fmaf(g.w, dw * rstd, b.w);
+    return o;
+}
+template <typename TO>
+__device__ __forceinline__ void ln256_store(TO* y, int lane, float4 o) {
+    if constexpr (sizeof(TO) == 4) {
+        reinterpret_cast<float4*>(y)[lane] = o;
+    } else {
+        typename lpv<TO>::x4 h;
+        h[0] = (TO)o.x; h[1] = (TO)o.y; h[2] = (TO)o.z; h[3] = (TO)o.w;
+        reinterpret_cast<typename lpv<TO>::x4*>(y)[lane] = h;
+    }
+}
 template <typename TO>
 __global__ __launch_bounds__(256) void layernorm256_kernel(const float* __restrict__ x, TO* __restrict__ y,
                                                            const float* __restrict__ gamma, const float* __restrict__ beta,
@@ -12,24 +35,26 @@
     float4 g = make_float4(1.f, 1.f, 1.f, 1.f), b = make_float4(0.f, 0.f, 0.f, 0.f);
     if (gamma) g = reinterpret_cast<const float4*>(gamma)[lane];
     if (beta) b = reinterpret_cast<const float4*>(beta)[lane];
-    for (int64_t m = wave; m < M; m += nwaves) {
-        const float4 v = reinterpret_cast<const float4*>(x + m * 256)[lane];
-        const float mean = wave_sum((v.x + v.y) + (v.z + v.w)) * (1.0f / 256.0f);
-        const float dx = v.x - mean, dy = v.y - mean, dz = v.z - mean, dw = v.w - mean;
-        const float var = wave_sum((dx * dx + dy * dy) + (dz * dz + dw * dw)) * (1.0f / 256.0f);
-        const float rstd = 1.0f / sqrtf(var + 1e-5f);
-        float4 o;
-        o.x = dx * rstd * g.x + b.x;
-        o.y = dy * rstd * g.y + b.y;
-        o.z = dz * rstd * g.z + b.z;
-        o.w = dw * rstd * g.w + b.w;
-        if (sizeof(TO) == 4) {
-            reinterpret_cast<float4*>(y + m * 256)[lane] = o;
-        } else {
-            typename lpv<TO>::x4 h;
-            h[0] = (TO)o.x; h[1] = (TO)o.y; h[2] = (TO)o.z; h[3] = (TO)o.w;
-            reinterpret_cast<typename lpv<TO>::x4*>(y + m * 256)[lane] = h;
-        }
+    for (int64_t m = wave; m < M; m += nwaves)
+        ln256_store<TO>(y + m * 256, lane, ln256_row(reinterpret_cast<const float4*>(x + m * 256)[lane], g, b));
+}
+template <typename TO>
+__global__ __launch_bounds__(256) void layernorm256_pair_kernel(const float* __restrict__ x, TO* __restrict__ y,
+                                                                const float* __restrict__ gamma, const float* __restrict__ beta,
+                                                                int64_t M) {
+    const int lane = threadIdx.x & 63;
+    const int64_t wave = (int64_t)blockIdx.x * 4 + (threadIdx.x >> 6);
+    const int64_t nwaves = (int64_t)gridDim.x * 4;
+    float4 g = make_float4(1.f, 1.f, 1.f, 1.f), b = make_float4(0.f, 0.f, 0.f, 0.f);
+    if (gamma) g = reinterpret_cast<const float4*>(gamma)[lane];
+    if (beta) b = reinterpret_cast<const float4*>(beta)[lane];
+    const float4 one = make_float4(1.f, 1.f, 1.f, 1.f), zero = make_float4(0.f, 0.f, 0.f, 0.f);
+    for (int64_t m = wave; m < M; m += 2 * nwaves) {
+        const int64_t m1 = m + nwaves;
+        const float4 v0 = reinterpret_cast<const float4*>(x + m * 256)[lane];
+        const float4 v1 = reinterpret_cast<const float4*>(x + (m1 < M ? m1 : m) * 256)[lane];
+        ln256_store<TO>(y + m * 256, lane, ln256_row(ln256_row(v0, g, b), one, zero));
+        if (m1 < M) ln256_store<TO>(y + m1 * 256, lane, ln256_row(ln256_row(v1, g, b), one, zero));
     }
 }
 
@@ -154,6 +179,18 @@
     return 0;
 }
 
+extern "C" int spei_layernorm256_pair(const float* x, void* y, int out_fmt, const float* gamma, const float* beta, int64_t M,
+                                      spei_stream_t stream) {
+    SPEI_REQUIRE(x && y && M > 0, "spei_layernorm256_pair: bad arguments");
+    SPEI_REQUIRE(out_fmt == SPEI_BF16 || out_fmt == SPEI_F16, "spei_layernorm256_pair: out_fmt=%d (a 16-bit format)", out_fmt);
+    SPEI_REQUIRE(((uintptr_t)x | (uintptr_t)gamma | (uintptr_t)beta) % 16 == 0 && (uintptr_t)y % 8 == 0, "spei_layernorm256_pair: alignment");
+    const dim3 grid((unsigned)((M + 7) / 8 < 8192 ? (M + 7) / 8 : 8192));
+    if (out_fmt == SPEI_BF16) hipLaunchKernelGGL(layernorm256_pair_kernel<__bf16>, grid, dim3(256), 0, (hipStream_t)stream, x, (__bf16*)y, gamma, beta, M);
+    else hipLaunchKernelGGL(layernorm256_pair_kernel<_Float16>, grid, dim3(256), 0, (hipStream_t)stream, x, (_Float16*)y, gamma, beta, M);
+    SPEI_CHECK_LAUNCH("spei_layernorm256_pair");
+    return 0;
+}
+
 static int window_attention_run(const void* q, const void* kv, int io_fmt, const float* relbias, void* out, int H, int W, int shift, int batch,
                                 spei_stream_t stream) {
     SPEI_REQUIRE(q && kv && relbias && out, "spei_window_attention: null pointer");
diff --git a/speinet_amd/engine.py b/speinet_amd/engine.py
--- a/speinet_amd/engine.py
+++ b/speinet_amd/engine.py
@@ -65,16 +65,21 @@
         self.xt0 = ctx.layernorm(self.x_first.t, sw["pe_g"], sw["pe_b"])
 
 
+def _yhat(ctx: Ctx, y_first: torch.Tensor, sw: dict, idt: torch.dtype) -> torch.Tensor:
+    if idt != torch.float32:
+        return ctx.layernorm_pair(y_first, sw["pe_g"], sw["pe_b"], idt)
+    return ctx.layernorm(ctx.layernorm(y_first, sw["pe_g"], sw["pe_b"]), out_dtype=idt)
+
+
 def swin(ctx: Ctx, sx: SwinX, feat: FMap, sw: dict, out: FMap) -> FMap:
     ctx = ctx.for_stage("swin")
     h, w = feat.H, feat.W
     m = h * w
     dev = feat.t.device
     y_first = ctx.igemm(feat, sw["conv_first_w"], sw["conv_first_b"], 256, ksize=3)
-    yt = ctx.layernorm(y_first.t, sw["pe_g"], sw["pe_b"])
     idt = ctx.inter_dtype()
-    yhat = ctx.layernorm(yt, out_dtype=idt)
-    del y_first, yt
+    yhat = _yhat(ctx, y_first.t, sw, idt)
+    del y_first
     r = sx.xt0.clone()
     bufs = [torch.empty(m, 256, device=dev), torch.empty(m, 256, device=dev)]
     xh = torch.empty(m, 256, device=dev, dtype=idt)
@@ -121,10 +126,8 @@
     m = h * w
     dev = feats.t.device
     y_first = ctx.igemm_batched(feats, sw["conv_first_w"], sw["conv_first_b"], 256, 3)
-    yt = ctx.layernorm(y_first.t, sw["pe_g"], sw["pe_b"])
-    idt = ctx.inter_dtype()
-    yhat = ctx.layernorm(yt, out_dtype=idt)
-    del y_first, yt
+    yhat = _yhat(ctx, y_first.t, sw, ctx.inter_dtype())
+    del y_first
     r = sx.xt0.repeat(B, 1)
     bufs = [torch.empty(B * m, 256, device=dev), torch.empty(B * m, 256, device=dev)]
     for layer in sw["layers"]:
@@ -146,7 +149,7 @@
 
 def search_plan(ctx: Ctx, f_fusion: FMap, lv3: FMap):
     ctx = ctx.for_stage("search")
-    return ctx.corr_plan(f_fusion, lv3, ctx.patch_invnorm(f_fusion), ctx.patch_invnorm(lv3))
+    return ctx.corr_plan(f_fusion, lv3)
 
 
 def search_finish(ctx: Ctx, plan, f_fusion: FMap, lv1: FMap, lv2: FMap, lv3: FMap, return_arg=False):
@@ -172,7 +175,7 @@
 def self_plan(ctx: Ctx, f_fusion: FMap):
     ctx = ctx.for_stage("search")
     ref = ctx.rot90(f_fusion)
-    return ctx.corr_plan(f_fusion, ref, ctx.patch_invnorm(f_fusion), ctx.patch_invnorm(ref))
+    return ctx.corr_plan(f_fusion, ref)
 
 
 def self_finish(ctx: Ctx, plan, f_fusion: FMap, P: dict):
@@ -315,11 +318,11 @@
         for b in group:
             m0 = first[b]
             cat = FMap(torch.empty(h3 * w3, 128 * n_seq, device=dev), h3, w3, 128 * n_seq)
-            f_mid = FMap(ctx.add(lv3.map(m0 + 1).t, lv3.map(m0).t), h3, w3, 128)
-            cat.t[:, :128].copy_(f_mid.t)
+            f_mid = cat.view(0, 128)
             fb = BMap.empty(len(others), h3, w3, 128, dev)
-            for k in range(len(others)):
-                ctx.add(lv3.map(m0 + 3 + 2 * k).t, lv3.map(m0 + 2 + 2 * k).t, out=fb.map(k).t)
+            pairs = range(1 + len(others))
+            ctx.add_batched([lv3.map(m0 + 1 + 2 * j) for j in pairs], [lv3.map(m0 + 2 * j) for j in pairs],
+                            [f_mid] + [fb.map(k) for k in range(len(others))])
             mr = m0 + 2 + 2 * len(others)
             lv = None if zero_ref[b] else (lv1.map(mr), lv2.map(mr), lv3.map(mr))
             yield from _fuse_tail(ctx, f_mid, fb, cat, lv, P, out[b], lanes)
diff --git a/speinet_amd/ops.py b/speinet_amd/ops.py
--- a/speinet_amd/ops.py
+++ b/speinet_amd/ops.py
@@ -657,6 +657,14 @@
                    "spei_layernorm256")
         return out
 
+    def layernorm_pair(self, x: torch.Tensor, g: torch.Tensor, b: torch.Tensor, out_dtype) -> torch.Tensor:
+        assert x.shape[1] == 256 and x.is_contiguous() and x.dtype == torch.float32 and out_dtype in (torch.bfloat16, torch.float16)
+        out = torch.empty(x.shape, device=x.device, dtype=out_dtype)
+        tp = self._tp
+        _lib.check(_lib.lib().spei_layernorm256_pair(tp(x), tp(out), fmt_of(out_dtype), tp(g), tp(b), x.shape[0], self._stream()),
+                   "spei_layernorm256_pair")
+        return out
+
     def window_attention(self, q: torch.Tensor, kv: torch.Tensor, relbias: torch.Tensor, H: int, W: int, shift: int,
                          out: Optional[torch.Tensor] = None) -> torch.Tensor:
         assert q.shape == (H * W, 256) and kv.shape == (H * W, 512) and relbias.shape == (8, 25, 25)
@@ -673,7 +681,17 @@
         _lib.check(_lib.lib().spei_patch_invnorm(self._fp(f), f.ld, self._tp(inv), f.H, f.W, f.C, self._stream()), "spei_patch_invnorm")
         return inv
 
-    def corr_plan(self, lr: FMap, ref: FMap, inv_lr: torch.Tensor, inv_ref: torch.Tensor) -> "CorrPlan":
+    def corr_prep(self, f: FMap, f16: int, split: bool = False):
+        assert f.C == 128 and not f.lp
+        dev = f.t.device
+        inv = torch.empty(f.H * f.W, device=dev)
+        hi = torch.empty(f.H * f.W, f.C, device=dev, dtype=LP_DTYPE[f16])
+        lo = torch.empty_like(hi) if split else None
+        _lib.check(_lib.lib().spei_corr_prep16(f16, self._fp(f), f.ld, self._tp(inv), self._tp(hi), self._tp(lo), f.H, f.W, f.C, self._stream()),
+                   "spei_corr_prep16")
+        return inv, hi, lo
+
+    def corr_plan(self, lr: FMap, ref: FMap, inv_lr: Optional[torch.Tensor] = None, inv_ref: Optional[torch.Tensor] = None) -> "CorrPlan":
         lib = _lib.lib()
         dev = lr.t.device
         tp, fp = self._tp, self._fp
@@ -688,18 +706,26 @@
             diag = 4 * diag_floats <= min(torch.cuda.mem_get_info(dev)[0] // 4, CORR_DIAG_WS_MAX)
         ws = torch.empty(diag_floats if diag else lib.spei_corr_ws_floats(n), device=dev)
         if self.precision == "f32":
+            inv_lr = self.patch_invnorm(lr) if inv_lr is None else inv_lr
+            inv_ref = self.patch_invnorm(ref) if inv_ref is None else inv_ref
             args = (fp(lr), lr.ld, fp(ref), ref.ld, tp(inv_lr), tp(inv_ref), *dims, tp(s), tp(arg), tp(ws))
             return CorrPlan(self, s, arg, "corr_argmax_kernel (f32 MFMA)", [(lib.spei_corr_argmax, "spei_corr_argmax", args)], [],
                             (lr, ref, inv_lr, inv_ref, ws))
         split = self.corr_precision == "bf16x3"
         f16 = BF16 if (rescore and self.corr_bf16) else self.fmt
         assert f16 == BF16 or (not split and lr.C == 128), "f16 correlation: slab kernel, single / top2"
-        parts = []
-        for f in (lr, ref):
-            hi = torch.empty(f.H * f.W, f.C, device=dev, dtype=LP_DTYPE[f16])
-            lo = torch.empty_like(hi) if split else None
-            _lib.check(lib.spei_split16(f16, fp(f), f.ld, tp(hi), tp(lo), f.H * f.W, f.C, self._stream()), "spei_split16")
+        parts, invs = [], []
+        for f, inv in ((lr, inv_lr), (ref, inv_ref)):
+            if inv is None and f.C == 128:
+                inv, hi, lo = self.corr_prep(f, f16, split)
+            else:
+                inv = self.patch_invnorm(f) if inv is None else inv
+                hi = torch.empty(f.H * f.W, f.C, device=dev, dtype=LP_DTYPE[f16])
+                lo = torch.empty_like(hi) if split else None
+                _lib.check(lib.spei_split16(f16, fp(f), f.ld, tp(hi), tp(lo), f.H * f.W, f.C, self._stream()), "spei_split16")
             parts += [hi, lo]
+            invs.append(inv)
+        inv_lr, inv_ref = invs
         fname = "f16" if f16 == F16 else "bf16"
         if rescore:
             arg2 = torch.empty(n, device=dev, dtype=torch.int32)
@@ -710,8 +736,8 @@
             else:
                 main = (lib.spei_corr_slab_top2_16, "spei_corr_slab_top2_16",
                         (f16, tp(parts[0]), tp(parts[2]), tp(inv_lr), tp(inv_ref), *dims, tp(s), tp(arg), tp(s2), tp(arg2), tp(ws)))
-            post = (lib.spei_corr_rescore, "spei_corr_rescore",
-                    (fp(lr), lr.ld, fp(ref), ref.ld, tp(inv_lr), tp(inv_ref), *dims, tp(s), tp(arg), tp(s2), tp(arg2)))
+            post = (lib.spei_corr_rescore_mq, "spei_corr_rescore_mq",
+                    (fp(lr), lr.ld, fp(ref), ref.ld, tp(inv_lr), tp(inv_ref), *dims, tp(s), tp(arg), tp(arg2)))
             return CorrPlan(self, s, arg, f"corr_{'diag' if diag else 'slab'}_kernel<top2, {fname}>", [main], [post],
                             (lr, ref, inv_lr, inv_ref, ws, parts, s2, arg2))
         args = (tp(parts[0]), tp(parts[1]), tp(parts[2]), tp(parts[3]), tp(inv_lr), tp(inv_ref), *dims, tp(s), tp(arg), tp(ws))
@@ -758,5 +784,16 @@
         _lib.check(_lib.lib().spei_add(self._tp(a), self._tp(b), self._tp(out), a.numel(), self._stream()), "spei_add")
         return out
 
+    def add_batched(self, a: list, b: list, out: list) -> None:
+        n = len(out)
+        assert 1 <= n <= 8 and len(a) == len(b) == n
+        rows, c = a[0].H * a[0].W, a[0].C
+        for x, y, o in zip(a, b, out):
+            assert (x.H * x.W, x.C, x.ld, x.off) == (rows, c, c, 0) == (y.H * y.W, y.C, y.ld, y.off) and (o.H * o.W, o.C) == (rows, c)
+            assert not (x.lp or y.lp or o.lp)
+        arr = lambda fs: (C.c_void_p * n)(*[self._fp(f).value for f in fs])
+        ldo = (C.c_int32 * n)(*[o.ld for o in out])
+        _lib.check(_lib.lib().spei_add_batched(arr(a), arr(b), arr(out), ldo, n, rows, c, self._stream()), "spei_add_batched")
+
 
 _BOOL_KNOBS = tuple(f.name for f in dataclasses.fields(Ctx) if f.type in (bool, "bool"))
```
